# harveybc/gym-fx

Measured on AMD Instinct MI355X. Metric: env-steps/sec (whole node) PPO EURUSD-1m 4096 vec-envs, higher is better.
Workload: dtype bf16; 1 GPU; model=PPO MLP(256,256) actor-critic bf16 MFMA, global_batch=524288, seq_len=32, parallelism=dp1, n_envs_per_gpu=4096, rollout_steps=128, obs_dim=260, preprocessor=feature_window_preprocessor, reward=pnl_reward, pairs=1

## Files before the change

### gymfx_amd/algo/ppo.py

```python
from __future__ import annotations

import time
from dataclasses import dataclass
from typing import Any, Dict, List

import torch

from ..envs.vec_env import VecFxEnv
from ..models.lstm import ActorCriticLSTM
from ..models.mlp import ActorCriticMLP
from ..ops import api


@dataclass
class PPOConfig:
    rollout_steps: int = 128
    ppo_epochs: int = 4
    minibatches: int = 8
    gamma: float = 0.99
    gae_lambda: float = 0.95
    clip_eps: float = 0.2
    ent_coef: float = 0.01
    vf_coef: float = 0.5
    lr: float = 3e-4
    max_grad_norm: float = 0.5
    seed: int = 0
    hidden: int = 256
    normalize_adv: bool = True
    shuffle_rows: bool = True
    use_graphs: bool = True
    policy: str = "mlp"
    bptt_len: int = 16
    fused_rollout: bool = False
    rollout_streams: int = 1
    fuse_sample: bool = True
    fuse_head: bool = False
    overlap_gather: bool = False

    @classmethod
    def from_config(cls, cfg: Dict[str, Any]) -> "PPOConfig":
        out = cls()
        mapping = {
            "rollout_steps": "rollout_steps",
            "ppo_epochs": "ppo_epochs",
            "minibatches": "minibatches",
            "gamma": "gamma",
            "gae_lambda": "gae_lambda",
            "clip_eps": "clip_eps",
            "ent_coef": "ent_coef",
            "vf_coef": "vf_coef",
            "lr": "learning_rate",
            "max_grad_norm": "max_grad_norm",
            "hidden": "hidden_size",
            "normalize_adv": "normalize_adv",
            "shuffle_rows": "shuffle_rows",
            "use_graphs": "use_graphs",
            "policy": "policy_model",
            "bptt_len": "bptt_len",
            "rollout_streams": "rollout_streams",
            "fused_rollout": "fused_rollout",
            "fuse_sample": "fuse_sample",
            "fuse_head": "fuse_head",
            "overlap_gather": "overlap_gather",
        }
        from ..config.merger import convert_type

        for attr, key in mapping.items():
            if cfg.get(key) is not None:
                cur = getattr(out, attr)
                val = convert_type(cfg[key]) if isinstance(cur, bool) else cfg[key]
                setattr(out, attr, type(cur)(val))
        if cfg.get("seed") is not None:
            out.seed = int(cfg["seed"])
        return out


class PPOTrainer:
    def __init__(self, env: VecFxEnv, cfg: PPOConfig, *, rank: int = 0,
                 world_size: int = 1, process_group=None):
        self.env = env
        self.cfg = cfg
        self.rank = rank
        self.world_size = world_size
        self.pg = process_group
        self.device = env.device
        if getattr(env.params, "action_space_mode", "discrete") != "discrete":
            raise ValueError(
                "PPO training uses the 3-way discrete head; set "
                "action_space_mode='discrete' (continuous mode is for "
                "external agents driving the env, reference "
                "env.py:343-360 coercion semantics)")

        N = env.n_envs
        T = cfg.rollout_steps
        D = env.obs_dim
        self.N, self.T, self.D = N, T, D
        n_actions = 3

        self.recurrent = cfg.policy == "lstm"
        if self.recurrent:
            if T % cfg.bptt_len != 0:
                raise ValueError("rollout_steps must divide by bptt_len")
            if not cfg.shuffle_rows:
                raise ValueError("recurrent PPO requires shuffle_rows")
            self.model = ActorCriticLSTM(
                D, n_actions, cfg.hidden, device=self.device, seed=cfg.seed
            )
        else:
            self.model = ActorCriticMLP(
                D, n_actions, cfg.hidden, device=self.device, seed=cfg.seed
            )

        dev = self.device
        self.obs_buf = torch.empty(T, N, D, dtype=torch.bfloat16, device=dev)
        self.act_buf = torch.empty(T, N, dtype=torch.int64, device=dev)
        self.logp_buf = torch.empty(T, N, dtype=torch.float32, device=dev)
        self.val_buf = torch.empty(T + 1, N, dtype=torch.float32, device=dev)
        self.rew_buf = torch.empty(T, N, dtype=torch.float32, device=dev)
        self.done_buf = torch.empty(T, N, dtype=torch.bool, device=dev)
        self.adv_buf = torch.empty(T, N, dtype=torch.float32, device=dev)
        self.ret_buf = torch.empty(T, N, dtype=torch.float32, device=dev)
        self._adv_part = torch.empty(512, dtype=torch.float32, device=dev)

        self.acts_rollout = self.model.alloc_acts(N)
        self.obs_bf16_step = torch.empty(N, D, dtype=torch.bfloat16, device=dev)

        TN = T * N
        self.obs_flat = self.obs_buf.view(TN, D)
        self.act_flat = self.act_buf.view(TN)
        self.logp_flat = self.logp_buf.view(TN)
        self.adv_flat = self.adv_buf.view(TN)
        self.ret_flat = self.ret_buf.view(TN)
        self.losses = torch.zeros(5, dtype=torch.float32, device=dev)

        if self.recurrent:
            H = cfg.hidden
            L = cfg.bptt_len
            self.n_chunks = T // L
            n_seq = self.n_chunks * N
            if n_seq % cfg.minibatches != 0:
                raise ValueError("(T/bptt_len)*n_envs must divide by minibatches")
            Mseq = n_seq // cfg.minibatches
            self.mseq = Mseq
            self.mb_rows = L * Mseq
            self.rnn_state = self.model.alloc_state(N)
            self.h0_buf = torch.zeros(self.n_chunks, N, H, dtype=torch.float32, device=dev)
            self.c0_buf = torch.zeros(self.n_chunks, N, H, dtype=torch.float32, device=dev)
            self.obs_mb_seq = torch.empty(L, Mseq, D, dtype=torch.bfloat16, device=dev)
            self.act_mb = torch.empty(L, Mseq, dtype=torch.int64, device=dev)
            self.logp_mb = torch.empty(L, Mseq, dtype=torch.float32, device=dev)
            self.adv_mb = torch.empty(L, Mseq, dtype=torch.float32, device=dev)
            self.ret_mb = torch.empty(L, Mseq, dtype=torch.float32, device=dev)
            self.done_mb = torch.empty(L, Mseq, dtype=torch.bool, device=dev)
            self.h0_mb = torch.empty(Mseq, H, dtype=torch.bfloat16, device=dev)
            self.c0_mb = torch.empty(Mseq, H, dtype=torch.float32, device=dev)
            self.bptt = self.model.alloc_bptt(L, Mseq)
            self.dhead = torch.empty(L * Mseq, n_actions + 1,
                                     dtype=torch.bfloat16, device=dev)
            self._boot_state = self.model.alloc_state(N)
            self._overlap = False
        else:
            M = TN // cfg.minibatches
            if M * cfg.minibatches != TN:
                raise ValueError("rollout_steps * n_envs must divide by minibatches")
            self.mb_rows = M
            self.acts_train = self.model.alloc_acts(M)
            self.scratch = self.model.alloc_scratch(M)
            self.dhead = torch.empty(M, n_actions + 1, dtype=torch.bfloat16, device=dev)
            self._overlap = (self.device.type == "cuda" and cfg.overlap_gather
                             and cfg.shuffle_rows)
            ns = 2 if self._overlap else 1
            self.obs_mb_s = [torch.empty(M, D, dtype=torch.bfloat16, device=dev)
                             for _ in range(ns)]
            self.act_mb_s = [torch.empty(M, dtype=torch.int64, device=dev)
                             for _ in range(ns)]
            self.logp_mb_s = [torch.empty(M, dtype=torch.float32, device=dev)
                              for _ in range(ns)]
            self.adv_mb_s = [torch.empty(M, dtype=torch.float32, device=dev)
                             for _ in range(ns)]
            self.ret_mb_s = [torch.empty(M, dtype=torch.float32, device=dev)
                             for _ in range(ns)]
            self.obs_mb = self.obs_mb_s[0]
            self.act_mb = self.act_mb_s[0]
            self.logp_mb = self.logp_mb_s[0]
            self.adv_mb = self.adv_mb_s[0]
            self.ret_mb = self.ret_mb_s[0]

        self.step_base = torch.zeros((), dtype=torch.int64, device=dev)
        self.mb_ctr = torch.zeros((), dtype=torch.int64, device=dev)
        self.sample_seed = cfg.seed * 1_000_003 + rank
        self.shuffle_seed = cfg.seed * 9973 + rank

        import os as _os
        self._fuse_gather = (
            not self.recurrent and self.device.type == "cuda"
            and cfg.shuffle_rows and not self._overlap
            and _os.environ.get("GYMFX_FUSE_GATHER", "0") == "1")
        self._fm = {"seed": self.shuffle_seed, "minibatches": cfg.minibatches,
                    "ctr_off": -1, "step_base": self.step_base,
                    "mb_ctr": self.mb_ctr}

        self.global_step = 0
        self.update_count = 0
        self.use_graphs = bool(cfg.use_graphs) and self.device.type == "cuda"
        self._split = (self.device.type == "cuda" and cfg.rollout_streams > 1
                       and N % 2 == 0)
        self._fused = (self.device.type == "cuda" and cfg.fused_rollout
                       and not self.recurrent and cfg.hidden == 256)
        self._fuse_sample = (self.device.type == "cuda" and cfg.fuse_sample
                             and getattr(env, "_native", None) is not None
                             and env.params.action_space_mode != "continuous")
        self._fuse_head = (self._fuse_sample and cfg.fuse_head
                           and cfg.hidden % 8 == 0 and n_actions + 1 <= 8
                           and not cfg.fused_rollout)
        if self._split:
            self._s2 = torch.cuda.Stream()
            self.acts_half = [self.model.alloc_acts(N // 2),
                              self.model.alloc_acts(N // 2)]
        if self._overlap:
            self._gs = torch.cuda.Stream()
        self._graphs_ready = False
        self.g_rollout = None
        self.g_gather = None
        self.g_fwd_bwd = None
        self.g_opt = None
        from ..parallel.ddp import GradAllReducer
        self._reducer = GradAllReducer(world_size, process_group)

    def _rollout_half(self, lo: int, hi: int, acts) -> None:
        env, model = self.env, self.model
        T = self.T
        rec = self.recurrent
        L = self.cfg.bptt_len if rec else 0
        state = None
        if rec:
            state = {"h": self.rnn_state["h"][lo:hi],
                     "c": self.rnn_state["c"][lo:hi]}
        for t in range(T):
            obs_t = self.obs_buf[t][lo:hi]
            h2 = None
            if rec:
                if t % L == 0:
                    ch = t // L
                    self.h0_buf[ch][lo:hi].copy_(state["h"])
                    self.c0_buf[ch][lo:hi].copy_(state["c"])
                if self._fuse_head:
                    model.step_forward(obs_t, state, acts, skip_head=True)
                    head, h2 = None, state["h"]
                else:
                    head = model.step_forward(obs_t, state, acts)
            elif self._fused:
                model.fused_step(
                    obs_t, self.act_buf[t][lo:hi], self.logp_buf[t][lo:hi],
                    self.val_buf[t][lo:hi], seed=self.sample_seed, step=t,
                    step_base=self.step_base, row_offset=lo,
                )
                head = None
            elif self._fuse_head:
                h2 = model.forward_hidden(obs_t, acts)
                head = None
            else:
                head = model.forward(obs_t, acts)
            fuse = self._fuse_sample and (head is not None or h2 is not None)
            if head is not None and not fuse:
                api.sample_head(
                    head, self.sample_seed, t,
                    self.act_buf[t][lo:hi], self.logp_buf[t][lo:hi],
                    self.val_buf[t][lo:hi], step_base=self.step_base,
                    row_offset=lo,
                )
            nxt = self.obs_buf[t + 1] if t + 1 < T else self.obs_bf16_step
            wname = "Wy" if rec else "W3"
            bname = "by" if rec else "b3"
            env.step(
                self.act_buf[t], reward_out=self.rew_buf[t],
                terminated_out=self.done_buf[t], obs_bf16_out=nxt,
                env_lo=lo, env_hi=hi,
                head=head if fuse else None,
                h2=h2 if fuse else None,
                w3t=model.wt(wname) if (fuse and h2 is not None) else None,
                b3=model.f32(bname) if (fuse and h2 is not None) else None,
                logp_out=self.logp_buf[t] if fuse else None,
                value_out=self.val_buf[t] if fuse else None,
                step_base=self.step_base if fuse else None,
                sample_seed=self.sample_seed, sample_step=t,
                rnn_h=state["h"] if rec else None,
                rnn_c=state["c"] if rec else None,
            )

    def _rollout_body(self) -> None:
        env, model = self.env, self.model
        T = self.T
        api.f32_to_bf16(env._obs, self.obs_buf[0])
        if self._split:
            half = self.N // 2
            ev_fork = torch.cuda.Event()
            ev_join = torch.cuda.Event()
            ev_fork.record()
            with torch.cuda.stream(self._s2):
                self._s2.wait_event(ev_fork)
                self._rollout_half(half, self.N, self.acts_half[1])
                ev_join.record()
            self._rollout_half(0, half, self.acts_half[0])
            torch.cuda.current_stream().wait_event(ev_join)
        else:
            self._rollout_half(0, self.N, self.acts_rollout)
        if self.recurrent:
            self._boot_state["h"].copy_(self.rnn_state["h"])
            self._boot_state["c"].copy_(self.rnn_state["c"])
            head = model.step_forward(self.obs_bf16_step, self._boot_state,
                                      self.acts_rollout, fused=False)
        else:
            head = model.forward(self.obs_bf16_step, self.acts_rollout)
        self.val_buf[T].copy_(head[:, -1])
        api.increment_counter(self.step_base, T)

    def _gae_body(self) -> None:
        api.gae(
            self.rew_buf, self.val_buf, self.done_buf, self.adv_buf,
            self.ret_buf, self.cfg.gamma, self.cfg.gae_lambda,
        )
        if self.cfg.normalize_adv:
            api.adv_normalize(self.adv_buf.view(-1), self._adv_part)

    def _gather_body(self, slot: int = 0) -> None:
        cfg = self.cfg
        if self.recurrent:
            api.mb_gather_seq(
                self.obs_buf, self.act_buf, self.logp_buf, self.adv_buf,
                self.ret_buf, self.done_buf, self.h0_buf, self.c0_buf,
                self.obs_mb_seq, self.act_mb, self.logp_mb, self.adv_mb,
                self.ret_mb, self.done_mb, self.h0_mb, self.c0_mb,
                L=cfg.bptt_len, seed=self.shuffle_seed,
                minibatches=cfg.minibatches, step_base=self.step_base,
                mb_ctr=self.mb_ctr,
            )
        else:
            api.mb_gather(
                self.obs_flat, self.act_flat, self.logp_flat, self.adv_flat,
                self.ret_flat, self.obs_mb_s[slot], self.act_mb_s[slot],
                self.logp_mb_s[slot], self.adv_mb_s[slot], self.ret_mb_s[slot],
                seed=self.shuffle_seed, minibatches=cfg.minibatches,
                step_base=self.step_base, mb_ctr=self.mb_ctr,
                skip_obs=self._fuse_gather,
            )
        api.increment_counter(self.mb_ctr, 1)

    def _fwd_bwd_body(self, slot: int = 0) -> None:
        cfg, model = self.cfg, self.model
        if self.recurrent:
            head = model.bptt_forward(self.obs_mb_seq, self.done_mb,
                                      self.h0_mb, self.c0_mb, self.bptt)
            api.ppo_loss_bwd(
                head, self.act_mb.view(-1), self.logp_mb.view(-1),
                self.adv_mb.view(-1), self.ret_mb.view(-1), self.dhead,
                clip_eps=cfg.clip_eps, ent_coef=cfg.ent_coef,
                vf_coef=cfg.vf_coef, inv_count=1.0 / self.mb_rows,
                losses=self.losses,
            )
            model.bptt_backward(self.obs_mb_seq, self.done_mb, self.dhead,
                                self.bptt)
            return
        if self._fuse_gather:
            head = model.forward(self.obs_flat, self.acts_train,
                                 a_feistel=self._fm)
        else:
            head = model.forward(self.obs_mb_s[slot], self.acts_train)
        api.ppo_loss_bwd(
            head, self.act_mb_s[slot], self.logp_mb_s[slot],
            self.adv_mb_s[slot], self.ret_mb_s[slot],
            self.dhead, clip_eps=cfg.clip_eps, ent_coef=cfg.ent_coef,
            vf_coef=cfg.vf_coef, inv_count=1.0 / self.mb_rows,
            losses=self.losses,
        )
        if self._fuse_gather:
            model.backward(self.obs_flat, self.acts_train, self.dhead,
                           self.scratch, a_feistel=self._fm)
        else:
            model.backward(self.obs_mb_s[slot], self.acts_train, self.dhead,
                           self.scratch)

    def _mb_body(self, slot: int = 0) -> None:
        self._gather_body(slot)
        self._fwd_bwd_body(slot)

    def _mb_body_noshuffle(self, epoch_mb: int) -> None:
        cfg, model = self.cfg, self.model
        M = self.mb_rows
        mb = epoch_mb % cfg.minibatches
        sl = slice(mb * M, (mb + 1) * M)
        self.obs_mb.copy_(self.obs_flat[sl])
        self.act_mb.copy_(self.act_flat[sl])
        self.logp_mb.copy_(self.logp_flat[sl])
        self.adv_mb.copy_(self.adv_flat[sl])
        self.ret_mb.copy_(self.ret_flat[sl])
        head = model.forward(self.obs_mb, self.acts_train)
        api.ppo_loss_bwd(
            head, self.act_mb, self.logp_mb, self.adv_mb, self.ret_mb,
            self.dhead, clip_eps=cfg.clip_eps, ent_coef=cfg.ent_coef,
            vf_coef=cfg.vf_coef, inv_count=1.0 / M, losses=self.losses,
        )
        model.backward(self.obs_mb, self.acts_train, self.dhead, self.scratch)

    def _opt_body(self) -> None:
        self.model.adam(self.cfg.lr, max_grad_norm=self.cfg.max_grad_norm)

    def _snapshot(self) -> Dict[str, Any]:
        m = self.model
        snap = {
            "params": m.params.clone(), "m": m.m.clone(), "v": m.v.clone(),
            "params_bf16": m.params_bf16.clone(),
            "adam_ctr": m.adam_ctr.clone(), "adam_step": m.adam_step,
            "step_base": self.step_base.clone(), "mb_ctr": self.mb_ctr.clone(),
            "obs": self.env._obs.clone(),
            "st": {k: v.clone() for k, v in self.env.st.to_dict().items()},
        }
        if self.recurrent:
            snap["rnn_h"] = self.rnn_state["h"].clone()
            snap["rnn_c"] = self.rnn_state["c"].clone()
        return snap

    def _restore(self, snap: Dict[str, Any]) -> None:
        m = self.model
        m.params.copy_(snap["params"])
        m.m.copy_(snap["m"])
        m.v.copy_(snap["v"])
        m.params_bf16.copy_(snap["params_bf16"])
        m._refresh_wt()
        m.adam_ctr.copy_(snap["adam_ctr"])
        m.adam_step = snap["adam_step"]
        self.step_base.copy_(snap["step_base"])
        self.mb_ctr.copy_(snap["mb_ctr"])
        self.env._obs.copy_(snap["obs"])
        st = self.env.st.to_dict()
        for k, v in snap["st"].items():
            st[k].copy_(v)
        if self.recurrent:
            self.rnn_state["h"].copy_(snap["rnn_h"])
            self.rnn_state["c"].copy_(snap["rnn_c"])

    def _capture_graphs(self) -> None:
        snap = self._snapshot()
        self._rollout_body()
        self._gae_body()
        self.mb_ctr.zero_()
        nslots = 2 if self._overlap else 1
        for s in range(nslots):
            self._mb_body(s)
        self._allreduce_grads()
        self._opt_body()
        torch.cuda.synchronize()
        self.g_rollout = torch.cuda.CUDAGraph()
        with torch.cuda.graph(self.g_rollout):
            self._rollout_body()
            self._gae_body()
        self.g_gather = []
        self.g_fwd_bwd = []
        for s in range(nslots):
            g = torch.cuda.CUDAGraph()
            with torch.cuda.graph(g):
                self._gather_body(s)
            self.g_gather.append(g)
            g = torch.cuda.CUDAGraph()
            with torch.cuda.graph(g):
                self._fwd_bwd_body(s)
            self.g_fwd_bwd.append(g)
        self.g_opt = torch.cuda.CUDAGraph()
        with torch.cuda.graph(self.g_opt):
            self._opt_body()
        torch.cuda.synchronize()
        self._restore(snap)
        torch.cuda.synchronize()
        self._graphs_ready = True

    def collect_rollout(self) -> None:
        if self.use_graphs and self._graphs_ready:
            self.g_rollout.replay()
        else:
            self._rollout_body()
            self._gae_body()
        self.global_step += self.T

    def compute_advantages(self) -> None:
        pass

    def update(self, with_stats: bool = True) -> Dict[str, float]:
        cfg = self.cfg
        self.losses.zero_()
        self.mb_ctr.zero_()
        graphs = self.use_graphs and self._graphs_ready
        n_mb = cfg.ppo_epochs * cfg.minibatches
        if not cfg.shuffle_rows:
            for i in range(n_mb):
                self._mb_body_noshuffle(i)
                self._allreduce_grads()
                self._opt_body()
            self.update_count += 1
            return self._stats(n_mb) if with_stats else {}
        def gather(slot: int) -> None:
# ... 157 lines not shown
```

### gymfx_amd/config/defaults.py

```python
from __future__ import annotations

DEFAULT_VALUES = {
    "mode": "inference",
    "driver_mode": "buy_hold",
    "steps": 500,

    "data_feed_plugin": "default_data_feed",
    "broker_plugin": "default_broker",
    "strategy_plugin": "default_strategy",
    "preprocessor_plugin": "default_preprocessor",
    "reward_plugin": "pnl_reward",
    "metrics_plugin": "default_metrics",

    "input_data_file": "examples/data/eurusd.csv",
    "date_column": "DATE_TIME",
    "price_column": "CLOSE",
    "instrument": "EUR_USD",
    "timeframe": "M1",
    "headers": True,
    "max_rows": None,

    "window_size": 32,
    "initial_cash": 10000.0,
    "position_size": 1.0,
    "simulation_engine": "vectorized",
    "execution_cost_profile": None,
    "commission": 0.0,
    "slippage": 0.0,

    "replay_actions_file": None,

    "remote_log": None,
    "remote_load_config": None,
    "remote_save_config": None,
    "username": None,
    "password": None,
    "load_config": None,
    "save_config": "./config_out.json",
    "save_log": "./debug_out.json",
    "results_file": "./results.json",
    "quiet_mode": False,

    "n_envs": 1,
    "device": "auto",
    "seed": None,
    "autoreset": False,
    "env_start_mode": "zero",
    "action_space_mode": "discrete",
    "continuous_action_threshold": 0.33,
    "min_equity": None,
    "financing_enabled": False,
    "rollover_rate_data": None,
    "financing_rate_data_file": None,
    "rollover_hour_utc": 22,
    "enforce_margin_preflight": False,

    "policy_model": "mlp",
    "hidden_size": 256,
    "rollout_steps": 128,
    "ppo_epochs": 4,
    "minibatches": 8,
    "bptt_len": 16,
    "learning_rate": 3e-4,
    "gamma": 0.99,
    "gae_lambda": 0.95,
    "clip_eps": 0.2,
    "ent_coef": 0.01,
    "vf_coef": 0.5,
    "max_grad_norm": 0.5,
    "train_updates": 10,
    "use_graphs": True,
    "fuse_sample": True,
    "overlap_gather": False,
    "checkpoint_file": None,
    "checkpoint_interval": 0,
    "resume": False,
    "trace_file": None,

    "serve_host": "127.0.0.1",
    "serve_port": 8400,

    "optimization_trials": 16,
    "optimization_steps": 256,
    "optimization_refine_trials": 0,
}
```

### gymfx_amd/models/lstm.py

```python
from __future__ import annotations

import math
from dataclasses import dataclass
from typing import Dict, Optional, Tuple

import torch

from ..ops import api


@dataclass
class _ParamSlice:
    name: str
    shape: Tuple[int, ...]
    sl: slice
    is_weight: bool


class ActorCriticLSTM:
    recurrent = True

    def __init__(
        self,
        obs_dim: int,
        n_actions: int = 3,
        hidden: int = 256,
        *,
        device: torch.device,
        seed: int = 0,
    ):
        self.obs_dim = obs_dim
        self.n_actions = n_actions
        self.hidden = hidden
        self.head_dim = n_actions + 1
        self.device = device
        H = hidden

        dims = [
            ("Wx", (obs_dim, 4 * H), True),
            ("Wh", (H, 4 * H), True),
            ("b", (4 * H,), False),
            ("Wy", (H, self.head_dim), True),
            ("by", (self.head_dim,), False),
        ]
        self.slices: Dict[str, _ParamSlice] = {}
        off = 0
        for name, shape, is_w in dims:
            n = int(torch.tensor(shape).prod())
            self.slices[name] = _ParamSlice(name, shape, slice(off, off + n), is_w)
            off += n
        self.n_params = off

        g = torch.Generator().manual_seed(seed)
        flat = torch.empty(off, dtype=torch.float32)
        for name, shape, is_w in dims:
            s = self.slices[name]
            if is_w:
                bound = 1.0 / math.sqrt(shape[0])
                flat[s.sl] = (torch.rand(s.sl.stop - s.sl.start, generator=g) * 2 - 1) * bound
            else:
                flat[s.sl] = 0.0
        b = flat[self.slices["b"].sl].view(H, 4)
        b[:, 1] = 1.0
        self.params = flat.to(device)
        self.grads = torch.zeros_like(self.params)
        self.m = torch.zeros_like(self.params)
        self.v = torch.zeros_like(self.params)
        self.params_bf16 = self.params.to(torch.bfloat16)
        self._wt: Dict[str, torch.Tensor] = {}
        for name in ("Wx", "Wh", "Wy"):
            K_, N_ = self.slices[name].shape
            self._wt[name] = torch.empty(N_, K_, dtype=torch.bfloat16, device=device)
        self._refresh_wt()
        self.adam_step = 0
        self.adam_ctr = torch.zeros((), dtype=torch.int32, device=device)
        self._clip_part = torch.zeros(256, dtype=torch.float32, device=device)
        self._clip_scale = torch.ones(1, dtype=torch.float32, device=device)
        self._wg_ws: Dict[str, Tuple[torch.Tensor, Optional[torch.Tensor], int]] = {}
        self.wgrad_slabs = 64

    def w(self, name: str) -> torch.Tensor:
        s = self.slices[name]
        return self.params_bf16[s.sl].view(*s.shape)

    def wt(self, name: str) -> torch.Tensor:
        return self._wt[name]

    def f32(self, name: str) -> torch.Tensor:
        s = self.slices[name]
        return self.params[s.sl].view(*s.shape)

    def grad(self, name: str) -> torch.Tensor:
        s = self.slices[name]
        return self.grads[s.sl].view(*s.shape)

    def _refresh_wt(self) -> None:
        for name, t in self._wt.items():
            api.transpose_bf16(self.w(name), t)

    def _wg_slabs(self, K: int, N: int) -> int:
        import os
        ov = os.environ.get("GYMFX_WGRAD_SLABS")
        if ov:
            return int(ov)
        tiles = ((K + 63) // 64) * ((N + 63) // 64)
        s = self.wgrad_slabs
        while tiles * s < 2048:
            s *= 2
        return s

    def _wg_workspace(self, name: str, K: int, N: int, want_db: bool):
        key = f"{name}:{K}x{N}"
        if key not in self._wg_ws:
            S = self._wg_slabs(K, N)
            dw = torch.empty(S, K, N, dtype=torch.float32, device=self.device)
            db = torch.empty(S, N, dtype=torch.float32, device=self.device) if want_db else None
            self._wg_ws[key] = (dw, db, S)
        return self._wg_ws[key]

    def alloc_state(self, M: int) -> Dict[str, torch.Tensor]:
        dev, H = self.device, self.hidden
        return {
            "h": torch.zeros(M, H, dtype=torch.bfloat16, device=dev),
            "c": torch.zeros(M, H, dtype=torch.float32, device=dev),
        }

    def alloc_acts(self, M: int) -> Dict[str, torch.Tensor]:
        dev, H = self.device, self.hidden
        return {
            "gates": torch.empty(M, 4 * H, dtype=torch.bfloat16, device=dev),
            "gates_h": torch.empty(M, 4 * H, dtype=torch.bfloat16, device=dev),
            "head": torch.empty(M, self.head_dim, dtype=torch.float32, device=dev),
            "h_tmp": torch.empty(M, H, dtype=torch.bfloat16, device=dev),
        }

    def step_forward(self, obs_bf16: torch.Tensor, state: Dict[str, torch.Tensor],
                     acts: Dict[str, torch.Tensor], *,
                     fused: bool = True,
                     skip_head: bool = False) -> "Optional[torch.Tensor]":
        gates = acts["gates"]
        api.gemm(obs_bf16, self.wt("Wx"), self.f32("b"), gates, act=1, trans_b=True)
        if fused and "h_tmp" in acts:
            api.lstm_step_fused(state["h"], self.wt("Wh"), gates,
                                acts["gates_h"], state["c"], state["c"],
                                acts["h_tmp"])
            state["h"], acts["h_tmp"] = acts["h_tmp"], state["h"]
        else:
            api.gemm(state["h"], self.wt("Wh"), None, acts["gates_h"], act=1,
                     trans_b=True)
            api.lstm_cell_fwd(gates, acts["gates_h"], state["c"], state["c"],
                              state["h"])
        if skip_head:
            return None
        api.gemm(state["h"], self.wt("Wy"), self.f32("by"), acts["head"], act=0, trans_b=True)
        return acts["head"]

    def alloc_bptt(self, L: int, M: int) -> Dict[str, torch.Tensor]:
        dev, H = self.device, self.hidden
        return {
            "h_in": torch.empty(L + 1, M, H, dtype=torch.bfloat16, device=dev),
            "c_in": torch.empty(L + 1, M, H, dtype=torch.float32, device=dev),
            "h_raw": torch.empty(L, M, H, dtype=torch.bfloat16, device=dev),
            "c_raw": torch.empty(L, M, H, dtype=torch.float32, device=dev),
            "gates": torch.empty(L, M, 4 * H, dtype=torch.bfloat16, device=dev),
            "acts": torch.empty(L, M, 4 * H, dtype=torch.bfloat16, device=dev),
            "gh_scratch": torch.empty(M, 4 * H, dtype=torch.bfloat16, device=dev),
            "head": torch.empty(L * M, self.head_dim, dtype=torch.float32, device=dev),
            "dgates": torch.empty(L, M, 4 * H, dtype=torch.bfloat16, device=dev),
            "dh_all": torch.empty(L, M, H, dtype=torch.bfloat16, device=dev),
            "dh_na": torch.empty(M, H, dtype=torch.float32, device=dev),
            "dh_nb": torch.empty(M, H, dtype=torch.float32, device=dev),
            "dc_a": torch.empty(M, H, dtype=torch.float32, device=dev),
            "dc_b": torch.empty(M, H, dtype=torch.float32, device=dev),
        }

    def bptt_forward(self, obs_seq: torch.Tensor, done_seq: torch.Tensor,
                     h0: torch.Tensor, c0: torch.Tensor,
                     buf: Dict[str, torch.Tensor]) -> torch.Tensor:
        L, M, D = obs_seq.shape
        H = self.hidden
        gates_flat = buf["gates"].view(L * M, 4 * H)
        api.gemm(obs_seq.view(L * M, D), self.wt("Wx"), self.f32("b"),
                 gates_flat, act=1, trans_b=True)
        buf["h_in"][0].copy_(h0)
        buf["c_in"][0].copy_(c0)
        for l in range(L):
            api.lstm_step_fused(buf["h_in"][l], self.wt("Wh"),
                                buf["gates"][l], buf["gh_scratch"],
                                buf["c_in"][l], buf["c_raw"][l],
                                buf["h_raw"][l], done_seq[l],
                                buf["h_in"][l + 1], buf["c_in"][l + 1],
                                acts_out=buf["acts"][l])
        api.gemm(buf["h_raw"].view(L * M, H), self.wt("Wy"), self.f32("by"),
                 buf["head"], act=0, trans_b=True)
        return buf["head"]

    def bptt_backward(self, obs_seq: torch.Tensor, done_seq: torch.Tensor,
                      dhead: torch.Tensor, buf: Dict[str, torch.Tensor]) -> None:
        L, M, D = obs_seq.shape
        H = self.hidden
        h_raw_flat = buf["h_raw"].view(L * M, H)
        dw_p, db_p, slabs = self._wg_workspace("Wy", H, self.head_dim, True)
        api.wgrad(h_raw_flat, dhead, self.grad("Wy"), self.grad("by"),
                  workspace=(dw_p, db_p), slabs=slabs)
        dh_flat = buf["dh_all"].view(L * M, H)
        api.gemm(dhead, self.w("Wy"), None, dh_flat, act=1, trans_b=True)
        dc_next: Optional[torch.Tensor] = None
        dh_next: Optional[torch.Tensor] = None
        dc_bufs = (buf["dc_a"], buf["dc_b"])
        dh_bufs = (buf["dh_na"], buf["dh_nb"])
        for l in range(L - 1, -1, -1):
            dc_out = dc_bufs[l & 1]
            dh_out = dh_bufs[l & 1] if l > 0 else None
            api.lstm_bwd_step(buf["acts"][l],
                              buf["c_in"][l], buf["c_raw"][l],
                              buf["dh_all"][l], dh_next, dc_next,
                              done_seq[l], self.w("Wh"), buf["dgates"][l],
                              dc_out, dh_out)
            dc_next = dc_out
            dh_next = dh_out
        dgates_flat = buf["dgates"].view(L * M, 4 * H)
        dw_p, db_p, slabs = self._wg_workspace("Wx", D, 4 * H, True)
        api.wgrad(obs_seq.view(L * M, D), dgates_flat, self.grad("Wx"),
                  self.grad("b"), workspace=(dw_p, db_p), slabs=slabs)
        dw_p, db_p, slabs = self._wg_workspace("Wh", H, 4 * H, False)
        api.wgrad(buf["h_in"][:L].reshape(L * M, H), dgates_flat,
                  self.grad("Wh"), None, workspace=(dw_p, db_p), slabs=slabs)

    def adam(self, lr: float, *, beta1=0.9, beta2=0.999, eps=1e-8,
             max_grad_norm: float = 0.0) -> None:
        self.adam_step += 1
        clip = None
        if max_grad_norm and max_grad_norm > 0:
            clip = (self._clip_part, max_grad_norm)
        api.adam(self.params, self.grads, self.m, self.v, self.params_bf16,
                 lr=lr, beta1=beta1, beta2=beta2, eps=eps, step=self.adam_step,
                 step_ctr=self.adam_ctr, clip=clip)
        api.increment_counter(self.adam_ctr, 1)
        self._refresh_wt()

    def zero_grad(self) -> None:
        self.grads.zero_()

    def state_dict(self) -> Dict[str, torch.Tensor]:
        return {
            "params": self.params.detach().cpu(),
            "m": self.m.detach().cpu(),
            "v": self.v.detach().cpu(),
            "adam_step": torch.tensor(int(self.adam_ctr.item())),
            "obs_dim": torch.tensor(self.obs_dim),
            "n_actions": torch.tensor(self.n_actions),
            "hidden": torch.tensor(self.hidden),
            "arch": "lstm",
        }

    def load_state_dict(self, sd: Dict[str, torch.Tensor]) -> None:
        self.params.copy_(sd["params"].to(self.device))
        self.m.copy_(sd["m"].to(self.device))
        self.v.copy_(sd["v"].to(self.device))
        self.adam_step = int(sd["adam_step"])
        self.adam_ctr.fill_(self.adam_step)
        self.params_bf16.copy_(self.params.to(torch.bfloat16))
        self._refresh_wt()
```

### gymfx_amd/models/mlp.py

```python
from __future__ import annotations

import math
from dataclasses import dataclass
from typing import Dict, Optional, Tuple

import torch

from ..ops import api


@dataclass
class _ParamSlice:
    name: str
    shape: Tuple[int, ...]
    sl: slice
    is_weight: bool


class ActorCriticMLP:
    def __init__(
        self,
        obs_dim: int,
        n_actions: int = 3,
        hidden: int = 256,
        *,
        device: torch.device,
        seed: int = 0,
    ):
        self.obs_dim = obs_dim
        self.n_actions = n_actions
        self.hidden = hidden
        self.head_dim = n_actions + 1
        self.device = device

        dims = [
            ("W1", (obs_dim, hidden), True),
            ("b1", (hidden,), False),
            ("W2", (hidden, hidden), True),
            ("b2", (hidden,), False),
            ("W3", (hidden, self.head_dim), True),
            ("b3", (self.head_dim,), False),
        ]
        self.slices: Dict[str, _ParamSlice] = {}
        off = 0
        for name, shape, is_w in dims:
            n = int(torch.tensor(shape).prod())
            self.slices[name] = _ParamSlice(name, shape, slice(off, off + n), is_w)
            off += n
        self.n_params = off

        g = torch.Generator().manual_seed(seed)
        flat = torch.empty(off, dtype=torch.float32)
        for name, shape, is_w in dims:
            s = self.slices[name]
            if is_w:
                fan_in = shape[0]
                bound = 1.0 / math.sqrt(fan_in)
                flat[s.sl] = (torch.rand(s.sl.stop - s.sl.start, generator=g) * 2 - 1) * bound
            else:
                flat[s.sl] = 0.0
        self.params = flat.to(device)
        self.grads = torch.zeros_like(self.params)
        self.m = torch.zeros_like(self.params)
        self.v = torch.zeros_like(self.params)
        self.params_bf16 = self.params.to(torch.bfloat16)
        self._wt: Dict[str, torch.Tensor] = {}
        for name in ("W1", "W2", "W3"):
            s = self.slices[name]
            K_, N_ = s.shape
            self._wt[name] = torch.empty(N_, K_, dtype=torch.bfloat16, device=device)
        self._refresh_wt()
        self.adam_step = 0
        self.adam_ctr = torch.zeros((), dtype=torch.int32, device=device)
        self._clip_part = torch.zeros(256, dtype=torch.float32, device=device)
        self._clip_scale = torch.ones(1, dtype=torch.float32, device=device)
        self._wg_ws: Dict[str, Tuple[torch.Tensor, Optional[torch.Tensor]]] = {}
        self.wgrad_slabs = 64

    def w(self, name: str) -> torch.Tensor:
        s = self.slices[name]
        return self.params_bf16[s.sl].view(*s.shape)

    def wt(self, name: str) -> torch.Tensor:
        return self._wt[name]

    def _refresh_wt(self) -> None:
        for name, t in self._wt.items():
            api.transpose_bf16(self.w(name), t)

    def f32(self, name: str) -> torch.Tensor:
        s = self.slices[name]
        return self.params[s.sl].view(*s.shape)

    def grad(self, name: str) -> torch.Tensor:
        s = self.slices[name]
        return self.grads[s.sl].view(*s.shape)

    def _wg_slabs(self, K: int, N: int) -> int:
        import os
        ov = os.environ.get("GYMFX_WGRAD_SLABS")
        if ov:
            return int(ov)
        tiles = ((K + 63) // 64) * ((N + 63) // 64)
        s = self.wgrad_slabs
        while tiles * s < 2048:
            s *= 2
        return s

    def _wg_workspace(self, name: str, K: int, N: int, want_db: bool):
        key = f"{name}:{K}x{N}"
        if key not in self._wg_ws:
            S = self._wg_slabs(K, N)
            dw = torch.empty(S, K, N, dtype=torch.float32, device=self.device)
            db = torch.empty(S, N, dtype=torch.float32, device=self.device) if want_db else None
            self._wg_ws[key] = (dw, db, S)
        return self._wg_ws[key]

    def alloc_acts(self, M: int) -> Dict[str, torch.Tensor]:
        dev = self.device
        return {
            "h1": torch.empty(M, self.hidden, dtype=torch.bfloat16, device=dev),
            "h2": torch.empty(M, self.hidden, dtype=torch.bfloat16, device=dev),
            "head": torch.empty(M, self.head_dim, dtype=torch.float32, device=dev),
        }

    def fused_step(self, obs_bf16: torch.Tensor, actions: torch.Tensor,
                   logp: torch.Tensor, value: torch.Tensor, *, seed: int,
                   step: int, step_base: torch.Tensor, row_offset: int = 0,
                   greedy: bool = False) -> None:
        from ..ops import native
        native.require().mlp_policy_rollout(
            obs_bf16, self.wt("W1"), self.f32("b1"), self.wt("W2"),
            self.f32("b2"), self.wt("W3"), self.f32("b3"), actions, logp,
            value, seed, step, step_base, row_offset, greedy)

    def forward(self, obs_bf16: torch.Tensor, acts: Dict[str, torch.Tensor],
                a_feistel: "Optional[dict]" = None) -> torch.Tensor:
        api.gemm(obs_bf16, self.wt("W1"), self.f32("b1"), acts["h1"], act=2,
                 trans_b=True, a_perm=a_feistel)
        api.gemm(acts["h1"], self.wt("W2"), self.f32("b2"), acts["h2"], act=2, trans_b=True)
        api.gemm(acts["h2"], self.wt("W3"), self.f32("b3"), acts["head"], act=0, trans_b=True)
        return acts["head"]

    def forward_hidden(self, obs_bf16: torch.Tensor,
                       acts: Dict[str, torch.Tensor]) -> torch.Tensor:
        api.gemm(obs_bf16, self.wt("W1"), self.f32("b1"), acts["h1"], act=2, trans_b=True)
        api.gemm(acts["h1"], self.wt("W2"), self.f32("b2"), acts["h2"], act=2, trans_b=True)
        return acts["h2"]

    def backward(
        self,
        obs_bf16: torch.Tensor,
        acts: Dict[str, torch.Tensor],
        dhead: torch.Tensor,
        scratch: Dict[str, torch.Tensor],
        a_feistel: "Optional[dict]" = None,
    ) -> None:
        M = dhead.shape[0]
        dh2 = scratch["dh2"]
        dh1 = scratch["dh1"]
        dw_p, db_p, slabs = self._wg_workspace("W3", self.hidden, self.head_dim, True)
        api.wgrad(acts["h2"], dhead, self.grad("W3"), self.grad("b3"),
                  workspace=(dw_p, db_p), slabs=slabs)
        api.gemm(dhead, self.w("W3"), None, dh2, Yact=acts["h2"], trans_b=True,
                 act=1, dact_tanh=True)
        dw_p, db_p, slabs = self._wg_workspace("W2", self.hidden, self.hidden, True)
        api.wgrad(acts["h1"], dh2, self.grad("W2"), self.grad("b2"),
                  workspace=(dw_p, db_p), slabs=slabs)
        api.gemm(dh2, self.w("W2"), None, dh1, Yact=acts["h1"], trans_b=True,
                 act=1, dact_tanh=True)
        dw_p, db_p, slabs = self._wg_workspace("W1", self.obs_dim, self.hidden, True)
        api.wgrad(obs_bf16, dh1, self.grad("W1"), self.grad("b1"),
                  workspace=(dw_p, db_p), slabs=slabs, x_perm=a_feistel)

    def alloc_scratch(self, M: int) -> Dict[str, torch.Tensor]:
        dev = self.device
        return {
            "dh2": torch.empty(M, self.hidden, dtype=torch.bfloat16, device=dev),
            "dh1": torch.empty(M, self.hidden, dtype=torch.bfloat16, device=dev),
        }

    def adam(self, lr: float, *, beta1=0.9, beta2=0.999, eps=1e-8,
             max_grad_norm: float = 0.0) -> None:
        self.adam_step += 1
        clip = None
        if max_grad_norm and max_grad_norm > 0:
            clip = (self._clip_part, max_grad_norm)
        api.adam(self.params, self.grads, self.m, self.v, self.params_bf16,
                 lr=lr, beta1=beta1, beta2=beta2, eps=eps, step=self.adam_step,
                 step_ctr=self.adam_ctr, clip=clip)
        api.increment_counter(self.adam_ctr, 1)
        self._refresh_wt()

    def zero_grad(self) -> None:
        self.grads.zero_()

    def state_dict(self) -> Dict[str, torch.Tensor]:
        return {
            "params": self.params.detach().cpu(),
            "m": self.m.detach().cpu(),
            "v": self.v.detach().cpu(),
            "adam_step": torch.tensor(int(self.adam_ctr.item())),
            "obs_dim": torch.tensor(self.obs_dim),
            "n_actions": torch.tensor(self.n_actions),
            "hidden": torch.tensor(self.hidden),
        }

    def load_state_dict(self, sd: Dict[str, torch.Tensor]) -> None:
        self.params.copy_(sd["params"].to(self.device))
        self.m.copy_(sd["m"].to(self.device))
        self.v.copy_(sd["v"].to(self.device))
        self.adam_step = int(sd["adam_step"])
        self.adam_ctr.fill_(self.adam_step)
        self.params_bf16.copy_(self.params.to(torch.bfloat16))
        self._refresh_wt()
```

### gymfx_amd/ops/api.py

```python
from __future__ import annotations

from typing import Optional, Tuple

import os

import torch

from . import native

_LSTM_FUSED = os.environ.get("GYMFX_LSTM_FUSED", "1") != "0"
_LSTM_BWD_FUSED = os.environ.get("GYMFX_LSTM_BWD_FUSED", "0") == "1"


def _use_native(t: torch.Tensor) -> bool:
    if t.is_cuda:
        native.require()
        return True
    return False



def gemm(
    A: torch.Tensor,
    B: torch.Tensor,
    bias: Optional[torch.Tensor],
    C: torch.Tensor,
    *,
    Yact: Optional[torch.Tensor] = None,
    trans_b: bool = False,
    act: int = 1,
    dact_tanh: bool = False,
    accum: bool = False,
    a_perm: "Optional[dict]" = None,
) -> torch.Tensor:
    if _use_native(A):
        if a_perm is not None:
            native.require().gemm(A, B, bias, C, Yact, trans_b, act,
                                  dact_tanh, accum,
                                  ap_seed=a_perm["seed"],
                                  ap_minibatches=a_perm["minibatches"],
                                  ap_ctr_off=a_perm.get("ctr_off", 0),
                                  ap_step_base=a_perm["step_base"],
                                  ap_mb_ctr=a_perm["mb_ctr"])
            return C
        native.require().gemm(A, B, bias, C, Yact, trans_b, act, dact_tanh,
                              accum)
        return C
    if a_perm is not None:
        A = A[_perm_rows(A.shape[0], C.shape[0], a_perm)]
    a = A.to(torch.float32)
    b = B.to(torch.float32)
    if trans_b:
        b = b.t()
    out = a @ b
    if bias is not None:
        out = out + bias
    if act == 2:
        out = torch.tanh(out)
    if dact_tanh:
        y = Yact.to(torch.float32)
        out = out * (1.0 - y * y)
    if act == 0:
        if accum:
            C.add_(out)
        else:
            C.copy_(out)
    else:
        C.copy_(out.to(torch.bfloat16))
    return C


def lstm_cell_fwd(
    gates_pre: torch.Tensor,
    gates_h: "Optional[torch.Tensor]",
    c_prev: torch.Tensor,
    c_new: torch.Tensor,
    h_new: torch.Tensor,
    done: "Optional[torch.Tensor]" = None,
    h_masked: "Optional[torch.Tensor]" = None,
    c_masked: "Optional[torch.Tensor]" = None,
    acts_out: "Optional[torch.Tensor]" = None,
) -> None:
    if _use_native(gates_pre):
        native.require().lstm_cell_fwd(gates_pre, gates_h, c_prev, c_new,
                                       h_new, done, h_masked, c_masked,
                                       acts_out)
        return
    gp = gates_pre.to(torch.float32)
    if gates_h is not None:
        gp = gp + gates_h.to(torch.float32)
    M, H4 = gp.shape
    H = H4 // 4
    gv = gp.view(M, H, 4)
    i = torch.sigmoid(gv[..., 0])
    f = torch.sigmoid(gv[..., 1])
    g = torch.tanh(gv[..., 2])
    o = torch.sigmoid(gv[..., 3])
    if acts_out is not None:
        acts_out.copy_(torch.stack([i, f, g, o], dim=2).view(M, 4 * H)
                       .to(torch.bfloat16))
    c = f * c_prev + i * g
    c_new.copy_(c)
    h_new.copy_((o * torch.tanh(c)).to(torch.bfloat16))
    if done is not None:
        keep = (~done).unsqueeze(1)
        h_masked.copy_(torch.where(keep, h_new, torch.zeros_like(h_new)))
        c_masked.copy_(torch.where(keep, c_new, torch.zeros_like(c_new)))


def lstm_cell_bwd(
    acts: torch.Tensor,
    c_prev: torch.Tensor,
    c_new: torch.Tensor,
    dh_head: torch.Tensor,
    dh_next: Optional[torch.Tensor],
    dc_next: Optional[torch.Tensor],
    done: Optional[torch.Tensor],
    dgates: torch.Tensor,
    dc_prev: torch.Tensor,
) -> None:
    if _use_native(acts):
        native.require().lstm_cell_bwd(acts, c_prev, c_new,
                                       dh_head, dh_next, dc_next, done,
                                       dgates, dc_prev)
        return
    M, H4 = acts.shape
    H = H4 // 4
    mask = None
    if done is not None:
        mask = (~done).to(torch.float32).unsqueeze(1)
    dh_head = dh_head.to(torch.float32)
    av = acts.to(torch.float32).view(M, H, 4)
    i = av[..., 0]
    f = av[..., 1]
    g = av[..., 2]
    o = av[..., 3]
    tc = torch.tanh(c_new)
    dh = dh_head.clone()
    if dh_next is not None:
        dh = dh + (mask * dh_next if mask is not None else dh_next)
    dc = dh * o * (1 - tc * tc)
    if dc_next is not None:
        dc = dc + (mask * dc_next if mask is not None else dc_next)
    d = torch.stack([
        dc * g * i * (1 - i),
        dc * c_prev * f * (1 - f),
        dc * i * (1 - g * g),
        dh * tc * o * (1 - o),
    ], dim=2).view(M, 4 * H)
    dgates.copy_(d.to(torch.bfloat16))
    dc_prev.copy_(dc * f)


def lstm_step_fused(
    h_in: torch.Tensor,
    wh_t: torch.Tensor,
    gates_pre: torch.Tensor,
    gates_h_buf: torch.Tensor,
    c_prev: torch.Tensor,
    c_new: torch.Tensor,
    h_new: torch.Tensor,
    done: "Optional[torch.Tensor]" = None,
    h_masked: "Optional[torch.Tensor]" = None,
    c_masked: "Optional[torch.Tensor]" = None,
    acts_out: "Optional[torch.Tensor]" = None,
) -> None:
    if _LSTM_FUSED and _use_native(gates_pre):
        ok = native.require().lstm_gemm_cell_fwd(
            h_in, wh_t, gates_pre, acts_out,
            c_prev, c_new, h_new, done, h_masked, c_masked)
        if ok:
            return
    gemm(h_in, wh_t, None, gates_h_buf, act=1, trans_b=True)
    lstm_cell_fwd(gates_pre, gates_h_buf, c_prev, c_new, h_new, done,
                  h_masked, c_masked, acts_out)


def lstm_bwd_step(
    acts: torch.Tensor,
    c_prev: torch.Tensor,
    c_new: torch.Tensor,
    dh_head: torch.Tensor,
    dh_next: "Optional[torch.Tensor]",
    dc_next: "Optional[torch.Tensor]",
    done: "Optional[torch.Tensor]",
    wh: torch.Tensor,
    dgates: torch.Tensor,
    dc_prev: torch.Tensor,
    dh_prev: "Optional[torch.Tensor]" = None,
) -> None:
    if _LSTM_BWD_FUSED and _use_native(acts):
        ok = native.require().lstm_bwd_fused(
            acts, c_prev, c_new, dh_head, dh_next, dc_next,
            done, wh, dgates, dc_prev, dh_prev)
        if ok:
            return
    lstm_cell_bwd(acts, c_prev, c_new, dh_head, dh_next,
                  dc_next, done, dgates, dc_prev)
    if dh_prev is not None:
        gemm(dgates, wh, None, dh_prev, act=0, trans_b=True)


def mask_reset(h: torch.Tensor, c: torch.Tensor, done: torch.Tensor) -> None:
    if _use_native(c):
        native.require().mask_reset(h, c, done)
        return
    h[done] = 0
    c[done] = 0


def masked_state(h_raw: torch.Tensor, c_raw: torch.Tensor,
                 done: torch.Tensor, h_in: torch.Tensor,
                 c_in: torch.Tensor) -> None:
    if _use_native(c_raw):
        native.require().masked_state(h_raw, c_raw, done, h_in, c_in)
        return
    keep = (~done).unsqueeze(1)
    h_in.copy_(torch.where(keep, h_raw, torch.zeros_like(h_raw)))
    c_in.copy_(torch.where(keep, c_raw, torch.zeros_like(c_raw)))


def wgrad(
    X: torch.Tensor,
    dY: torch.Tensor,
    dW: torch.Tensor,
    db: Optional[torch.Tensor],
    *,
    workspace: Optional[Tuple[torch.Tensor, Optional[torch.Tensor]]] = None,
    slabs: int = 64,
    x_perm: "Optional[dict]" = None,
) -> None:
    if _use_native(X):
        K, N = dW.shape
        if workspace is None:
            dW_part = torch.empty(slabs, K, N, dtype=torch.float32, device=X.device)
            db_part = (
                torch.empty(slabs, N, dtype=torch.float32, device=X.device)
                if db is not None
                else None
            )
        else:
            dW_part, db_part = workspace
        if x_perm is not None:
            native.require().wgrad(X, dY, dW_part, db_part, dW, db, slabs,
                                   ap_seed=x_perm["seed"],
                                   ap_minibatches=x_perm["minibatches"],
                                   ap_ctr_off=x_perm.get("ctr_off", 0),
                                   ap_step_base=x_perm["step_base"],
                                   ap_mb_ctr=x_perm["mb_ctr"])
            return
        native.require().wgrad(X, dY, dW_part, db_part, dW, db, slabs)
        return
    if x_perm is not None:
        X = X[_perm_rows(X.shape[0], dY.shape[0], x_perm)]
    x = X.to(torch.float32)
    dy = dY.to(torch.float32)
    dW.copy_(x.t() @ dy)
    if db is not None:
        db.copy_(dy.sum(dim=0))


def gae(
    rewards: torch.Tensor,
    values: torch.Tensor,
    dones: torch.Tensor,
    adv: torch.Tensor,
    ret: torch.Tensor,
    gamma: float,
    lam: float,
) -> None:
    if _use_native(rewards):
        native.require().gae(rewards, values, dones, adv, ret, gamma, lam)
        return
    T, N = rewards.shape
    running = torch.zeros(N, dtype=torch.float32)
    for t in range(T - 1, -1, -1):
        nonterm = (~dones[t]).to(torch.float32)
        delta = rewards[t] + gamma * values[t + 1] * nonterm - values[t]
        running = delta + gamma * lam * nonterm * running
        adv[t] = running
        ret[t] = running + values[t]


def adam(
    p: torch.Tensor,
    g: torch.Tensor,
    m: torch.Tensor,
    v: torch.Tensor,
    p_bf16: Optional[torch.Tensor],
    *,
    lr: float,
    beta1: float = 0.9,
    beta2: float = 0.999,
    eps: float = 1e-8,
    step: int = 1,
    gscale: Optional[torch.Tensor] = None,
    step_ctr: Optional[torch.Tensor] = None,
    clip: "Optional[Tuple[torch.Tensor, float]]" = None,
) -> None:
    if _use_native(p):
        if clip is not None:
            part, max_norm = clip
            native.require().adam(p, g, m, v, p_bf16, lr, beta1, beta2, eps,
                                  step, None, step_ctr, part, float(max_norm))
        else:
            native.require().adam(p, g, m, v, p_bf16, lr, beta1, beta2, eps,
                                  step, gscale, step_ctr)
        return
    if step_ctr is not None:
        step = int(step_ctr.item()) + 1
    if clip is not None:
        _, max_norm = clip
        norm = g.norm()
        s = float(max_norm / norm) if (max_norm > 0 and norm > max_norm) else 1.0
    else:
        s = float(gscale.item()) if gscale is not None else 1.0
    geff = g * s
    m.mul_(beta1).add_(geff, alpha=1 - beta1)
    v.mul_(beta2).addcmul_(geff, geff, value=1 - beta2)
    mhat = m / (1 - beta1 ** step)
    vhat = v / (1 - beta2 ** step)
    p.addcdiv_(mhat, vhat.sqrt() + eps, value=-lr)
    if p_bf16 is not None:
        p_bf16.copy_(p.to(torch.bfloat16))


def grad_clip_scale(
    g: torch.Tensor, max_norm: float, part: torch.Tensor, scale: torch.Tensor
) -> None:
    if _use_native(g):
        native.require().grad_clip(g, max_norm, part, scale)
        return
    norm = g.norm()
    s = max_norm / norm if (max_norm > 0 and norm > max_norm) else torch.ones(())
    scale.fill_(float(s))


def sample_head(
    head: torch.Tensor,
    seed: int,
    step: int,
    actions: torch.Tensor,
    logp: torch.Tensor,
    value: Optional[torch.Tensor] = None,
    entropy: Optional[torch.Tensor] = None,
    greedy: bool = False,
    step_base: Optional[torch.Tensor] = None,
    row_offset: int = 0,
) -> None:
    if _use_native(head):
        native.require().sample_head(head, seed, step, actions, logp, value,
                                     entropy, greedy, step_base, row_offset)
        return
    if step_base is not None:
        step = step + int(step_base.item())
    M, W = head.shape
    A = W - 1
    logits = head[:, :A]
    logz = torch.logsumexp(logits, dim=1, keepdim=True)
    logpi = logits - logz
    pi = logpi.exp()
    if greedy:
        a = logits.argmax(dim=1)
    else:
        u = _splitmix_uniform(seed, step, M, row_offset)
        cdf = pi.cumsum(dim=1)
        a = (u.unsqueeze(1) >= cdf).sum(dim=1).clamp(max=A - 1)
    actions.copy_(a)
    logp.copy_(logpi.gather(1, a.unsqueeze(1)).squeeze(1))
    if value is not None:
        value.copy_(head[:, A])
    if entropy is not None:
        entropy.copy_(-(pi * logpi).sum(dim=1))


def _splitmix_uniform(seed: int, step: int, M: int,
                      row_offset: int = 0) -> torch.Tensor:
    m = torch.arange(row_offset, row_offset + M, dtype=torch.int64)
    x = (seed ^ (step * 0x51E1F5 + m * 0x9E37)) & 0xFFFFFFFFFFFFFFFF

    def mix(x):
        mask = (1 << 64) - 1
        x = (x + 0x9E3779B97F4A7C15) & mask
        x = ((x ^ (x >> 30)) * 0xBF58476D1CE4E5B9) & mask
        x = ((x ^ (x >> 27)) * 0x94D049BB133111EB) & mask
        return x ^ (x >> 31)

    vals = [mix(int(v)) for v in x.tolist()]
    u = torch.tensor([(v >> 11) * (1.0 / 9007199254740992.0) for v in vals],
                     dtype=torch.float32)
    return u.clamp(max=0.999999)


def ppo_loss_bwd(
    head: torch.Tensor,
    actions: torch.Tensor,
    old_logp: torch.Tensor,
    adv: torch.Tensor,
    ret: torch.Tensor,
    dhead: torch.Tensor,
    *,
    clip_eps: float,
    ent_coef: float,
    vf_coef: float,
    inv_count: float,
    losses: Optional[torch.Tensor] = None,
) -> None:
    if _use_native(head):
        native.require().ppo_loss_bwd(
            head, actions, old_logp, adv, ret, dhead, clip_eps, ent_coef,
            vf_coef, inv_count, losses,
        )
        return
    M, W = head.shape
    A = W - 1
    logits = head[:, :A]
    logz = torch.logsumexp(logits, dim=1, keepdim=True)
    logpi = logits - logz
    pi = logpi.exp()
    lp = logpi.gather(1, actions.unsqueeze(1)).squeeze(1)
    ratio = (lp - old_logp).exp()
    surr1 = ratio * adv
    rclip = ratio.clamp(1 - clip_eps, 1 + clip_eps)
    surr2 = rclip * adv
    g_lp = torch.where(surr1 <= surr2, -adv * ratio, torch.zeros_like(ratio))
    onehot = torch.nn.functional.one_hot(actions, A).to(torch.float32)
    H = -(pi * logpi).sum(dim=1)
    dlogits = g_lp.unsqueeze(1) * (onehot - pi)
    dlogits = dlogits + ent_coef * pi * (logpi + H.unsqueeze(1))
    v = head[:, A]
    dv = vf_coef * (v - ret)
    d = torch.cat([dlogits, dv.unsqueeze(1)], dim=1) * inv_count
    dhead.copy_(d.to(torch.bfloat16))
    if losses is not None:
        losses[0] += float((-torch.minimum(surr1, surr2)).sum()) * inv_count
        losses[1] += float((0.5 * (v - ret) ** 2).sum()) * inv_count
        losses[2] += float(H.sum()) * inv_count
        losses[3] += float((old_logp - lp).sum()) * inv_count
        clipped = (ratio > 1 + clip_eps) | (ratio < 1 - clip_eps)
        losses[4] += float(clipped.to(torch.float32).sum()) * inv_count


def adv_normalize(adv: torch.Tensor, part: torch.Tensor) -> None:
    if _use_native(adv):
        native.require().adv_normalize(adv, part)
        return
    mean = adv.mean()
    var = (adv * adv).mean() - mean * mean
    adv.sub_(mean).div_(var.clamp(min=0).sqrt() + 1e-8)


def f32_to_bf16(src: torch.Tensor, dst: torch.Tensor) -> None:
    if _use_native(src):
        native.require().f32_to_bf16(src, dst)
        return
    dst.view(-1).copy_(src.reshape(-1).to(torch.bfloat16))



_U64 = (1 << 64) - 1


def _splitmix64_int(x: int) -> int:
    x = (x + 0x9E3779B97F4A7C15) & _U64
    x = ((x ^ (x >> 30)) * 0xBF58476D1CE4E5B9) & _U64
    x = ((x ^ (x >> 27)) * 0x94D049BB133111EB) & _U64
    return x ^ (x >> 31)


def feistel_key(seed: int, step_base: int, epoch: int) -> int:
    return _splitmix64_int(
        (seed ^ (step_base * 0x9E3779B97F4A7C15) ^ (epoch << 32)) & _U64
    )


def _perm_rows(n_rows: int, m_rows: int, perm: dict) -> torch.Tensor:
    ctr = int(perm["mb_ctr"].item()) + int(perm.get("ctr_off", 0))
    minibatches = int(perm["minibatches"])
    epoch, mb = ctr // minibatches, ctr % minibatches
    key = feistel_key(int(perm["seed"]), int(perm["step_base"].item()), epoch)
    return feistel_perm(n_rows, key)[mb * m_rows:(mb + 1) * m_rows]


def feistel_perm(n: int, key: int) -> torch.Tensor:
    import numpy as np

    bits = 2
    while (1 << bits) < n:
        bits += 2
    half = bits // 2
    mask = np.uint64((1 << half) - 1)
    x = np.arange(n, dtype=np.uint64)
    active = np.ones(n, dtype=bool)
    while active.any():
        xa = x[active]
        a = xa & mask
        b = xa >> np.uint64(half)
        for r in range(4):
            h = (np.uint64(key) ^ np.uint64(r << 48) ^ b).astype(np.uint64)
            with np.errstate(over="ignore"):
                h = h + np.uint64(0x9E3779B97F4A7C15)
                h = (h ^ (h >> np.uint64(30))) * np.uint64(0xBF58476D1CE4E5B9)
                h = (h ^ (h >> np.uint64(27))) * np.uint64(0x94D049BB133111EB)
                h = h ^ (h >> np.uint64(31))
            f = h & mask
            a, b = b, a ^ f
        xa = (b << np.uint64(half)) | a
        x[active] = xa
        active = x >= n
    return torch.from_numpy(x.astype(np.int64))


def mb_gather(
    obs_src: torch.Tensor,
    act_src: torch.Tensor,
    logp_src: torch.Tensor,
    adv_src: torch.Tensor,
    ret_src: torch.Tensor,
    obs_mb: torch.Tensor,
    act_mb: torch.Tensor,
    logp_mb: torch.Tensor,
    adv_mb: torch.Tensor,
    ret_mb: torch.Tensor,
    *,
    seed: int,
    minibatches: int,
    step_base: torch.Tensor,
    mb_ctr: torch.Tensor,
    skip_obs: bool = False,
) -> None:
    if _use_native(obs_src):
        native.require().mb_gather(
            obs_src, act_src, logp_src, adv_src, ret_src, obs_mb, act_mb,
            logp_mb, adv_mb, ret_mb, seed, minibatches, step_base, mb_ctr,
            skip_obs,
        )
        return
    n = obs_src.shape[0]
    M = obs_mb.shape[0]
    ctr = int(mb_ctr.item())
    epoch, mb = ctr // minibatches, ctr % minibatches
    key = feistel_key(seed, int(step_base.item()), epoch)
    src = feistel_perm(n, key)[mb * M:(mb + 1) * M]
    if not skip_obs:
        obs_mb.copy_(obs_src[src])
    act_mb.copy_(act_src[src])
    logp_mb.copy_(logp_src[src])
    adv_mb.copy_(adv_src[src])
    ret_mb.copy_(ret_src[src])


def mb_gather_seq(
    obs_src: torch.Tensor,
    act_src: torch.Tensor,
    logp_src: torch.Tensor,
    adv_src: torch.Tensor,
    ret_src: torch.Tensor,
    done_src: torch.Tensor,
    h0_src: torch.Tensor,
    c0_src: torch.Tensor,
    obs_mb: torch.Tensor,
    act_mb: torch.Tensor,
    logp_mb: torch.Tensor,
    adv_mb: torch.Tensor,
    ret_mb: torch.Tensor,
    done_mb: torch.Tensor,
    h0_mb: torch.Tensor,
    c0_mb: torch.Tensor,
    *,
    L: int,
    seed: int,
    minibatches: int,
    step_base: torch.Tensor,
    mb_ctr: torch.Tensor,
) -> None:
    n_chunks, N, H = h0_src.shape
    if _use_native(obs_src):
        native.require().mb_gather_seq(
            obs_src.view(-1, obs_src.shape[-1]), act_src.view(-1),
            logp_src.view(-1), adv_src.view(-1), ret_src.view(-1),
            done_src.view(-1),
            h0_src, c0_src, obs_mb.view(-1, obs_mb.shape[-1]),
            act_mb.view(-1), logp_mb.view(-1), adv_mb.view(-1),
            ret_mb.view(-1), done_mb.view(-1), h0_mb, c0_mb, L, N, seed,
            minibatches, step_base, mb_ctr,
        )
        return
    Mseq = c0_mb.shape[0]
    n_seq = n_chunks * N
    ctr = int(mb_ctr.item())
    epoch, mb = ctr // minibatches, ctr % minibatches
    key = feistel_key(seed, int(step_base.item()), epoch)
    src = feistel_perm(n_seq, key)[mb * Mseq:(mb + 1) * Mseq]
    chunk = src // N
    env = src % N
    h0_mb.copy_(h0_src[chunk, env].to(torch.bfloat16))
    c0_mb.copy_(c0_src[chunk, env])
    for li in range(L):
        t = chunk * L + li
        obs_mb[li].copy_(obs_src[t, env])
        act_mb[li].copy_(act_src[t, env])
        logp_mb[li].copy_(logp_src[t, env])
        adv_mb[li].copy_(adv_src[t, env])
        ret_mb[li].copy_(ret_src[t, env])
        done_mb[li].copy_(done_src[t, env])


def increment_counter(ctr: torch.Tensor, delta: int) -> None:
    if _use_native(ctr):
        native.require().increment_counter(ctr, delta)
        return
    ctr.add_(delta)


def transpose_bf16(src: torch.Tensor, dst: torch.Tensor) -> None:
    if _use_native(src):
        native.require().transpose_bf16(src, dst)
        return
    dst.copy_(src.t())
```

### gymfx_amd/ops/csrc/bindings.cpp

```cpp
#include <torch/extension.h>

#include <c10/hip/HIPStream.h>
#include <hip/hip_runtime.h>

#include <unordered_map>
#include <string>
#include <vector>

#include "env_common.h"

namespace gymfx {

void launch_env_step(const EnvPtrs& P, const EnvParamsK& K, int env_lo,
                     int env_cnt, hipStream_t stream);
void launch_build_obs(const EnvPtrs& P, const EnvParamsK& K, int env_lo,
                      int env_cnt, hipStream_t stream);
void launch_env_step_obs(const EnvPtrs& P, const EnvParamsK& K, int env_lo,
                         int env_cnt, hipStream_t stream);
void launch_gemm(const void* A, const void* B, const float* bias, void* C,
                 const void* Yact, int M, int N, int K, bool trans_b, int act,
                 bool dact_tanh, bool add_bias, bool accum, hipStream_t stream,
                 const FeistelMap* fmp = nullptr);
void launch_lstm_cell_fwd(const void* gates_pre, const void* gates_h,
                          const float* c_prev, float* c_new, void* h_new,
                          const bool* done, void* h_masked, float* c_masked,
                          void* acts_out, int64_t M, int H,
                          hipStream_t stream);
void launch_lstm_cell_bwd(const void* acts, const float* c_prev,
                          const float* c_new, const void* dh_head,
                          const float* dh_next, const float* dc_next,
                          const bool* done, void* dgates, float* dc_prev,
                          int64_t M, int H, hipStream_t stream);
bool launch_lstm_gemm_cell_fwd(const void* A, const void* B,
                               const void* gates_pre, void* acts_out,
                               const float* c_prev, float* c_new, void* h_new,
                               const bool* done, void* h_masked,
                               float* c_masked, int M, int N, int K,
                               hipStream_t stream);
bool launch_lstm_bwd_fused(const void* acts, const float* c_prev,
                           const float* c_new, const void* dh_head,
                           const float* dh_next, const float* dc_next,
                           const bool* done, const void* B, void* dgates,
                           float* dc_prev, float* dh_prev, int M, int H,
                           hipStream_t stream);
void launch_mask_reset(void* h, float* c, const bool* done, int64_t M, int H,
                       hipStream_t stream);
void launch_masked_state(const void* h_raw, const float* c_raw,
                         const bool* done, void* h_in, float* c_in, int64_t M,
                         int H, hipStream_t stream);
void launch_mb_gather_seq(const void* obs_src, const int64_t* act_src,
                          const float* logp_src, const float* adv_src,
                          const float* ret_src, const bool* done_src,
                          const float* h0_src,
                          const float* c0_src, void* obs_mb, int64_t* act_mb,
                          float* logp_mb, float* adv_mb, float* ret_mb,
                          bool* done_mb,
                          void* h0_mb, float* c0_mb, int Mseq, int L, int D,
                          int H, int N, uint32_t n_seq, int half,
                          uint64_t seed, int minibatches,
                          const unsigned long long* step_base,
                          const unsigned long long* mb_ctr,
                          hipStream_t stream);
void launch_wgrad(const void* X, const void* dY, float* dW_part, float* db_part,
                  float* dW, float* db, int M, int N, int K, int slabs,
                  hipStream_t stream, const FeistelMap* fmp = nullptr);
void launch_gae(const float* rewards, const float* values, const bool* dones,
                float* adv, float* ret, int T, int N, float gamma, float lam,
                hipStream_t stream);
void launch_adam(float* p, const float* g, float* m, float* v, void* p_bf16,
                 int64_t n, float lr, float beta1, float beta2, float eps,
                 float bc1, float bc2, const float* gscale, const int* step_ctr,
                 hipStream_t stream);
void launch_grad_clip(const float* g, int64_t n, float max_norm, float* part,
                      float* scale, int nparts, hipStream_t stream);
void launch_grad_sumsq(const float* g, int64_t n, float* part, int nparts,
                       hipStream_t stream);
void launch_adam_clip(float* p, const float* g, float* m, float* v,
                      void* p_bf16, int64_t n, float lr, float beta1,
                      float beta2, float eps, float bc1, float bc2,
                      const int* step_ctr, const float* clip_part, int nparts,
                      float max_norm, hipStream_t stream);
void launch_sample_head(const float* head, int M, int n_actions, uint64_t seed,
                        uint64_t step, int64_t* actions, float* logp,
                        float* value, float* entropy, int greedy,
                        const unsigned long long* step_base, int row_offset,
                        hipStream_t stream);
void launch_increment_u64(unsigned long long* ctr, unsigned long long delta,
                          hipStream_t stream);
void launch_mlp_policy_rollout(const void* obs, const void* W1t,
                               const float* b1, const void* W2t,
                               const float* b2, const void* W3t,
                               const float* b3, int64_t* actions, float* logp,
                               float* value, int N, int D, int n_actions,
                               uint64_t seed, uint64_t step,
                               const unsigned long long* step_base,
                               int row_offset, int greedy, hipStream_t stream);
void launch_increment_i32(int* ctr, int delta, hipStream_t stream);
void launch_mb_gather(const void* obs_src, const int64_t* act_src,
                      const float* logp_src, const float* adv_src,
                      const float* ret_src, void* obs_mb, int64_t* act_mb,
                      float* logp_mb, float* adv_mb, float* ret_mb, int M,
                      int D, uint32_t n, int half, uint64_t seed,
                      int minibatches, const unsigned long long* step_base,
                      const unsigned long long* mb_ctr, hipStream_t stream,
                      int skip_obs = 0);
void launch_ppo_loss_bwd(const float* head, const int64_t* actions,
                         const float* old_logp, const float* adv,
                         const float* ret, void* dhead, int M, int n_actions,
                         float clip_eps, float ent_coef, float vf_coef,
                         float inv_count, float* losses, hipStream_t stream);
void launch_adv_normalize(float* adv, int64_t n, float* part, int nparts,
                          hipStream_t stream);
void launch_f32_to_bf16(const float* in, void* out, int64_t n,
                        hipStream_t stream);
void launch_transpose_bf16(const void* src, void* dst, int K, int N,
                           hipStream_t stream);

namespace {

using TensorMap = std::unordered_map<std::string, torch::Tensor>;

template <typename T>
T* ptr(TensorMap& m, const char* key, bool required = true) {
  auto it = m.find(key);
  if (it == m.end() || !it->second.defined()) {
    TORCH_CHECK(!required, "GymFxEngine: missing tensor '", key, "'");
    return nullptr;
  }
  return it->second.data_ptr<T>();
}

}

struct GymFxEngine {
  EnvPtrs P{};
  EnvParamsK K{};
  TensorMap state, market, outputs;
  bool continuous = false;

  GymFxEngine(const py::dict& iparams, const py::dict& fparams,
              const py::dict& state_d, const py::dict& market_d) {
    for (auto item : state_d)
      state[py::cast<std::string>(item.first)] = py::cast<torch::Tensor>(item.second);
    for (auto item : market_d)
      market[py::cast<std::string>(item.first)] = py::cast<torch::Tensor>(item.second);

    auto gi = [&](const char* k) { return py::cast<int64_t>(iparams[k]); };
    auto gf = [&](const char* k) { return py::cast<double>(fparams[k]); };

    K.n_envs = (int)gi("n_envs");
    K.T = (int)gi("T");
    K.window = (int)gi("window");
    K.n_features = (int)gi("n_features");
    K.reward_id = (int)gi("reward_id");
    K.strategy_id = (int)gi("strategy_id");
    K.prep_id = (int)gi("prep_id");
    K.scaling_mode = (int)gi("scaling_mode");
    K.scale_window = (int)gi("scale_window");
    K.sharpe_window = (int)gi("sharpe_window");
    K.atr_period = (int)gi("atr_period");
    K.size_mode = (int)gi("size_mode");
    K.risk_mode = (int)gi("risk_mode");
    K.collision_policy = (int)gi("collision_policy");
    K.limit_policy = (int)gi("limit_policy");
    K.latency_bars = (int)gi("latency_bars");
    K.margin_model = (int)gi("margin_model");
    K.flags = (int)gi("flags");
    K.obs_dim = (int)gi("obs_dim");
    K.off_features = (int)gi("off_features");
    K.off_prices = (int)gi("off_prices");
    K.off_returns = (int)gi("off_returns");
    K.off_agent = (int)gi("off_agent");
    K.off_fc = (int)gi("off_fc");
    K.off_cal = (int)gi("off_cal");
    continuous = (K.flags & F_CONTINUOUS) != 0;

    K.initial_cash = gf("initial_cash");
    K.position_size = gf("position_size");
    K.commission = gf("commission");
    K.slippage = gf("slippage");
    K.leverage = gf("leverage");
    K.min_equity = gf("min_equity");
    K.cont_threshold = gf("cont_threshold");
    K.reward_scale = gf("reward_scale");
    K.annualization = gf("annualization");
    K.penalty_lambda = gf("penalty_lambda");
    K.sl_pips = gf("sl_pips");
    K.tp_pips = gf("tp_pips");
    K.pip_size = gf("pip_size");
    K.k_sl = gf("k_sl");
    K.k_tp = gf("k_tp");
    K.rel_volume = gf("rel_volume");
    K.min_order_volume = gf("min_order_volume");
    K.max_order_volume = gf("max_order_volume");
    K.min_sltp_frac = gf("min_sltp_frac");
    K.max_sltp_frac = gf("max_sltp_frac");
    K.baseline_rel_volume = gf("baseline_rel_volume");
    K.max_risk_rel_volume = gf("max_risk_rel_volume");
    K.sl_shrink_alpha = gf("sl_shrink_alpha");
    K.tp_shrink_alpha = gf("tp_shrink_alpha");
    K.min_k_sl = gf("min_k_sl");
    K.min_rr = gf("min_rr");
    K.mplf = gf("mplf");
    K.fc_pen_coef = gf("fc_pen_coef");
    K.fc_pen_window_hours = gf("fc_pen_window_hours");
    K.feature_clip = gf("feature_clip");
    K.overlay_threshold = gf("overlay_threshold");
    K.margin_init_rate = gf("margin_init_rate");

    P.open_px = ptr<float>(market, "open");
    P.high_px = ptr<float>(market, "high");
    P.low_px = ptr<float>(market, "low");
    P.close_px = ptr<float>(market, "close");
    P.price_px = ptr<float>(market, "price");
    P.features = ptr<float>(market, "features", false);
    P.p1 = ptr<double>(market, "feat_prefix1", false);
    P.p2 = ptr<double>(market, "feat_prefix2", false);
    P.binary_mask = ptr<bool>(market, "binary_mask", false);
    P.ev_no_trade = ptr<float>(market, "ev_no_trade");
    P.force_close = ptr<float>(market, "force_close", false);
    P.calendar = ptr<float>(market, "calendar", false);
    P.sess_entry = ptr<bool>(market, "sess_entry");
    P.sess_close = ptr<bool>(market, "sess_close");
    P.roll_rate = ptr<float>(market, "roll_rate", false);

    P.cursor = ptr<int>(state, "cursor");
    P.started = ptr<bool>(state, "started");
    P.terminated = ptr<bool>(state, "terminated");
    P.pos = ptr<double>(state, "pos");
    P.avg_entry = ptr<double>(state, "avg_entry");
    P.cash = ptr<double>(state, "cash");
    P.margin_used = ptr<double>(state, "margin_used");
    P.equity = ptr<double>(state, "equity");
    P.prev_equity = ptr<double>(state, "prev_equity");
    P.peak_equity = ptr<double>(state, "peak_equity");
    P.commission_paid = ptr<double>(state, "commission_paid");
    P.last_trade_cost = ptr<double>(state, "last_trade_cost");
    P.trade_count = ptr<int>(state, "trade_count");
    P.pend_close = ptr<bool>(state, "pend_close");
    P.pend_open_dir = ptr<int8_t>(state, "pend_open_dir");
    P.pend_open_size = ptr<float>(state, "pend_open_size");
    P.pend_sl = ptr<float>(state, "pend_sl");
    P.pend_tp = ptr<float>(state, "pend_tp");
    P.pend_wait = ptr<int>(state, "pend_wait");
    P.br_active = ptr<bool>(state, "br_active");
    P.br_armed = ptr<bool>(state, "br_armed");
    P.br_sl = ptr<float>(state, "br_sl");
    P.br_tp = ptr<float>(state, "br_tp");
    P.tr_ring = ptr<float>(state, "tr_ring");
    P.tr_count = ptr<int>(state, "tr_count");
    P.tr_sum = ptr<float>(state, "tr_sum");
    P.prev_close_atr = ptr<float>(state, "prev_close_atr");
    P.rew_ring = ptr<float>(state, "rew_ring");
    P.rew_count = ptr<int>(state, "rew_count");
    P.rew_s1 = ptr<double>(state, "rew_s1");
    P.rew_s2 = ptr<double>(state, "rew_s2");
    P.trade_won = ptr<int>(state, "trade_won");
    P.trade_lost = ptr<int>(state, "trade_lost");
// ... 82 lines not shown
                      rnn_h->scalar_type() == torch::kBFloat16 &&
                      rnn_h->dim() == 2 && rnn_h->size(0) == cnt,
                  "rnn_h must be contiguous bf16 [env_cnt, H]");
      TORCH_CHECK(rnn_c->is_contiguous() &&
                      rnn_c->scalar_type() == torch::kFloat32 &&
                      rnn_c->sizes() == rnn_h->sizes(),
                  "rnn_c must be contiguous f32 [env_cnt, H]");
      P.rnn_h = rnn_h->data_ptr();
      P.rnn_c = rnn_c->data_ptr<float>();
      K.rnn_hidden = (int)rnn_h->size(1);
    }
    if (h2.has_value()) {
      TORCH_CHECK(!continuous, "fused sampling requires discrete actions");
      TORCH_CHECK(!head.has_value(), "pass either head or h2, not both");
      TORCH_CHECK(w3t.has_value() && b3.has_value(), "h2 needs w3t and b3");
      TORCH_CHECK(h2->is_contiguous() &&
                      h2->scalar_type() == torch::kBFloat16 && h2->dim() == 2,
                  "h2 must be contiguous bf16 [env_cnt, H]");
      TORCH_CHECK(w3t->is_contiguous() &&
                      w3t->scalar_type() == torch::kBFloat16 &&
                      w3t->dim() == 2 && w3t->size(1) == h2->size(1),
                  "w3t must be contiguous bf16 [A+1, H]");
      TORCH_CHECK(h2->size(1) % 8 == 0, "H must be a multiple of 8");
      TORCH_CHECK(w3t->size(0) <= 8, "head width must be <= 8");
      TORCH_CHECK(b3->scalar_type() == torch::kFloat32 &&
                      b3->numel() == w3t->size(0),
                  "b3 must be f32 [A+1]");
      TORCH_CHECK(logp_out.has_value() && value_out.has_value(),
                  "fused sampling needs logp_out and value_out");
      P.h2 = h2->data_ptr();
      P.w3t = w3t->data_ptr();
      P.b3 = b3->data_ptr<float>();
      P.actions_out = actions.data_ptr<int64_t>();
      P.logp_out = logp_out->data_ptr<float>();
      P.value_out = value_out->data_ptr<float>();
      K.head_hidden = (int)h2->size(1);
      K.sample_nact = (int)w3t->size(0) - 1;
      K.sample_seed = (unsigned long long)sample_seed;
      K.sample_step = (long long)sample_step;
      if (step_base.has_value()) {
        P.step_base = reinterpret_cast<const unsigned long long*>(
            step_base->data_ptr());
      }
    }
    if (head.has_value()) {
      TORCH_CHECK(!continuous, "fused sampling requires discrete actions");
      TORCH_CHECK(head->is_contiguous() &&
                      head->scalar_type() == torch::kFloat32 &&
                      head->dim() == 2 &&
                      head->size(0) >= (env_hi <= 0 ? K.n_envs : env_hi) - env_lo,
                  "head must be contiguous f32 [env_cnt, A+1]");
      TORCH_CHECK(logp_out.has_value() && value_out.has_value(),
                  "fused sampling needs logp_out and value_out");
      TORCH_CHECK(logp_out->is_contiguous() &&
                      logp_out->scalar_type() == torch::kFloat32 &&
                      logp_out->numel() == K.n_envs,
                  "logp_out must be contiguous f32 [n_envs]");
      TORCH_CHECK(value_out->is_contiguous() &&
                      value_out->scalar_type() == torch::kFloat32 &&
                      value_out->numel() == K.n_envs,
                  "value_out must be contiguous f32 [n_envs]");
      P.head = head->data_ptr<float>();
      P.actions_out = actions.data_ptr<int64_t>();
      P.logp_out = logp_out->data_ptr<float>();
      P.value_out = value_out->data_ptr<float>();
      K.sample_nact = (int)head->size(1) - 1;
      K.sample_seed = (unsigned long long)sample_seed;
      K.sample_step = (long long)sample_step;
      if (step_base.has_value()) {
        TORCH_CHECK(step_base->scalar_type() == torch::kUInt64 ||
                        step_base->scalar_type() == torch::kInt64,
                    "step_base must be a 64-bit counter tensor");
        P.step_base = reinterpret_cast<const unsigned long long*>(
            step_base->data_ptr());
      }
    }
    torch::Tensor rew = outputs["reward"];
    if (reward_out.has_value()) {
      TORCH_CHECK(reward_out->is_contiguous() &&
                      reward_out->scalar_type() == torch::kFloat32 &&
                      reward_out->numel() == K.n_envs,
                  "reward_out must be contiguous f32 [n_envs]");
      rew = *reward_out;
    }
    torch::Tensor term = outputs["terminated"];
    if (terminated_out.has_value()) {
      TORCH_CHECK(terminated_out->is_contiguous() &&
                      terminated_out->scalar_type() == torch::kBool &&
                      terminated_out->numel() == K.n_envs,
                  "terminated_out must be contiguous bool [n_envs]");
      term = *terminated_out;
    }
    P.reward_out = rew.data_ptr<float>();
    P.terminated_out = term.data_ptr<bool>();
    hipStream_t stream = c10::hip::getCurrentHIPStream().stream();
    if (fuse_obs) {
      set_obs_ptrs(obs_out, obs_bf16_out);
      launch_env_step_obs(P, K, (int)env_lo, (int)(env_hi - env_lo), stream);
    } else {
      launch_env_step(P, K, (int)env_lo, (int)(env_hi - env_lo), stream);
      build_obs(obs_out, obs_bf16_out, env_lo, env_hi);
    }
    py::dict out;
    out["reward"] = rew;
    out["base_reward"] = outputs["base_reward"];
    out["force_close_reward_penalty"] = outputs["penalty"];
    out["terminated"] = term;
    out["coerced_action"] = outputs["coerced"];
    return out;
  }

  void set_obs_ptrs(torch::Tensor& obs_out,
                    c10::optional<torch::Tensor>& obs_bf16_out) {
    TORCH_CHECK(obs_out.is_contiguous() && obs_out.scalar_type() == torch::kFloat32,
                "obs_out must be contiguous f32");
    TORCH_CHECK(obs_out.numel() == (int64_t)K.n_envs * K.obs_dim, "obs_out shape");
    P.obs_out = obs_out.data_ptr<float>();
    P.obs_bf16_out = nullptr;
    if (obs_bf16_out.has_value()) {
      TORCH_CHECK(obs_bf16_out->is_contiguous() &&
                      obs_bf16_out->scalar_type() == torch::kBFloat16 &&
                      obs_bf16_out->numel() == (int64_t)K.n_envs * K.obs_dim,
                  "obs_bf16_out must be contiguous bf16 [n_envs, obs_dim]");
      P.obs_bf16_out = obs_bf16_out->data_ptr();
    }
  }

  void build_obs(torch::Tensor obs_out,
                 c10::optional<torch::Tensor> obs_bf16_out,
                 int64_t env_lo = 0, int64_t env_hi = 0) {
    if (env_hi <= 0) env_hi = K.n_envs;
    set_obs_ptrs(obs_out, obs_bf16_out);
    hipStream_t stream = c10::hip::getCurrentHIPStream().stream();
    launch_build_obs(P, K, (int)env_lo, (int)(env_hi - env_lo), stream);
  }
};

}

namespace {

hipStream_t cur_stream() { return c10::hip::getCurrentHIPStream().stream(); }

void check_bf16(const torch::Tensor& t, const char* name) {
  TORCH_CHECK(t.is_contiguous() && t.scalar_type() == torch::kBFloat16,
              name, " must be contiguous bf16");
}

void check_f32(const torch::Tensor& t, const char* name) {
  TORCH_CHECK(t.is_contiguous() && t.scalar_type() == torch::kFloat32,
              name, " must be contiguous f32");
}

static gymfx::FeistelMap make_fmap(int64_t n_rows, int M_mb, int64_t seed,
                                   int64_t minibatches, int64_t ctr_off,
                                   torch::Tensor step_base,
                                   torch::Tensor mb_ctr) {
  gymfx::FeistelMap fm;
  fm.n = (uint32_t)n_rows;
  int bits = 2;
  while ((1ll << bits) < n_rows) bits += 2;
  fm.half = bits / 2;
  fm.seed = (uint64_t)seed;
  fm.minibatches = (int)minibatches;
  fm.M_mb = M_mb;
  fm.ctr_off = (long long)ctr_off;
  fm.step_base = reinterpret_cast<const unsigned long long*>(
      step_base.data_ptr());
  fm.mb_ctr = reinterpret_cast<const unsigned long long*>(mb_ctr.data_ptr());
  return fm;
}

void gemm_op(torch::Tensor A, torch::Tensor B, c10::optional<torch::Tensor> bias,
             torch::Tensor C, c10::optional<torch::Tensor> Yact, bool trans_b,
             int64_t act, bool dact_tanh, bool accum,
             int64_t ap_seed, int64_t ap_minibatches, int64_t ap_ctr_off,
             c10::optional<torch::Tensor> ap_step_base,
             c10::optional<torch::Tensor> ap_mb_ctr) {
  TORCH_CHECK(!accum || (act == 0 && !dact_tanh && !bias.has_value()),
              "accum only supported for plain f32-out gemm");
  check_bf16(A, "A");
  check_bf16(B, "B");
  const int M = (int)A.size(0), K = (int)A.size(1);
  const int N = trans_b ? (int)B.size(0) : (int)B.size(1);
  TORCH_CHECK((trans_b ? B.size(1) : B.size(0)) == K, "gemm K mismatch");
  TORCH_CHECK(C.size(1) == N && (C.size(0) == M || ap_step_base.has_value()),
              "gemm C shape");
  if (act == 0) check_f32(C, "C"); else check_bf16(C, "C");
  const float* bias_p = nullptr;
  if (bias.has_value()) {
    check_f32(*bias, "bias");
    TORCH_CHECK(bias->numel() == N, "bias numel");
    bias_p = bias->data_ptr<float>();
  }
  const void* y_p = nullptr;
  if (dact_tanh) {
    TORCH_CHECK(Yact.has_value(), "dact_tanh needs Yact");
    check_bf16(*Yact, "Yact");
    y_p = Yact->data_ptr();
  }
  if (ap_step_base.has_value()) {
    TORCH_CHECK(ap_mb_ctr.has_value(), "a_perm needs mb_ctr");
    const int M_mb = (int)C.size(0);
    gymfx::FeistelMap fm = make_fmap(A.size(0), M_mb, ap_seed,
                                     ap_minibatches, ap_ctr_off,
                                     *ap_step_base, *ap_mb_ctr);
    gymfx::launch_gemm(A.data_ptr(), B.data_ptr(), bias_p, C.data_ptr(), y_p,
                       M_mb, N, K, trans_b, (int)act, dact_tanh,
                       bias_p != nullptr, accum, cur_stream(), &fm);
    return;
  }
  gymfx::launch_gemm(A.data_ptr(), B.data_ptr(), bias_p, C.data_ptr(), y_p, M,
                     N, K, trans_b, (int)act, dact_tanh, bias_p != nullptr,
                     accum, cur_stream());
}

void lstm_cell_fwd_op(torch::Tensor gates_pre,
                      c10::optional<torch::Tensor> gates_h,
                      torch::Tensor c_prev,
                      torch::Tensor c_new, torch::Tensor h_new,
                      c10::optional<torch::Tensor> done,
                      c10::optional<torch::Tensor> h_masked,
                      c10::optional<torch::Tensor> c_masked,
                      c10::optional<torch::Tensor> acts_out) {
  check_bf16(gates_pre, "gates_pre");
  check_f32(c_prev, "c_prev");
  check_f32(c_new, "c_new");
  check_bf16(h_new, "h_new");
  const int64_t M = c_prev.size(0);
  const int H = (int)c_prev.size(1);
  TORCH_CHECK(gates_pre.size(0) == M && gates_pre.size(1) == 4 * H,
              "gates_pre shape");
  const void* gh = nullptr;
  if (gates_h.has_value()) {
    check_bf16(*gates_h, "gates_h");
    gh = gates_h->data_ptr();
  }
  const bool* done_p = nullptr;
  void* hm_p = nullptr;
  float* cm_p = nullptr;
  if (done.has_value()) {
    TORCH_CHECK(h_masked.has_value() && c_masked.has_value(),
                "done needs h_masked and c_masked outputs");
    TORCH_CHECK(done->scalar_type() == torch::kBool && done->numel() == M,
                "done must be bool [M]");
    check_bf16(*h_masked, "h_masked");
    check_f32(*c_masked, "c_masked");
    done_p = done->data_ptr<bool>();
    hm_p = h_masked->data_ptr();
    cm_p = c_masked->data_ptr<float>();
  }
  void* acts_p = nullptr;
  if (acts_out.has_value()) {
    check_bf16(*acts_out, "acts_out");
    acts_p = acts_out->data_ptr();
  }
  gymfx::launch_lstm_cell_fwd(gates_pre.data_ptr(), gh,
                              c_prev.data_ptr<float>(),
                              c_new.data_ptr<float>(), h_new.data_ptr(),
                              done_p, hm_p, cm_p, acts_p, M, H,
                              cur_stream());
}

void lstm_cell_bwd_op(torch::Tensor acts, torch::Tensor c_prev,
                      torch::Tensor c_new, torch::Tensor dh_head,
                      c10::optional<torch::Tensor> dh_next,
                      c10::optional<torch::Tensor> dc_next,
                      c10::optional<torch::Tensor> done,
                      torch::Tensor dgates, torch::Tensor dc_prev) {
  check_bf16(acts, "acts");
  check_f32(c_prev, "c_prev");
  check_f32(c_new, "c_new");
  check_bf16(dh_head, "dh_head");
  check_bf16(dgates, "dgates");
  check_f32(dc_prev, "dc_prev");
  const int64_t M = c_prev.size(0);
  const int H = (int)c_prev.size(1);
  TORCH_CHECK(acts.size(0) == M && acts.size(1) == 4 * H, "acts shape");
  TORCH_CHECK(H % 4 == 0, "H must be a multiple of 4");
  const float* dhn = dh_next.has_value() ? dh_next->data_ptr<float>() : nullptr;
  const float* dcn = dc_next.has_value() ? dc_next->data_ptr<float>() : nullptr;
  const bool* dn = done.has_value() ? done->data_ptr<bool>() : nullptr;
  gymfx::launch_lstm_cell_bwd(
      acts.data_ptr(), c_prev.data_ptr<float>(),
      c_new.data_ptr<float>(), dh_head.data_ptr(), dhn, dcn, dn,
      dgates.data_ptr(), dc_prev.data_ptr<float>(), M, H, cur_stream());
}

bool lstm_gemm_cell_fwd_op(torch::Tensor A, torch::Tensor B,
                           torch::Tensor gates_pre,
                           c10::optional<torch::Tensor> acts_out,
                           torch::Tensor c_prev, torch::Tensor c_new,
                           torch::Tensor h_new,
                           c10::optional<torch::Tensor> done,
                           c10::optional<torch::Tensor> h_masked,
                           c10::optional<torch::Tensor> c_masked) {
  check_bf16(A, "A");
  check_bf16(B, "B");
  check_bf16(gates_pre, "gates_pre");
  check_f32(c_prev, "c_prev");
  check_f32(c_new, "c_new");
  check_bf16(h_new, "h_new");
  const int M = (int)A.size(0);
  const int K = (int)A.size(1);
  const int N = (int)B.size(0);
  TORCH_CHECK(B.size(1) == K, "B must be Wh^T [4H, H]");
  TORCH_CHECK(N == 4 * K, "N must equal 4*H");
  TORCH_CHECK(gates_pre.size(0) == M && gates_pre.size(1) == N,
              "gates_pre shape");
  void* acts_p = nullptr;
  if (acts_out.has_value()) {
    check_bf16(*acts_out, "acts_out");
    acts_p = acts_out->data_ptr();
  }
  const bool* done_p = nullptr;
  void* hm_p = nullptr;
  float* cm_p = nullptr;
  if (done.has_value()) {
    TORCH_CHECK(h_masked.has_value() && c_masked.has_value(),
                "done needs h_masked and c_masked outputs");
    done_p = done->data_ptr<bool>();
    hm_p = h_masked->data_ptr();
    cm_p = c_masked->data_ptr<float>();
  }
  return gymfx::launch_lstm_gemm_cell_fwd(
      A.data_ptr(), B.data_ptr(), gates_pre.data_ptr(), acts_p,
      c_prev.data_ptr<float>(), c_new.data_ptr<float>(), h_new.data_ptr(),
      done_p, hm_p, cm_p, M, N, K, cur_stream());
}

bool lstm_bwd_fused_op(torch::Tensor acts, torch::Tensor c_prev,
                       torch::Tensor c_new, torch::Tensor dh_head,
                       c10::optional<torch::Tensor> dh_next,
                       c10::optional<torch::Tensor> dc_next,
                       c10::optional<torch::Tensor> done, torch::Tensor B,
                       torch::Tensor dgates, torch::Tensor dc_prev,
                       c10::optional<torch::Tensor> dh_prev) {
  check_bf16(acts, "acts");
  check_f32(c_prev, "c_prev");
  check_f32(c_new, "c_new");
  check_bf16(dh_head, "dh_head");
  check_bf16(B, "B");
  check_bf16(dgates, "dgates");
  check_f32(dc_prev, "dc_prev");
  const int M = (int)c_prev.size(0);
  const int H = (int)c_prev.size(1);
  TORCH_CHECK(B.size(0) == H && B.size(1) == 4 * H, "B must be Wh [H, 4H]");
  const float* dhn = dh_next.has_value() ? dh_next->data_ptr<float>() : nullptr;
  const float* dcn = dc_next.has_value() ? dc_next->data_ptr<float>() : nullptr;
  const bool* dn = done.has_value() ? done->data_ptr<bool>() : nullptr;
  float* dhp = dh_prev.has_value() ? dh_prev->data_ptr<float>() : nullptr;
  return gymfx::launch_lstm_bwd_fused(
      acts.data_ptr(), c_prev.data_ptr<float>(),
      c_new.data_ptr<float>(), dh_head.data_ptr(), dhn, dcn, dn,
      B.data_ptr(), dgates.data_ptr(), dc_prev.data_ptr<float>(), dhp, M, H,
      cur_stream());
}

void mask_reset_op(torch::Tensor h, torch::Tensor c, torch::Tensor done) {
  check_bf16(h, "h");
  check_f32(c, "c");
  const int64_t M = c.size(0);
  const int H = (int)c.size(1);
  gymfx::launch_mask_reset(h.data_ptr(), c.data_ptr<float>(),
                           done.data_ptr<bool>(), M, H, cur_stream());
}

void masked_state_op(torch::Tensor h_raw, torch::Tensor c_raw,
                     torch::Tensor done, torch::Tensor h_in,
                     torch::Tensor c_in) {
  check_bf16(h_raw, "h_raw");
  check_f32(c_raw, "c_raw");
  check_bf16(h_in, "h_in");
  check_f32(c_in, "c_in");
  const int64_t M = c_raw.size(0);
  const int H = (int)c_raw.size(1);
  gymfx::launch_masked_state(h_raw.data_ptr(), c_raw.data_ptr<float>(),
                             done.data_ptr<bool>(), h_in.data_ptr(),
                             c_in.data_ptr<float>(), M, H, cur_stream());
}

void mb_gather_seq_op(torch::Tensor obs_src, torch::Tensor act_src,
                      torch::Tensor logp_src, torch::Tensor adv_src,
                      torch::Tensor ret_src, torch::Tensor done_src,
                      torch::Tensor h0_src,
                      torch::Tensor c0_src, torch::Tensor obs_mb,
                      torch::Tensor act_mb, torch::Tensor logp_mb,
                      torch::Tensor adv_mb, torch::Tensor ret_mb,
                      torch::Tensor done_mb,
                      torch::Tensor h0_mb, torch::Tensor c0_mb, int64_t L,
                      int64_t N, int64_t seed, int64_t minibatches,
                      torch::Tensor step_base, torch::Tensor mb_ctr) {
  check_bf16(obs_src, "obs_src");
  check_bf16(obs_mb, "obs_mb");
  check_bf16(h0_mb, "h0_mb");
  check_f32(h0_src, "h0_src");
  check_f32(c0_src, "c0_src");
  check_f32(c0_mb, "c0_mb");
  const int D = (int)obs_src.size(-1);
  const int H = (int)c0_mb.size(-1);
  const int Mseq = (int)c0_mb.size(0);
  const int64_t n_chunks = h0_src.numel() / ((int64_t)N * H);
  const int64_t n_seq = n_chunks * N;
  TORCH_CHECK((int64_t)Mseq * minibatches == n_seq,
              "Mseq * minibatches != n_seq");
  int bits = 2;
  while ((1ll << bits) < n_seq) bits += 2;
  gymfx::launch_mb_gather_seq(
      obs_src.data_ptr(), act_src.data_ptr<int64_t>(),
      logp_src.data_ptr<float>(), adv_src.data_ptr<float>(),
      ret_src.data_ptr<float>(), done_src.data_ptr<bool>(),
      h0_src.data_ptr<float>(),
      c0_src.data_ptr<float>(), obs_mb.data_ptr(),
      act_mb.data_ptr<int64_t>(), logp_mb.data_ptr<float>(),
      adv_mb.data_ptr<float>(), ret_mb.data_ptr<float>(),
      done_mb.data_ptr<bool>(), h0_mb.data_ptr(),
      c0_mb.data_ptr<float>(), Mseq, (int)L, D, H, (int)N, (uint32_t)n_seq,
      bits / 2, (uint64_t)seed, (int)minibatches,
      reinterpret_cast<const unsigned long long*>(step_base.data_ptr()),
      reinterpret_cast<const unsigned long long*>(mb_ctr.data_ptr()),
      cur_stream());
}



void wgrad_op(torch::Tensor X, torch::Tensor dY, torch::Tensor dW_part,
              c10::optional<torch::Tensor> db_part, torch::Tensor dW,
              c10::optional<torch::Tensor> db, int64_t slabs,
              int64_t ap_seed, int64_t ap_minibatches, int64_t ap_ctr_off,
              c10::optional<torch::Tensor> ap_step_base,
              c10::optional<torch::Tensor> ap_mb_ctr) {
  check_bf16(X, "X");
  check_bf16(dY, "dY");
  check_f32(dW, "dW");
  check_f32(dW_part, "dW_part");
  const bool aperm = ap_step_base.has_value();
  const int M = aperm ? (int)dY.size(0) : (int)X.size(0);
  const int K = (int)X.size(1), N = (int)dY.size(1);
  TORCH_CHECK(dY.size(0) == M, "wgrad M mismatch");
  TORCH_CHECK(dW.size(0) == K && dW.size(1) == N, "dW shape");
  TORCH_CHECK(dW_part.numel() >= slabs * (int64_t)K * N, "dW_part too small");
  float* dbp = nullptr;
  float* dbo = nullptr;
  if (db_part.has_value() && db.has_value()) {
    check_f32(*db_part, "db_part");
    check_f32(*db, "db");
    dbp = db_part->data_ptr<float>();
    dbo = db->data_ptr<float>();
  }
  if (aperm) {
    TORCH_CHECK(ap_mb_ctr.has_value(), "a_perm needs mb_ctr");
    gymfx::FeistelMap fm = make_fmap(X.size(0), M, ap_seed, ap_minibatches,
                                     ap_ctr_off, *ap_step_base, *ap_mb_ctr);
    gymfx::launch_wgrad(X.data_ptr(), dY.data_ptr(),
                        dW_part.data_ptr<float>(), dbp, dW.data_ptr<float>(),
                        dbo, M, N, K, (int)slabs, cur_stream(), &fm);
    return;
  }
  gymfx::launch_wgrad(X.data_ptr(), dY.data_ptr(), dW_part.data_ptr<float>(),
                      dbp, dW.data_ptr<float>(), dbo, M, N, K, (int)slabs,
                      cur_stream());
}

void gae_op(torch::Tensor rewards, torch::Tensor values, torch::Tensor dones,
            torch::Tensor adv, torch::Tensor ret, double gamma, double lam) {
  check_f32(rewards, "rewards");
  check_f32(values, "values");
  check_f32(adv, "adv");
  check_f32(ret, "ret");
  TORCH_CHECK(dones.scalar_type() == torch::kBool && dones.is_contiguous());
  const int T = (int)rewards.size(0), N = (int)rewards.size(1);
  TORCH_CHECK(values.size(0) == T + 1 && values.size(1) == N, "values shape");
  gymfx::launch_gae(rewards.data_ptr<float>(), values.data_ptr<float>(),
                    dones.data_ptr<bool>(), adv.data_ptr<float>(),
                    ret.data_ptr<float>(), T, N, (float)gamma, (float)lam,
                    cur_stream());
}

void adam_op(torch::Tensor p, torch::Tensor g, torch::Tensor m, torch::Tensor v,
             c10::optional<torch::Tensor> p_bf16, double lr, double beta1,
             double beta2, double eps, int64_t step,
             c10::optional<torch::Tensor> gscale,
             c10::optional<torch::Tensor> step_ctr,
             c10::optional<torch::Tensor> clip_part, double clip_max_norm) {
  check_f32(p, "p");
  check_f32(g, "g");
  check_f32(m, "m");
  check_f32(v, "v");
  const int64_t n = p.numel();
  TORCH_CHECK(g.numel() == n && m.numel() == n && v.numel() == n);
  void* pb = nullptr;
  if (p_bf16.has_value()) {
    check_bf16(*p_bf16, "p_bf16");
    pb = p_bf16->data_ptr();
  }
  const float* gs = nullptr;
  if (gscale.has_value()) gs = gscale->data_ptr<float>();
  const int* sc = nullptr;
  if (step_ctr.has_value()) {
    TORCH_CHECK(step_ctr->scalar_type() == torch::kInt32, "step_ctr int32");
    sc = step_ctr->data_ptr<int>();
  }
  const float bc1 = 1.f - powf((float)beta1, (float)step);
  const float bc2 = 1.f - powf((float)beta2, (float)step);
  if (clip_part.has_value() && clip_max_norm > 0) {
    check_f32(*clip_part, "clip_part");
    float* part = clip_part->data_ptr<float>();
    const int nparts = (int)clip_part->numel();
    gymfx::launch_grad_sumsq(g.data_ptr<float>(), n, part, nparts,
                             cur_stream());
    gymfx::launch_adam_clip(p.data_ptr<float>(), g.data_ptr<float>(),
                            m.data_ptr<float>(), v.data_ptr<float>(), pb, n,
                            (float)lr, (float)beta1, (float)beta2, (float)eps,
                            bc1, bc2, sc, part, nparts, (float)clip_max_norm,
                            cur_stream());
    return;
  }
  gymfx::launch_adam(p.data_ptr<float>(), g.data_ptr<float>(),
                     m.data_ptr<float>(), v.data_ptr<float>(), pb, n, (float)lr,
                     (float)beta1, (float)beta2, (float)eps, bc1, bc2, gs, sc,
                     cur_stream());
}

void grad_clip_op(torch::Tensor g, double max_norm, torch::Tensor part,
                  torch::Tensor scale) {
  check_f32(g, "g");
  check_f32(part, "part");
  check_f32(scale, "scale");
  gymfx::launch_grad_clip(g.data_ptr<float>(), g.numel(), (float)max_norm,
                          part.data_ptr<float>(), scale.data_ptr<float>(),
                          (int)part.numel(), cur_stream());
}

void sample_head_op(torch::Tensor head, int64_t seed, int64_t step,
                    torch::Tensor actions, torch::Tensor logp,
                    c10::optional<torch::Tensor> value,
                    c10::optional<torch::Tensor> entropy, bool greedy,
                    c10::optional<torch::Tensor> step_base,
                    int64_t row_offset) {
  check_f32(head, "head");
  const int M = (int)head.size(0);
  const int n_actions = (int)head.size(1) - 1;
  TORCH_CHECK(actions.scalar_type() == torch::kInt64);
  const unsigned long long* sb = nullptr;
  if (step_base.has_value()) {
    TORCH_CHECK(step_base->scalar_type() == torch::kUInt64 ||
                    step_base->scalar_type() == torch::kInt64,
                "step_base must be a 64-bit counter tensor");
    sb = reinterpret_cast<const unsigned long long*>(step_base->data_ptr());
  }
  gymfx::launch_sample_head(
      head.data_ptr<float>(), M, n_actions, (uint64_t)seed, (uint64_t)step,
      actions.data_ptr<int64_t>(), logp.data_ptr<float>(),
      value.has_value() ? value->data_ptr<float>() : nullptr,
      entropy.has_value() ? entropy->data_ptr<float>() : nullptr,
      greedy ? 1 : 0, sb, (int)row_offset, cur_stream());
}

void mlp_policy_rollout_op(torch::Tensor obs, torch::Tensor W1t,
                           torch::Tensor b1, torch::Tensor W2t,
                           torch::Tensor b2, torch::Tensor W3t,
                           torch::Tensor b3, torch::Tensor actions,
                           torch::Tensor logp, torch::Tensor value,
                           int64_t seed, int64_t step,
                           c10::optional<torch::Tensor> step_base,
                           int64_t row_offset, bool greedy) {
  check_bf16(obs, "obs");
  check_bf16(W1t, "W1t");
  check_bf16(W2t, "W2t");
  check_bf16(W3t, "W3t");
  const int N = (int)obs.size(0);
  const int D = (int)obs.size(1);
  const int H = (int)W1t.size(0);
  const int head_dim = (int)W3t.size(0);
  TORCH_CHECK(H == 256 && W2t.size(0) == 256 && W2t.size(1) == 256,
              "fused rollout requires hidden == 256");
  TORCH_CHECK(W1t.size(1) == D, "W1t shape");
  TORCH_CHECK(head_dim <= 16 && W3t.size(1) == 256, "W3t shape");
  const unsigned long long* sb = nullptr;
  if (step_base.has_value())
    sb = reinterpret_cast<const unsigned long long*>(step_base->data_ptr());
  gymfx::launch_mlp_policy_rollout(
      obs.data_ptr(), W1t.data_ptr(), b1.data_ptr<float>(), W2t.data_ptr(),
      b2.data_ptr<float>(), W3t.data_ptr(), b3.data_ptr<float>(),
      actions.data_ptr<int64_t>(), logp.data_ptr<float>(),
      value.data_ptr<float>(), N, D, head_dim - 1, (uint64_t)seed,
      (uint64_t)step, sb, (int)row_offset, greedy, cur_stream());
}

void increment_counter_op(torch::Tensor ctr, int64_t delta) {
  TORCH_CHECK(ctr.numel() == 1, "counter must be scalar");
  if (ctr.scalar_type() == torch::kInt32) {
    gymfx::launch_increment_i32(ctr.data_ptr<int>(), (int)delta, cur_stream());
  } else {
    TORCH_CHECK(ctr.scalar_type() == torch::kUInt64 ||
                    ctr.scalar_type() == torch::kInt64,
                "counter must be i32/i64/u64");
    gymfx::launch_increment_u64(
        reinterpret_cast<unsigned long long*>(ctr.data_ptr()),
        (unsigned long long)delta, cur_stream());
  }
}

void mb_gather_op(torch::Tensor obs_src, torch::Tensor act_src,
                  torch::Tensor logp_src, torch::Tensor adv_src,
                  torch::Tensor ret_src, torch::Tensor obs_mb,
                  torch::Tensor act_mb, torch::Tensor logp_mb,
                  torch::Tensor adv_mb, torch::Tensor ret_mb, int64_t seed,
                  int64_t minibatches, torch::Tensor step_base,
                  torch::Tensor mb_ctr, bool skip_obs) {
  check_bf16(obs_src, "obs_src");
  check_bf16(obs_mb, "obs_mb");
  const int64_t n = obs_src.size(0);
  const int D = (int)obs_src.size(1);
  const int M = (int)obs_mb.size(0);
  TORCH_CHECK(obs_mb.size(1) == D, "obs_mb D mismatch");
  TORCH_CHECK(act_src.numel() == n && logp_src.numel() == n &&
                  adv_src.numel() == n && ret_src.numel() == n,
              "src numel mismatch");
  TORCH_CHECK(act_mb.numel() == M && logp_mb.numel() == M &&
                  adv_mb.numel() == M && ret_mb.numel() == M,
              "mb numel mismatch");
  TORCH_CHECK((int64_t)M * minibatches == n, "M * minibatches != n");
  int bits = 2;
  while ((1ll << bits) < n) bits += 2;
  gymfx::launch_mb_gather(
      obs_src.data_ptr(), act_src.data_ptr<int64_t>(),
      logp_src.data_ptr<float>(), adv_src.data_ptr<float>(),
      ret_src.data_ptr<float>(), obs_mb.data_ptr(),
      act_mb.data_ptr<int64_t>(), logp_mb.data_ptr<float>(),
      adv_mb.data_ptr<float>(), ret_mb.data_ptr<float>(), M, D, (uint32_t)n,
      bits / 2, (uint64_t)seed, (int)minibatches,
      reinterpret_cast<const unsigned long long*>(step_base.data_ptr()),
      reinterpret_cast<const unsigned long long*>(mb_ctr.data_ptr()),
      cur_stream(), skip_obs ? 1 : 0);
}

void ppo_loss_bwd_op(torch::Tensor head, torch::Tensor actions,
                     torch::Tensor old_logp, torch::Tensor adv,
                     torch::Tensor ret, torch::Tensor dhead, double clip_eps,
                     double ent_coef, double vf_coef, double inv_count,
                     c10::optional<torch::Tensor> losses) {
  check_f32(head, "head");
  check_bf16(dhead, "dhead");
  const int M = (int)head.size(0);
  const int n_actions = (int)head.size(1) - 1;
  gymfx::launch_ppo_loss_bwd(
      head.data_ptr<float>(), actions.data_ptr<int64_t>(),
      old_logp.data_ptr<float>(), adv.data_ptr<float>(), ret.data_ptr<float>(),
      dhead.data_ptr(), M, n_actions, (float)clip_eps, (float)ent_coef,
      (float)vf_coef, (float)inv_count,
      losses.has_value() ? losses->data_ptr<float>() : nullptr, cur_stream());
}

void adv_normalize_op(torch::Tensor adv, torch::Tensor part) {
  check_f32(adv, "adv");
  check_f32(part, "part");
  gymfx::launch_adv_normalize(adv.data_ptr<float>(), adv.numel(),
                              part.data_ptr<float>(), (int)(part.numel() / 2),
                              cur_stream());
}

void f32_to_bf16_op(torch::Tensor in, torch::Tensor out) {
  check_f32(in, "in");
  check_bf16(out, "out");
  gymfx::launch_f32_to_bf16(in.data_ptr<float>(), out.data_ptr(), in.numel(),
                            cur_stream());
}

void transpose_bf16_op(torch::Tensor src, torch::Tensor dst) {
  check_bf16(src, "src");
  check_bf16(dst, "dst");
  const int K = (int)src.size(0), N = (int)src.size(1);
  TORCH_CHECK(dst.size(0) == N && dst.size(1) == K, "transpose shape");
  gymfx::launch_transpose_bf16(src.data_ptr(), dst.data_ptr(), K, N,
                               cur_stream());
}

}

PYBIND11_MODULE(TORCH_EXTENSION_NAME, m) {
  m.def("gemm", &gemm_op,
        "C = act(A @ B + bias); trans_b reads B as [N,K]; act 0=f32 1=bf16 "
        "2=tanh-bf16; dact_tanh multiplies by (1-Yact^2); accum does C += ",
        py::arg("A"), py::arg("B"), py::arg("bias"), py::arg("C"),
        py::arg("Yact") = py::none(), py::arg("trans_b") = false,
        py::arg("act") = 1, py::arg("dact_tanh") = false,
        py::arg("accum") = false, py::arg("ap_seed") = 0,
        py::arg("ap_minibatches") = 1, py::arg("ap_ctr_off") = 0,
        py::arg("ap_step_base") = py::none(),
        py::arg("ap_mb_ctr") = py::none());
  m.def("lstm_cell_fwd", &lstm_cell_fwd_op, py::arg("gates_pre"),
        py::arg("gates_h"), py::arg("c_prev"), py::arg("c_new"),
        py::arg("h_new"), py::arg("done") = py::none(),
        py::arg("h_masked") = py::none(), py::arg("c_masked") = py::none(),
        py::arg("acts_out") = py::none());
  m.def("lstm_gemm_cell_fwd", &lstm_gemm_cell_fwd_op,
        "fused h@Wh^T recurrent GEMM + LSTM cell epilogue; returns False "
        "when the shape has no fused kernel (caller falls back)",
        py::arg("A"), py::arg("B"), py::arg("gates_pre"),
        py::arg("acts_out"), py::arg("c_prev"), py::arg("c_new"),
        py::arg("h_new"), py::arg("done") = py::none(),
        py::arg("h_masked") = py::none(), py::arg("c_masked") = py::none());
  m.def("lstm_bwd_fused", &lstm_bwd_fused_op,
        "fused LSTM cell backward + dgates @ Wh recurrent dgrad; returns "
        "False when the shape has no fused kernel (caller falls back)",
        py::arg("acts"), py::arg("c_prev"),
        py::arg("c_new"), py::arg("dh_head"), py::arg("dh_next"),
        py::arg("dc_next"), py::arg("done"), py::arg("B"), py::arg("dgates"),
        py::arg("dc_prev"), py::arg("dh_prev") = py::none());
  m.def("lstm_cell_bwd", &lstm_cell_bwd_op, py::arg("acts"),
        py::arg("c_prev"), py::arg("c_new"), py::arg("dh_head"),
        py::arg("dh_next"), py::arg("dc_next"), py::arg("done"),
        py::arg("dgates"), py::arg("dc_prev"));
  m.def("mask_reset", &mask_reset_op, py::arg("h"), py::arg("c"),
        py::arg("done"));
  m.def("masked_state", &masked_state_op, py::arg("h_raw"), py::arg("c_raw"),
        py::arg("done"), py::arg("h_in"), py::arg("c_in"));
  m.def("mb_gather_seq", &mb_gather_seq_op, py::arg("obs_src"),
        py::arg("act_src"), py::arg("logp_src"), py::arg("adv_src"),
        py::arg("ret_src"), py::arg("done_src"), py::arg("h0_src"),
        py::arg("c0_src"),
        py::arg("obs_mb"), py::arg("act_mb"), py::arg("logp_mb"),
        py::arg("adv_mb"), py::arg("ret_mb"), py::arg("done_mb"),
        py::arg("h0_mb"),
        py::arg("c0_mb"), py::arg("L"), py::arg("N"), py::arg("seed"),
        py::arg("minibatches"), py::arg("step_base"), py::arg("mb_ctr"));
  m.def("wgrad", &wgrad_op, py::arg("X"), py::arg("dY"), py::arg("dW_part"),
        py::arg("db_part"), py::arg("dW"), py::arg("db"), py::arg("slabs"),
        py::arg("ap_seed") = 0, py::arg("ap_minibatches") = 1,
        py::arg("ap_ctr_off") = 0, py::arg("ap_step_base") = py::none(),
        py::arg("ap_mb_ctr") = py::none());
  m.def("gae", &gae_op);
  m.def("adam", &adam_op, py::arg("p"), py::arg("g"), py::arg("m"),
        py::arg("v"), py::arg("p_bf16"), py::arg("lr"), py::arg("beta1"),
        py::arg("beta2"), py::arg("eps"), py::arg("step"),
        py::arg("gscale") = py::none(), py::arg("step_ctr") = py::none(),
        py::arg("clip_part") = py::none(), py::arg("clip_max_norm") = 0.0);
  m.def("grad_clip", &grad_clip_op);
  m.def("sample_head", &sample_head_op, py::arg("head"), py::arg("seed"),
        py::arg("step"), py::arg("actions"), py::arg("logp"),
        py::arg("value") = py::none(), py::arg("entropy") = py::none(),
        py::arg("greedy") = false, py::arg("step_base") = py::none(),
        py::arg("row_offset") = 0);
  m.def("increment_counter", &increment_counter_op, py::arg("ctr"),
        py::arg("delta"));
  m.def("mlp_policy_rollout", &mlp_policy_rollout_op, py::arg("obs"),
        py::arg("W1t"), py::arg("b1"), py::arg("W2t"), py::arg("b2"),
        py::arg("W3t"), py::arg("b3"), py::arg("actions"), py::arg("logp"),
        py::arg("value"), py::arg("seed"), py::arg("step"),
        py::arg("step_base") = py::none(), py::arg("row_offset") = 0,
        py::arg("greedy") = false);
  m.def("mb_gather", &mb_gather_op, py::arg("obs_src"), py::arg("act_src"),
        py::arg("logp_src"), py::arg("adv_src"), py::arg("ret_src"),
        py::arg("obs_mb"), py::arg("act_mb"), py::arg("logp_mb"),
        py::arg("adv_mb"), py::arg("ret_mb"), py::arg("seed"),
        py::arg("minibatches"), py::arg("step_base"), py::arg("mb_ctr"), py::arg("skip_obs") = false);
  m.def("ppo_loss_bwd", &ppo_loss_bwd_op, py::arg("head"), py::arg("actions"),
        py::arg("old_logp"), py::arg("adv"), py::arg("ret"), py::arg("dhead"),
        py::arg("clip_eps"), py::arg("ent_coef"), py::arg("vf_coef"),
        py::arg("inv_count"), py::arg("losses") = py::none());
  m.def("adv_normalize", &adv_normalize_op);
  m.def("f32_to_bf16", &f32_to_bf16_op);
  m.def("transpose_bf16", &transpose_bf16_op);
  py::class_<gymfx::GymFxEngine>(m, "GymFxEngine")
      .def(py::init<const py::dict&, const py::dict&, const py::dict&, const py::dict&>())
      .def("step", &gymfx::GymFxEngine::step, py::arg("actions"),
           py::arg("obs_out"), py::arg("reward_out") = py::none(),
           py::arg("terminated_out") = py::none(),
           py::arg("obs_bf16_out") = py::none(), py::arg("env_lo") = 0,
           py::arg("env_hi") = 0, py::arg("head") = py::none(),
           py::arg("logp_out") = py::none(), py::arg("value_out") = py::none(),
           py::arg("step_base") = py::none(), py::arg("sample_seed") = 0,
           py::arg("sample_step") = 0, py::arg("fuse_obs") = false,
           py::arg("h2") = py::none(), py::arg("w3t") = py::none(),
           py::arg("b3") = py::none(), py::arg("rnn_h") = py::none(),
           py::arg("rnn_c") = py::none())
      .def("build_obs", &gymfx::GymFxEngine::build_obs, py::arg("obs_out"),
           py::arg("obs_bf16_out") = py::none(), py::arg("env_lo") = 0,
           py::arg("env_hi") = 0);
  m.attr("EXEC_COUNTER_N") = (int)gymfx::EXEC_COUNTER_N;
  m.attr("ACT_COUNTER_N") = (int)gymfx::ACT_COUNTER_N;
}
```

### gymfx_amd/ops/csrc/env_common.h

```cpp
#pragma once

#include <hip/hip_runtime.h>
#include <cstdint>

#define GFX_DEV __device__ __forceinline__

namespace gymfx {

enum RewardId { REWARD_PNL = 0, REWARD_SHARPE = 1, REWARD_DD = 2 };
enum StrategyId { STRAT_DIRECT = 0, STRAT_FIXED = 1, STRAT_ATR = 2 };
enum PrepId { PREP_DEFAULT = 0, PREP_FEATURE_WINDOW = 1 };
enum ScalingMode { SCALE_NONE = 0, SCALE_ROLLING = 1, SCALE_EXPANDING = 2 };
enum SizeMode { SIZE_FX_UNITS = 0, SIZE_NOTIONAL = 1 };
enum RiskMode { RISK_FIXED = 0, RISK_RELVOL = 1, RISK_MARGIN = 2 };
enum CollisionPolicy { COLL_WORST = 0, COLL_OHLC = 1, COLL_ADAPTIVE = 2 };
enum LimitPolicy { LIM_TOUCH = 0, LIM_CROSS = 1, LIM_CONSERVATIVE = 2 };
enum MarginModel { MARGIN_LEVERAGED = 0, MARGIN_STANDARD = 1 };

enum Flags {
  F_CONTINUOUS = 1 << 0,
  F_INCLUDE_PRICE = 1 << 1,
  F_INCLUDE_AGENT = 1 << 2,
  F_STAGEB_OBS = 1 << 3,
  F_CALENDAR_OBS = 1 << 4,
  F_OVERLAY = 1 << 5,
  F_OVERLAY_BLOCK = 1 << 6,
  F_OVERLAY_FF = 1 << 7,
  F_SESSION_FILTER = 1 << 8,
  F_HAS_MINFRAC = 1 << 9,
  F_HAS_MAXFRAC = 1 << 10,
  F_HAS_RELVOL = 1 << 11,
  F_HAS_MPLF = 1 << 12,
  F_STAGEB_PENALTY = 1 << 13,
  F_AUTORESET = 1 << 14,
  F_FINANCING = 1 << 15,
  F_PREFLIGHT = 1 << 16,
};

enum ExecCounter {
  E_ENTRY_ACTIONS_SEEN = 0,
  E_ENTRY_ORDERS_SUBMITTED,
  E_BLOCKED_SESSION_FILTER,
  E_BLOCKED_ATR_WARMUP,
  E_BLOCKED_NON_POSITIVE_ATR,
  E_BLOCKED_NON_POSITIVE_SIZE,
  E_BLOCKED_NON_POSITIVE_PRICE,
  E_DEFAULT_ORDERS_SUBMITTED,
  E_PLUGIN_APPLY_ERRORS,
  E_EV_NO_TRADE_ACTIVE_STEPS,
  E_EV_ACTION_OVERRIDES,
  E_EV_BLOCKED_ENTRIES,
  E_EV_FORCED_FLAT_ACTIONS,
  E_EV_FORCED_FLAT_ORDERS,
  E_SESSION_FORCE_CLOSES,
  E_BRACKET_SL_FILLS,
  E_BRACKET_TP_FILLS,
  E_MARGIN_PREFLIGHT_DENIED,
  EXEC_COUNTER_N,
};

enum ActCounter {
  A_STEPS = 0,
  A_HOLD,
  A_LONG,
  A_SHORT,
  A_NON_HOLD,
  A_DEADBAND,
  ACT_COUNTER_N,
};

#ifdef __HIPCC__
GFX_DEV float fast_exp(float x) {
  return __builtin_amdgcn_exp2f(x * 1.4426950408889634f);
}
GFX_DEV float fast_log(float x) {
  return __builtin_amdgcn_logf(x) * 0.6931471805599453f;
}
GFX_DEV uint64_t splitmix64(uint64_t x) {
  x += 0x9E3779B97F4A7C15ull;
  x = (x ^ (x >> 30)) * 0xBF58476D1CE4E5B9ull;
  x = (x ^ (x >> 27)) * 0x94D049BB133111EBull;
  return x ^ (x >> 31);
}
GFX_DEV float head_logz(const float* row, int n_actions) {
  float mx = row[0];
  for (int j = 1; j < n_actions; ++j) mx = fmaxf(mx, row[j]);
  float z = 0.f;
  for (int j = 0; j < n_actions; ++j) z += fast_exp(row[j] - mx);
  return fast_log(z) + mx;
}
GFX_DEV int sample_categorical(const float* row, int n_actions, float logz,
                               uint64_t seed, uint64_t step, int64_t mg) {
  const uint64_t r =
      splitmix64(seed ^ (step * 0x51E1F5ull + (uint64_t)mg * 0x9E37ull));
  float u = (float)((r >> 11) * (1.0 / 9007199254740992.0));
  u = fminf(u, 0.999999f);
  float c = 0.f;
  int a = n_actions - 1;
  for (int j = 0; j < n_actions; ++j) {
    c += fast_exp(row[j] - logz);
    if (u < c) { a = j; break; }
  }
  return a;
}
#endif

struct FeistelMap {
  uint32_t n = 0;
  int half = 0;
  uint64_t seed = 0;
  int minibatches = 1;
  int M_mb = 0;
  long long ctr_off = 0;
  const unsigned long long* step_base = nullptr;
  const unsigned long long* mb_ctr = nullptr;
};

struct EnvParamsK {
  int n_envs, T, window, n_features;
  int reward_id, strategy_id, prep_id;
  int scaling_mode, scale_window, sharpe_window, atr_period;
  int size_mode, risk_mode;
  int collision_policy, limit_policy, latency_bars, margin_model;
  int flags;
  int obs_dim;
  int off_features, off_prices, off_returns, off_agent, off_fc, off_cal;

  double initial_cash, position_size, commission, slippage, leverage, min_equity;
  double cont_threshold, reward_scale, annualization, penalty_lambda;
  double sl_pips, tp_pips, pip_size;
  double k_sl, k_tp, rel_volume, min_order_volume, max_order_volume;
  double min_sltp_frac, max_sltp_frac;
  double baseline_rel_volume, max_risk_rel_volume;
  double sl_shrink_alpha, tp_shrink_alpha, min_k_sl, min_rr, mplf;
  double fc_pen_coef, fc_pen_window_hours;
  double feature_clip, overlay_threshold;
  double margin_init_rate;
  int head_hidden;
  int rnn_hidden;
  unsigned long long sample_seed;
  long long sample_step;
  int sample_nact;
};

struct EnvPtrs {
  const float *open_px, *high_px, *low_px, *close_px, *price_px;
  const float *features;
  const double *p1, *p2;
  const bool *binary_mask;
  const float *ev_no_trade;
  const float *force_close;
  const float *calendar;
  const bool *sess_entry, *sess_close;
  const float *roll_rate;
  int *cursor;
  bool *started, *terminated;
  double *pos, *avg_entry, *cash, *margin_used, *equity, *prev_equity, *peak_equity;
  double *commission_paid, *last_trade_cost;
  int *trade_count;
  bool *pend_close;
  int8_t *pend_open_dir;
  float *pend_open_size, *pend_sl, *pend_tp;
  int *pend_wait;
  bool *br_active, *br_armed;
  float *br_sl, *br_tp;
  float *tr_ring;
  int *tr_count;
  float *tr_sum;
  float *prev_close_atr;
  float *rew_ring;
  int *rew_count;
  double *rew_s1, *rew_s2;
  int *trade_won, *trade_lost;
  double *trade_pnl_sum, *trade_pnl_sumsq;
  double *metric_peak, *max_dd_money, *max_dd_pct, *ret_sum, *ret_sumsq;
  int *ret_count;
  int *episode_step;
  double *episode_return;
  int *start_offset;
  const int *lo_bar;
  const int *end_bar;
  const int *inst_id;
  const float *pip_env;
  int *exec_diag;
  int *act_diag;
  float *raw_abs_sum, *raw_min, *raw_max;
  const float *head;
  const void *h2;
  const void *w3t;
  const float *b3;
  void *rnn_h;
  float *rnn_c;
  int64_t *actions_out;
  float *logp_out;
  float *value_out;
  const unsigned long long *step_base;
  const void *actions;
  float *reward_out, *base_reward_out, *penalty_out;
  bool *terminated_out;
  int64_t *coerced_out;
  float *obs_out;
  void *obs_bf16_out;
};

}
```

### gymfx_amd/ops/csrc/ppo_kernels.hip

```cpp
#include "env_common.h"

#include <hip/hip_bf16.h>

#include <algorithm>

namespace gymfx {

typedef __attribute__((ext_vector_type(8))) __bf16 bf16x8;
typedef __attribute__((ext_vector_type(4))) float f32x4;

GFX_DEV float bf2f(__bf16 v) { return (float)v; }
GFX_DEV __bf16 f2bf(float v) { return (__bf16)v; }

GFX_DEV float fast_tanh(float x) {
  x = fminf(fmaxf(x, -15.f), 15.f);
  const float e = __builtin_amdgcn_exp2f(x * 2.885390081777927f);
  return 1.f - 2.f * __builtin_amdgcn_rcpf(e + 1.f);
}

GFX_DEV uint32_t feistel_encrypt_once(uint32_t x, int half, uint32_t mask,
                                      uint64_t key) {
  uint32_t a = x & mask;
  uint32_t b = x >> half;
  for (int r = 0; r < 4; ++r) {
// ... 523 lines not shown
  if (e >= elems) return;
  float s = 0.f;
  for (int k = threadIdx.x; k < slabs; k += 256)
    s += part[(int64_t)k * elems + e];
  red[threadIdx.x] = s;
  __syncthreads();
  for (int w = 128; w > 0; w >>= 1) {
    if (threadIdx.x < w) red[threadIdx.x] += red[threadIdx.x + w];
    __syncthreads();
  }
  if (threadIdx.x == 0) out[e] = red[0];
}

__global__ __launch_bounds__(256) void transpose_bf16_kernel(
    const __bf16* __restrict__ src, __bf16* __restrict__ dst, int K, int N) {
  __shared__ __bf16 tile[64][64 + 4];
  const int kb = blockIdx.x * 64;
  const int nb = blockIdx.y * 64;
  for (int e = threadIdx.x; e < 64 * 8; e += 256) {
    const int r = e >> 3;
    const int c8 = (e & 7) * 8;
    const int gk = kb + r;
    const int gn = nb + c8;
    bf16x8 v = {};
    if (gk < K) {
      if (gn + 8 <= N) {
        v = *reinterpret_cast<const bf16x8*>(&src[(int64_t)gk * N + gn]);
      } else {
        for (int i = 0; i < 8; ++i)
          v[i] = (gn + i < N) ? src[(int64_t)gk * N + gn + i] : (__bf16)0.f;
      }
    }
    *reinterpret_cast<bf16x8*>(&tile[r][c8]) = v;
  }
  __syncthreads();
  for (int e = threadIdx.x; e < 64 * 8; e += 256) {
    const int r = e >> 3;
    const int c8 = (e & 7) * 8;
    const int gn = nb + r;
    const int gk = kb + c8;
    if (gn >= N) continue;
    if (gk + 8 <= K) {
      bf16x8 v;
      for (int i = 0; i < 8; ++i) v[i] = tile[c8 + i][r];
      *reinterpret_cast<bf16x8*>(&dst[(int64_t)gn * K + gk]) = v;
    } else {
      for (int i = 0; i < 8 && gk + i < K; ++i)
        dst[(int64_t)gn * K + gk + i] = tile[c8 + i][r];
    }
  }
}

__global__ void f32_to_bf16_kernel(const float* __restrict__ in,
                                   __bf16* __restrict__ out, int64_t n) {
  for (int64_t i = (int64_t)blockIdx.x * blockDim.x + threadIdx.x; i < n;
       i += (int64_t)gridDim.x * blockDim.x)
    out[i] = f2bf(in[i]);
}

__global__ void gae_kernel(const float* __restrict__ rewards,
                           const float* __restrict__ values,
                           const bool* __restrict__ dones,
                           float* __restrict__ adv, float* __restrict__ ret,
                           int T, int N, float gamma, float lam) {
  const int n = blockIdx.x * blockDim.x + threadIdx.x;
  if (n >= N) return;
  float running = 0.f;
  for (int t = T - 1; t >= 0; --t) {
    const float nonterm = dones[(int64_t)t * N + n] ? 0.f : 1.f;
    const float delta = rewards[(int64_t)t * N + n] +
                        gamma * values[(int64_t)(t + 1) * N + n] * nonterm -
                        values[(int64_t)t * N + n];
    running = delta + gamma * lam * nonterm * running;
    adv[(int64_t)t * N + n] = running;
    ret[(int64_t)t * N + n] = running + values[(int64_t)t * N + n];
  }
}

__global__ void adam_kernel(float* __restrict__ p, const float* __restrict__ g,
                            float* __restrict__ m, float* __restrict__ v,
                            __bf16* __restrict__ p_bf16, int64_t n, float lr,
                            float beta1, float beta2, float eps, float bc1,
                            float bc2, const float* __restrict__ gscale,
                            const int* __restrict__ step_ctr,
                            const float* __restrict__ clip_part, int nparts,
                            float max_norm) {
  if (step_ctr) {
    const float st = (float)(*step_ctr + 1);
    bc1 = 1.f - powf(beta1, st);
    bc2 = 1.f - powf(beta2, st);
  }
  float s = 1.f;
  if (clip_part) {
    __shared__ float red[256];
    float acc = 0.f;
    for (int i = threadIdx.x; i < nparts; i += 256) acc += clip_part[i];
    red[threadIdx.x] = acc;
    __syncthreads();
    for (int w = 128; w > 0; w >>= 1) {
      if (threadIdx.x < w) red[threadIdx.x] += red[threadIdx.x + w];
      __syncthreads();
    }
    const float norm = sqrtf(red[0]);
    s = (max_norm > 0.f && norm > max_norm) ? max_norm / norm : 1.f;
  } else if (gscale) {
    s = *gscale;
  }
  for (int64_t i = (int64_t)blockIdx.x * blockDim.x + threadIdx.x; i < n;
       i += (int64_t)gridDim.x * blockDim.x) {
    const float gi = g[i] * s;
    const float mi = beta1 * m[i] + (1.f - beta1) * gi;
    const float vi = beta2 * v[i] + (1.f - beta2) * gi * gi;
    m[i] = mi;
    v[i] = vi;
    const float mhat = mi / bc1;
    const float vhat = vi / bc2;
    const float pi = p[i] - lr * mhat / (sqrtf(vhat) + eps);
    p[i] = pi;
    if (p_bf16) p_bf16[i] = f2bf(pi);
  }
}

__global__ void sumsq_partial_kernel(const float* __restrict__ g, int64_t n,
                                     float* __restrict__ part) {
  __shared__ float red[256];
  float s = 0.f;
  for (int64_t i = (int64_t)blockIdx.x * blockDim.x + threadIdx.x; i < n;
       i += (int64_t)gridDim.x * blockDim.x)
    s += g[i] * g[i];
  red[threadIdx.x] = s;
  __syncthreads();
  for (int w = 128; w > 0; w >>= 1) {
    if (threadIdx.x < w) red[threadIdx.x] += red[threadIdx.x + w];
    __syncthreads();
  }
  if (threadIdx.x == 0) part[blockIdx.x] = red[0];
}

__global__ void clip_scale_kernel(const float* __restrict__ part, int nparts,
                                  float max_norm, float* __restrict__ scale) {
  __shared__ float red[256];
  float s = 0.f;
  for (int i = threadIdx.x; i < nparts; i += 256) s += part[i];
  red[threadIdx.x] = s;
  __syncthreads();
  for (int w = 128; w > 0; w >>= 1) {
    if (threadIdx.x < w) red[threadIdx.x] += red[threadIdx.x + w];
    __syncthreads();
  }
  if (threadIdx.x == 0) {
    const float norm = sqrtf(red[0]);
    *scale = (max_norm > 0.f && norm > max_norm) ? max_norm / norm : 1.f;
  }
}

__global__ void sample_head_kernel(const float* __restrict__ head, int M,
                                   int n_actions, uint64_t seed, uint64_t step,
                                   int64_t* __restrict__ actions,
                                   float* __restrict__ logp,
                                   float* __restrict__ value,
                                   float* __restrict__ entropy,
                                   int greedy,
                                   const unsigned long long* __restrict__ step_base,
                                   int row_offset) {
  const int m = blockIdx.x * blockDim.x + threadIdx.x;
  if (m >= M) return;
  if (step_base) step += *step_base;
  const int64_t mg = m + row_offset;
  const float* row = head + (int64_t)m * (n_actions + 1);
  const float logz = head_logz(row, n_actions);

  int a = 0;
  if (greedy) {
    float best = row[0];
    for (int j = 1; j < n_actions; ++j)
      if (row[j] > best) { best = row[j]; a = j; }
  } else {
    a = sample_categorical(row, n_actions, logz, seed, step, mg);
  }
  actions[m] = a;
  logp[m] = row[a] - logz;
  if (value) value[m] = row[n_actions];
  if (entropy) {
    float h = 0.f;
    for (int j = 0; j < n_actions; ++j) {
      const float lp = row[j] - logz;
      h -= fast_exp(lp) * lp;
    }
    entropy[m] = h;
  }
}

__global__ void ppo_loss_bwd_kernel(
    const float* __restrict__ head, const int64_t* __restrict__ actions,
    const float* __restrict__ old_logp, const float* __restrict__ adv,
    const float* __restrict__ ret, __bf16* __restrict__ dhead, int M,
    int n_actions, float clip_eps, float ent_coef, float vf_coef,
    float inv_count, float* __restrict__ losses) {
  const int m = blockIdx.x * blockDim.x + threadIdx.x;
  float l_pi = 0.f, l_v = 0.f, l_ent = 0.f, l_kl = 0.f, l_clip = 0.f;
  if (m < M) {
    const float* row = head + (int64_t)m * (n_actions + 1);
    __bf16* drow = dhead + (int64_t)m * (n_actions + 1);
    float mx = row[0];
    for (int j = 1; j < n_actions; ++j) mx = fmaxf(mx, row[j]);
    float z = 0.f;
    for (int j = 0; j < n_actions; ++j) z += expf(row[j] - mx);
    const float logz = logf(z) + mx;
    const int a = (int)actions[m];
    const float lp = row[a] - logz;
    const float ratio = expf(lp - old_logp[m]);
    const float A = adv[m];
    const bool clipped = (ratio > 1.f + clip_eps) || (ratio < 1.f - clip_eps);
    const float surr1 = ratio * A;
    const float rclip = fminf(fmaxf(ratio, 1.f - clip_eps), 1.f + clip_eps);
    const float surr2 = rclip * A;
    const float g_lp = (surr1 <= surr2) ? (-A * ratio) : 0.f;
    float H = 0.f;
    for (int j = 0; j < n_actions; ++j) {
      const float lpj = row[j] - logz;
      H -= expf(lpj) * lpj;
    }
    for (int j = 0; j < n_actions; ++j) {
      const float pj = expf(row[j] - logz);
      const float onehot = (j == a) ? 1.f : 0.f;
      float d = g_lp * (onehot - pj);
      d += ent_coef * pj * ((row[j] - logz) + H);
      drow[j] = f2bf(d * inv_count);
    }
    const float v = row[n_actions];
    const float dv = vf_coef * (v - ret[m]);
    drow[n_actions] = f2bf(dv * inv_count);

    l_pi = -fminf(surr1, surr2);
    l_v = 0.5f * (v - ret[m]) * (v - ret[m]);
    l_ent = H;
    l_kl = old_logp[m] - lp;
    l_clip = clipped ? 1.f : 0.f;
  }
  __shared__ float red[256];
  float vals[5] = {l_pi, l_v, l_ent, l_kl, l_clip};
  for (int s = 0; s < 5; ++s) {
    red[threadIdx.x] = vals[s];
    __syncthreads();
    for (int w = 128; w > 0; w >>= 1) {
      if (threadIdx.x < w) red[threadIdx.x] += red[threadIdx.x + w];
      __syncthreads();
    }
    if (threadIdx.x == 0 && losses) atomicAdd(&losses[s], red[0] * inv_count);
    __syncthreads();
  }
}

__global__ void adv_norm_stats_kernel(const float* __restrict__ adv, int64_t n,
                                      float* __restrict__ part ) {
  __shared__ float red[512];
  float s = 0.f, ss = 0.f;
  for (int64_t i = (int64_t)blockIdx.x * blockDim.x + threadIdx.x; i < n;
       i += (int64_t)gridDim.x * blockDim.x) {
    s += adv[i];
    ss += adv[i] * adv[i];
  }
  red[threadIdx.x] = s;
  red[256 + threadIdx.x] = ss;
  __syncthreads();
  for (int w = 128; w > 0; w >>= 1) {
    if (threadIdx.x < w) {
      red[threadIdx.x] += red[threadIdx.x + w];
      red[256 + threadIdx.x] += red[256 + threadIdx.x + w];
    }
    __syncthreads();
  }
  if (threadIdx.x == 0) {
    part[blockIdx.x] = red[0];
    part[gridDim.x + blockIdx.x] = red[256];
  }
}

__global__ void adv_norm_apply_kernel(float* __restrict__ adv, int64_t n,
                                      const float* __restrict__ part,
                                      int nparts) {
  __shared__ float mean_s, inv_std_s;
  if (threadIdx.x == 0) {
    float s = 0.f, ss = 0.f;
    for (int i = 0; i < nparts; ++i) { s += part[i]; ss += part[nparts + i]; }
    const float mean = s / (float)n;
    float var = ss / (float)n - mean * mean;
    var = fmaxf(var, 0.f);
    mean_s = mean;
    inv_std_s = 1.f / (sqrtf(var) + 1e-8f);
  }
  __syncthreads();
  for (int64_t i = (int64_t)blockIdx.x * blockDim.x + threadIdx.x; i < n;
       i += (int64_t)gridDim.x * blockDim.x)
    adv[i] = (adv[i] - mean_s) * inv_std_s;
}

GFX_DEV float fast_sigmoid(float x) {
  x = fminf(fmaxf(x, -30.f), 30.f);
  return __builtin_amdgcn_rcpf(1.f + __builtin_amdgcn_exp2f(-x * 1.4426950408889634f));
}

typedef __attribute__((ext_vector_type(4))) __bf16 bf16x4;

GFX_DEV f32x4 gate_pre4(const __bf16* __restrict__ gates_pre,
                        const __bf16* __restrict__ gates_h, int64_t idx4) {
// ... 453 lines not shown
  const int wr = wave >> 1, wc = wave & 1;
  const int row_a = lane & 15;
  const int kseg = lane >> 4;
  const int a_r = tid >> 2, a_c8 = (tid & 3) * 8;
  const int b_r = tid >> 2, b_c8 = (tid & 3) * 8;
  const int crow_base = (lane >> 4) * 4;
  const int ccol = lane & 15;
  f32x4 acc[2][8];
  bf16x8 ra, rb[4];

  for (int layer = 0; layer < 2; ++layer) {
    const bool from_global = layer == 0;
    const __bf16* Wt = from_global ? W1t : W2t;
    const float* bias = from_global ? b1 : b2;
    const int K = from_global ? D : H;
    const __bf16(*Ximg)[LDH] = Himg[0];
    __bf16(*Yimg)[LDH] = Himg[layer];
    const int ktiles = (K + BK - 1) / BK;
    for (int mi = 0; mi < 2; ++mi)
      for (int ni = 0; ni < 8; ++ni) acc[mi][ni] = f32x4{};
    for (int kt = -1; kt + 1 < ktiles + 1; ++kt) {
      const int knext = (kt + 1) * BK;
      if (kt + 1 < ktiles) {
        if (from_global) {
          ra = bf16x8{};
          const int gr = bm + a_r;
          if (gr < N) {
            const int gk = knext + a_c8;
            if (gk + 8 <= K) {
              ra = *reinterpret_cast<const bf16x8*>(&obs[(int64_t)gr * D + gk]);
            } else {
              for (int i = 0; i < 8; ++i)
                ra[i] = (gk + i < K) ? obs[(int64_t)gr * D + gk + i]
                                     : (__bf16)0.f;
            }
          }
        } else {
          ra = *reinterpret_cast<const bf16x8*>(&Ximg[a_r][knext + a_c8]);
        }
        for (int j = 0; j < 4; ++j) {
          const int gn = b_r + j * 64;
          const int gk = knext + b_c8;
          if (gk + 8 <= K) {
            rb[j] = *reinterpret_cast<const bf16x8*>(&Wt[(int64_t)gn * K + gk]);
          } else {
            rb[j] = bf16x8{};
            for (int i = 0; i < 8; ++i)
              rb[j][i] = (gk + i < K) ? Wt[(int64_t)gn * K + gk + i]
                                      : (__bf16)0.f;
          }
        }
      }
      if (kt >= 0) {
        const int cur = kt & 1;
        bf16x8 af[2], bf[8];
        for (int mi = 0; mi < 2; ++mi)
          af[mi] = *reinterpret_cast<const bf16x8*>(
              &As[cur][wr * 32 + mi * 16 + row_a][kseg * 8]);
        for (int ni = 0; ni < 8; ++ni)
          bf[ni] = *reinterpret_cast<const bf16x8*>(
              &Bs[cur][wc * 128 + ni * 16 + row_a][kseg * 8]);
        for (int mi = 0; mi < 2; ++mi)
          for (int ni = 0; ni < 8; ++ni)
            acc[mi][ni] = __builtin_amdgcn_mfma_f32_16x16x32_bf16(
                af[mi], bf[ni], acc[mi][ni], 0, 0, 0);
      }
      if (kt + 1 < ktiles) {
        const int nxt = (kt + 1) & 1;
        *reinterpret_cast<bf16x8*>(&As[nxt][a_r][a_c8]) = ra;
        for (int j = 0; j < 4; ++j)
          *reinterpret_cast<bf16x8*>(&Bs[nxt][b_r + j * 64][b_c8]) = rb[j];
      }
      __syncthreads();
    }
    for (int mi = 0; mi < 2; ++mi)
      for (int ni = 0; ni < 8; ++ni) {
        const int lcol = wc * 128 + ni * 16 + ccol;
        for (int r = 0; r < 4; ++r) {
          const int lrow = wr * 32 + mi * 16 + crow_base + r;
          float v = acc[mi][ni][r] + bias[lcol];
          Yimg[lrow][lcol] = f2bf(fast_tanh(v));
        }
      }
    __syncthreads();
  }

  {
    f32x4 hacc = {};
    const int hrow = wave * 16 + row_a;
    for (int kt = 0; kt < H / BK; ++kt) {
      bf16x8 af, bf;
      af = *reinterpret_cast<const bf16x8*>(
          &Himg[1][hrow][kt * BK + kseg * 8]);
      for (int i = 0; i < 8; ++i) {
        const int k = kt * BK + kseg * 8 + i;
        bf[i] = (row_a <= n_actions) ? W3t[(int64_t)row_a * H + k] : (__bf16)0.f;
      }
      hacc = __builtin_amdgcn_mfma_f32_16x16x32_bf16(af, bf, hacc, 0, 0, 0);
    }
    for (int r = 0; r < 4; ++r) {
      const int lrow = wave * 16 + crow_base + r;
      if (ccol <= n_actions)
        Head[lrow][ccol] = hacc[r] + b3[ccol];
    }
  }
  __syncthreads();

  if (tid < BM) {
    const int gr = bm + tid;
    if (gr < N) {
      const float* row = Head[tid];
      float mx = row[0];
      for (int j = 1; j < n_actions; ++j) mx = fmaxf(mx, row[j]);
      float z = 0.f;
      for (int j = 0; j < n_actions; ++j) z += fast_exp(row[j] - mx);
      const float logz = fast_log(z) + mx;
      uint64_t st = step;
      if (step_base) st += *step_base;
      int a = 0;
      if (greedy) {
        float best = row[0];
        for (int j = 1; j < n_actions; ++j)
          if (row[j] > best) { best = row[j]; a = j; }
      } else {
        const int64_t mg = gr + row_offset;
        const uint64_t r =
            splitmix64(seed ^ (st * 0x51E1F5ull + (uint64_t)mg * 0x9E37ull));
        float u = (float)((r >> 11) * (1.0 / 9007199254740992.0));
        u = fminf(u, 0.999999f);
        float c = 0.f;
        a = n_actions - 1;
        for (int j = 0; j < n_actions; ++j) {
          c += fast_exp(row[j] - logz);
          if (u < c) { a = j; break; }
        }
      }
      actions[gr] = a;
      logp[gr] = row[a] - logz;
      if (value) value[gr] = row[n_actions];
    }
  }
}

__global__ void increment_u64_kernel(unsigned long long* __restrict__ ctr,
                                     unsigned long long delta) {
  if (threadIdx.x == 0 && blockIdx.x == 0) *ctr += delta;
}

__global__ void increment_i32_kernel(int* __restrict__ ctr, int delta) {
  if (threadIdx.x == 0 && blockIdx.x == 0) *ctr += delta;
}


__global__ __launch_bounds__(256) void mb_gather_kernel(
    const __bf16* __restrict__ obs_src, const int64_t* __restrict__ act_src,
    const float* __restrict__ logp_src, const float* __restrict__ adv_src,
    const float* __restrict__ ret_src, __bf16* __restrict__ obs_mb,
    int64_t* __restrict__ act_mb, float* __restrict__ logp_mb,
    float* __restrict__ adv_mb, float* __restrict__ ret_mb, int M, int D,
    uint32_t n, int half, uint64_t seed, int minibatches,
    const unsigned long long* __restrict__ step_base,
    const unsigned long long* __restrict__ mb_ctr, int skip_obs) {
  const int row = blockIdx.x * 4 + (threadIdx.x >> 6);
  const int lane = threadIdx.x & 63;
  if (row >= M) return;
  const unsigned long long ctr = *mb_ctr;
  const uint32_t epoch = (uint32_t)(ctr / (unsigned)minibatches);
  const uint32_t mb = (uint32_t)(ctr % (unsigned)minibatches);
  const uint64_t key = splitmix64(seed ^ (*step_base * 0x9E3779B97F4A7C15ull) ^
                                  ((uint64_t)epoch << 32));
  const uint32_t dst = mb * (uint32_t)M + (uint32_t)row;
  const uint32_t src = feistel_perm_idx(dst, n, half, key);

  const __bf16* src_row = obs_src + (int64_t)src * D;
  __bf16* dst_row = obs_mb + (int64_t)row * D;
  if (skip_obs) {
  } else if ((D & 3) == 0) {
    const int chunks = D >> 2;
    const uint64_t* s64 = reinterpret_cast<const uint64_t*>(src_row);
    uint64_t* d64 = reinterpret_cast<uint64_t*>(dst_row);
    for (int c = lane; c < chunks; c += 64) d64[c] = s64[c];
  } else {
    for (int c = lane; c < D; c += 64) dst_row[c] = src_row[c];
  }
  if (lane == 0) {
    act_mb[row] = act_src[src];
    logp_mb[row] = logp_src[src];
    adv_mb[row] = adv_src[src];
    ret_mb[row] = ret_src[src];
  }
}

__global__ __launch_bounds__(256) void mb_gather_seq_kernel(
    const __bf16* __restrict__ obs_src,
    const int64_t* __restrict__ act_src,
    const float* __restrict__ logp_src, const float* __restrict__ adv_src,
    const float* __restrict__ ret_src,
    const bool* __restrict__ done_src,
    const float* __restrict__ h0_src,
    const float* __restrict__ c0_src,
    __bf16* __restrict__ obs_mb,
    int64_t* __restrict__ act_mb,
    float* __restrict__ logp_mb, float* __restrict__ adv_mb,
    float* __restrict__ ret_mb,
    bool* __restrict__ done_mb,
    __bf16* __restrict__ h0_mb,
    float* __restrict__ c0_mb,
    int Mseq, int L, int D, int H, int N, uint32_t n_seq, int half,
    uint64_t seed, int minibatches,
    const unsigned long long* __restrict__ step_base,
    const unsigned long long* __restrict__ mb_ctr) {
  const int row = blockIdx.x * 4 + (threadIdx.x >> 6);
  const int lane = threadIdx.x & 63;
  if (row >= Mseq) return;
  const unsigned long long ctr = *mb_ctr;
  const uint32_t epoch = (uint32_t)(ctr / (unsigned)minibatches);
  const uint32_t mb = (uint32_t)(ctr % (unsigned)minibatches);
  const uint64_t key = splitmix64(seed ^ (*step_base * 0x9E3779B97F4A7C15ull) ^
                                  ((uint64_t)epoch << 32));
  const uint32_t dst = mb * (uint32_t)Mseq + (uint32_t)row;
  const uint32_t src = feistel_perm_idx(dst, n_seq, half, key);
  const int chunk = (int)(src / (uint32_t)N);
  const int env = (int)(src % (uint32_t)N);
  {
    const float* hs = h0_src + ((int64_t)chunk * N + env) * H;
    const float* cs = c0_src + ((int64_t)chunk * N + env) * H;
    __bf16* hd = h0_mb + (int64_t)row * H;
    float* cd = c0_mb + (int64_t)row * H;
    for (int j = lane; j < H; j += 64) {
      hd[j] = f2bf(hs[j]);
      cd[j] = cs[j];
    }
  }
  for (int l = 0; l < L; ++l) {
    const int64_t t = (int64_t)chunk * L + l;
    const __bf16* srow = obs_src + (t * N + env) * D;
    __bf16* drow = obs_mb + ((int64_t)l * Mseq + row) * D;
    if ((D & 3) == 0) {
      const int chunks8 = D >> 2;
      const uint64_t* s64 = reinterpret_cast<const uint64_t*>(srow);
      uint64_t* d64 = reinterpret_cast<uint64_t*>(drow);
      for (int c = lane; c < chunks8; c += 64) d64[c] = s64[c];
    } else {
      for (int c = lane; c < D; c += 64) drow[c] = srow[c];
    }
    if (lane == 0) {
      const int64_t si = t * N + env;
      const int64_t di = (int64_t)l * Mseq + row;
      act_mb[di] = act_src[si];
      logp_mb[di] = logp_src[si];
      adv_mb[di] = adv_src[si];
      ret_mb[di] = ret_src[si];
      done_mb[di] = done_src[si];
    }
  }
}

static inline int ceil_div(int a, int b) { return (a + b - 1) / b; }

void launch_lstm_cell_fwd(const void* gates_pre, const void* gates_h,
                          const float* c_prev, float* c_new, void* h_new,
                          const bool* done, void* h_masked, float* c_masked,
                          void* acts_out, int64_t M, int H,
                          hipStream_t stream) {
  int64_t total = M * H;
  int blocks = (int)std::min<int64_t>((total + 255) / 256, 2048);
  hipLaunchKernelGGL(lstm_cell_fwd_kernel, dim3(blocks), dim3(256), 0, stream,
                     reinterpret_cast<const __bf16*>(gates_pre),
                     reinterpret_cast<const __bf16*>(gates_h),
                     c_prev, c_new, reinterpret_cast<__bf16*>(h_new), done,
                     reinterpret_cast<__bf16*>(h_masked), c_masked,
                     reinterpret_cast<__bf16*>(acts_out), M, H);
}

void launch_lstm_cell_bwd(const void* acts, const float* c_prev,
                          const float* c_new, const void* dh_head,
                          const float* dh_next, const float* dc_next,
                          const bool* done, void* dgates, float* dc_prev,
                          int64_t M, int H, hipStream_t stream) {
  int64_t total = M * (H / 4);
  int blocks = (int)std::min<int64_t>((total + 255) / 256, 2048);
  hipLaunchKernelGGL(lstm_cell_bwd_kernel, dim3(blocks), dim3(256), 0, stream,
                     reinterpret_cast<const __bf16*>(acts),
                     c_prev, c_new, reinterpret_cast<const __bf16*>(dh_head),
                     dh_next, dc_next, done,
                     reinterpret_cast<__bf16*>(dgates), dc_prev, M, H);
}

bool launch_lstm_gemm_cell_fwd(const void* A, const void* B,
                               const void* gates_pre, void* acts_out,
                               const float* c_prev, float* c_new, void* h_new,
                               const bool* done, void* h_masked,
                               float* c_masked, int M, int N, int K,
                               hipStream_t stream) {
  if (N % 64 != 0) return false;
  dim3 grid(ceil_div(M, 64), N / 64);
  if (acts_out) {
    hipLaunchKernelGGL((lstm_gemm_cell_fwd_kernel<true>), grid, dim3(256), 0,
                       stream, reinterpret_cast<const __bf16*>(A),
                       reinterpret_cast<const __bf16*>(B),
                       reinterpret_cast<const __bf16*>(gates_pre),
                       reinterpret_cast<__bf16*>(acts_out), c_prev, c_new,
                       reinterpret_cast<__bf16*>(h_new), done,
                       reinterpret_cast<__bf16*>(h_masked), c_masked, M, N, K);
  } else {
    hipLaunchKernelGGL((lstm_gemm_cell_fwd_kernel<false>), grid, dim3(256), 0,
                       stream, reinterpret_cast<const __bf16*>(A),
                       reinterpret_cast<const __bf16*>(B),
                       reinterpret_cast<const __bf16*>(gates_pre), nullptr,
                       c_prev, c_new, reinterpret_cast<__bf16*>(h_new), done,
                       reinterpret_cast<__bf16*>(h_masked), c_masked, M, N, K);
  }
  return true;
}

bool launch_lstm_bwd_fused(const void* acts, const float* c_prev,
                           const float* c_new, const void* dh_head,
                           const float* dh_next, const float* dc_next,
                           const bool* done, const void* B, void* dgates,
                           float* dc_prev, float* dh_prev, int M, int H,
                           hipStream_t stream) {
  if (H % 64 != 0) return false;
  dim3 grid(ceil_div(M, 64), dh_prev ? H / 64 : 1);
  hipLaunchKernelGGL(lstm_bwd_fused_kernel, grid, dim3(256), 0, stream,
                     reinterpret_cast<const __bf16*>(acts), c_prev, c_new,
                     reinterpret_cast<const __bf16*>(dh_head), dh_next,
                     dc_next, done,
                     reinterpret_cast<const __bf16*>(B),
                     reinterpret_cast<__bf16*>(dgates), dc_prev, dh_prev, M,
                     H);
  return true;
}

void launch_mask_reset(void* h, float* c, const bool* done, int64_t M, int H,
                       hipStream_t stream) {
  int64_t total = M * H;
  int blocks = (int)std::min<int64_t>((total + 255) / 256, 2048);
  hipLaunchKernelGGL(mask_reset_kernel, dim3(blocks), dim3(256), 0, stream,
                     reinterpret_cast<__bf16*>(h), c, done, M, H);
}

void launch_masked_state(const void* h_raw, const float* c_raw,
                         const bool* done, void* h_in, float* c_in, int64_t M,
                         int H, hipStream_t stream) {
  int64_t total = M * H;
  int blocks = (int)std::min<int64_t>((total + 255) / 256, 2048);
  hipLaunchKernelGGL(masked_state_kernel, dim3(blocks), dim3(256), 0, stream,
                     reinterpret_cast<const __bf16*>(h_raw), c_raw, done,
                     reinterpret_cast<__bf16*>(h_in), c_in, M, H);
}

void launch_mb_gather_seq(const void* obs_src, const int64_t* act_src,
                          const float* logp_src, const float* adv_src,
                          const float* ret_src, const bool* done_src,
                          const float* h0_src,
                          const float* c0_src, void* obs_mb, int64_t* act_mb,
                          float* logp_mb, float* adv_mb, float* ret_mb,
                          bool* done_mb,
                          void* h0_mb, float* c0_mb, int Mseq, int L, int D,
                          int H, int N, uint32_t n_seq, int half,
                          uint64_t seed, int minibatches,
                          const unsigned long long* step_base,
                          const unsigned long long* mb_ctr,
                          hipStream_t stream) {
  hipLaunchKernelGGL(mb_gather_seq_kernel, dim3(ceil_div(Mseq, 4)), dim3(256),
                     0, stream, reinterpret_cast<const __bf16*>(obs_src),
                     act_src, logp_src, adv_src, ret_src, done_src, h0_src,
                     c0_src, reinterpret_cast<__bf16*>(obs_mb), act_mb,
                     logp_mb, adv_mb, ret_mb, done_mb,
                     reinterpret_cast<__bf16*>(h0_mb), c0_mb,
                     Mseq, L, D, H, N, n_seq, half, seed, minibatches,
                     step_base, mb_ctr);
}

void launch_mlp_policy_rollout(const void* obs, const void* W1t,
                               const float* b1, const void* W2t,
                               const float* b2, const void* W3t,
                               const float* b3, int64_t* actions, float* logp,
                               float* value, int N, int D, int n_actions,
                               uint64_t seed, uint64_t step,
                               const unsigned long long* step_base,
                               int row_offset, int greedy,
                               hipStream_t stream) {
  hipLaunchKernelGGL(mlp_policy_rollout_kernel, dim3(ceil_div(N, 64)),
                     dim3(256), 0, stream,
                     reinterpret_cast<const __bf16*>(obs),
                     reinterpret_cast<const __bf16*>(W1t), b1,
                     reinterpret_cast<const __bf16*>(W2t), b2,
                     reinterpret_cast<const __bf16*>(W3t), b3, actions, logp,
                     value, N, D, n_actions, seed, step, step_base, row_offset,
                     greedy);
}

void launch_increment_u64(unsigned long long* ctr, unsigned long long delta,
                          hipStream_t stream) {
  hipLaunchKernelGGL(increment_u64_kernel, dim3(1), dim3(1), 0, stream, ctr,
                     delta);
}

void launch_increment_i32(int* ctr, int delta, hipStream_t stream) {
  hipLaunchKernelGGL(increment_i32_kernel, dim3(1), dim3(1), 0, stream, ctr,
                     delta);
}

void launch_mb_gather(const void* obs_src, const int64_t* act_src,
                      const float* logp_src, const float* adv_src,
                      const float* ret_src, void* obs_mb, int64_t* act_mb,
                      float* logp_mb, float* adv_mb, float* ret_mb, int M,
                      int D, uint32_t n, int half, uint64_t seed,
                      int minibatches, const unsigned long long* step_base,
                      const unsigned long long* mb_ctr, hipStream_t stream,
                      int skip_obs) {
  hipLaunchKernelGGL(mb_gather_kernel, dim3(ceil_div(M, 4)), dim3(256), 0,
                     stream, reinterpret_cast<const __bf16*>(obs_src), act_src,
                     logp_src, adv_src, ret_src,
                     reinterpret_cast<__bf16*>(obs_mb), act_mb, logp_mb, adv_mb,
                     ret_mb, M, D, n, half, seed, minibatches, step_base,
                     mb_ctr, skip_obs);
}

void launch_gemm(const void* A, const void* B, const float* bias, void* C,
                 const void* Yact, int M, int N, int K, bool trans_b, int act,
                 bool dact_tanh, bool add_bias, bool accum,
                 hipStream_t stream, const FeistelMap* fmp = nullptr) {
  const __bf16* a = reinterpret_cast<const __bf16*>(A);
  const __bf16* b = reinterpret_cast<const __bf16*>(B);
  const __bf16* y = reinterpret_cast<const __bf16*>(Yact);
  static const int wide_env = [] {
    const char* e = getenv("GYMFX_GEMM_WIDE");
    return e ? atoi(e) : -1;
  }();
  static const int bk64_env = [] {
    const char* e = getenv("GYMFX_GEMM_BK64");
    return e ? atoi(e) : -1;
  }();
  const bool mid = (N >= 96) &&
                   (wide_env == 4 ||
                    (wide_env == -1 && N >= 1024 && M >= 16384));
  const bool wide = (N >= 192) && !mid && wide_env == 1;
  const bool bk64 = trans_b && !wide && !mid &&
                    (bk64_env == 1 || (bk64_env != 0 && K >= 512));
  dim3 grid(ceil_div(M, 64), ceil_div(N, wide ? 256 : (mid ? 128 : 64)));
  dim3 block(256);
  static const int n1_env = [] {
    const char* e = getenv("GYMFX_GEMM_N1");
    return e ? atoi(e) : -1;
  }();
  if (bk64 && act == 0 && !dact_tanh && !add_bias && !accum && !fmp &&
      N <= 256 &&
      (n1_env == 1 || (n1_env == -1 && (int64_t)M * N <= 64 * 64 * 256))) {
    dim3 grid_n1(ceil_div(M, 64), ceil_div(N, 32));
    hipLaunchKernelGGL((gemm_kernel<true, 0, false, false, 1, false, 64>),
                       grid_n1, block, 0, stream, a, b, bias, C, y, M, N, K);
    return;
  }
  if (fmp) {
    if (!(trans_b && act == 2 && !dact_tanh && add_bias && !accum)) {
      abort();
    }
    hipLaunchKernelGGL((gemm_kernel<true, 2, false, true, 2, false, 32, true>),
                       grid, block, 0, stream, a, b, bias, C, y, M, N, K,
                       *fmp);
    return;
  }

#define GEMM_LAUNCH(TB, ACT, DT, AB)                                          \
  do {                                                                        \
    if (wide)                                                                 \
      hipLaunchKernelGGL((gemm_kernel<TB, ACT, DT, AB, 8>), grid, block, 0,   \
                         stream, a, b, bias, C, y, M, N, K);                  \
    else if (mid)                                                             \
      hipLaunchKernelGGL((gemm_kernel<TB, ACT, DT, AB, 4>), grid, block, 0,   \
                         stream, a, b, bias, C, y, M, N, K);                  \
    else if (bk64)                                                            \
      hipLaunchKernelGGL((gemm_kernel<TB, ACT, DT, AB, 2, false, 64>), grid,  \
                         block, 0, stream, a, b, bias, C, y, M, N, K);        \
    else                                                                      \
      hipLaunchKernelGGL((gemm_kernel<TB, ACT, DT, AB, 2>), grid, block, 0,   \
                         stream, a, b, bias, C, y, M, N, K);                  \
  } while (0)
  if (accum) {
    if (trans_b)
      if (wide) hipLaunchKernelGGL((gemm_kernel<true, 0, false, false, 8, true>), grid, block, 0, stream, a, b, bias, C, y, M, N, K);
      else if (mid) hipLaunchKernelGGL((gemm_kernel<true, 0, false, false, 4, true>), grid, block, 0, stream, a, b, bias, C, y, M, N, K);
      else hipLaunchKernelGGL((gemm_kernel<true, 0, false, false, 2, true>), grid, block, 0, stream, a, b, bias, C, y, M, N, K);
    else
      if (wide) hipLaunchKernelGGL((gemm_kernel<false, 0, false, false, 8, true>), grid, block, 0, stream, a, b, bias, C, y, M, N, K);
      else if (mid) hipLaunchKernelGGL((gemm_kernel<false, 0, false, false, 4, true>), grid, block, 0, stream, a, b, bias, C, y, M, N, K);
      else hipLaunchKernelGGL((gemm_kernel<false, 0, false, false, 2, true>), grid, block, 0, stream, a, b, bias, C, y, M, N, K);
    return;
  }
  if (!trans_b && !dact_tanh) {
    if (act == 0) { if (add_bias) GEMM_LAUNCH(false, 0, false, true); else GEMM_LAUNCH(false, 0, false, false); }
    else if (act == 1) { if (add_bias) GEMM_LAUNCH(false, 1, false, true); else GEMM_LAUNCH(false, 1, false, false); }
    else { if (add_bias) GEMM_LAUNCH(false, 2, false, true); else GEMM_LAUNCH(false, 2, false, false); }
  } else if (trans_b && !dact_tanh) {
    if (act == 0) { if (add_bias) GEMM_LAUNCH(true, 0, false, true); else GEMM_LAUNCH(true, 0, false, false); }
    else if (act == 1) { if (add_bias) GEMM_LAUNCH(true, 1, false, true); else GEMM_LAUNCH(true, 1, false, false); }
    else { if (add_bias) GEMM_LAUNCH(true, 2, false, true); else GEMM_LAUNCH(true, 2, false, false); }
  } else if (trans_b && dact_tanh) {
    GEMM_LAUNCH(true, 1, true, false);
  } else {
    GEMM_LAUNCH(false, 1, true, false);
  }
#undef GEMM_LAUNCH
}

void launch_wgrad(const void* X, const void* dY, float* dW_part, float* db_part,
                  float* dW, float* db, int M, int N, int K, int slabs,
                  hipStream_t stream, const FeistelMap* fmp = nullptr) {
  const __bf16* x = reinterpret_cast<const __bf16*>(X);
  const __bf16* dy = reinterpret_cast<const __bf16*>(dY);
  static const int big_env = [] {
    const char* e = getenv("GYMFX_WGRAD_BIG");
    return e ? atoi(e) : -1;
  }();
  const bool big = K >= 128 && N >= 128 &&
                   (big_env >= 0
                        ? big_env != 0
                        : (int64_t)ceil_div(K, 128) * ceil_div(N, 128) * slabs >=
                              384);
  const int m_per_slab = (M + slabs - 1) / slabs;
  const int TW = big ? 128 : 64;
  const bool glds_ok = N % TW == 0 && K >= TW && m_per_slab % 64 == 0 &&
                       M % slabs == 0;
  (void)0;
  if (glds_ok) {
#define WG_GLDS(WDB, FK, FN, GRID)                                            \
  do {                                                                        \
    if (fmp)                                                                  \
      hipLaunchKernelGGL((wgrad_glds_kernel<WDB, FK, FN, true>), GRID,        \
                         dim3(256), 0, stream, x, dy, dW_part, db_part, M, N, \
                         K, slabs, *fmp);                                     \
    else                                                                      \
      hipLaunchKernelGGL((wgrad_glds_kernel<WDB, FK, FN>), GRID, dim3(256),   \
                         0, stream, x, dy, dW_part, db_part, M, N, K, slabs); \
  } while (0)
    if (big) {
      const int t44 = ceil_div(K, 128), t54 = ceil_div(K, 160);
      if (t54 < t44 && N <= 512) {
        dim3 g0(t54, N / TW, slabs);
        if (db_part) WG_GLDS(true, 5, 4, g0);
        else WG_GLDS(false, 5, 4, g0);
      } else {
        dim3 g0(t44, N / TW, slabs);
        if (db_part) WG_GLDS(true, 4, 4, g0);
        else WG_GLDS(false, 4, 4, g0);
      }
    } else {
      dim3 g0(ceil_div(K, 64), N / TW, slabs);
      if (db_part) WG_GLDS(true, 2, 2, g0);
      else WG_GLDS(false, 2, 2, g0);
    }
#undef WG_GLDS
  } else {
    dim3 grid(ceil_div(K, big ? 128 : 64), ceil_div(N, big ? 128 : 64), slabs);
#define WG_PART(WDB, FK, FN)                                                  \
  do {                                                                        \
    if (fmp)                                                                  \
      hipLaunchKernelGGL((wgrad_partial_kernel<WDB, FK, FN, true>), grid,     \
                         dim3(256), 0, stream, x, dy, dW_part, db_part, M, N, \
                         K, slabs, 0, *fmp);                                  \
    else                                                                      \
      hipLaunchKernelGGL((wgrad_partial_kernel<WDB, FK, FN>), grid,           \
                         dim3(256), 0, stream, x, dy, dW_part, db_part, M, N, \
                         K, slabs, 0);                                        \
  } while (0)
    if (db_part) {
      if (big) WG_PART(true, 4, 4);
      else WG_PART(true, 2, 2);
    } else {
      if (big) WG_PART(false, 4, 4);
      else WG_PART(false, 2, 2);
    }
#undef WG_PART
  }
  int64_t elems = (int64_t)K * N;
  if (elems <= 4096) {
    hipLaunchKernelGGL(slab_reduce_small_kernel, dim3((int)elems), dim3(256),
                       0, stream, dW_part, dW, elems, slabs);
  } else {
    int blocks = (int)std::min<int64_t>((elems + 1023) / 1024, 1024);
    hipLaunchKernelGGL(slab_reduce_kernel, dim3(blocks), dim3(256), 0, stream,
                       dW_part, dW, elems, slabs);
  }
  if (db_part && db)
    hipLaunchKernelGGL(slab_reduce_small_kernel, dim3(N), dim3(256), 0, stream,
                       db_part, db, (int64_t)N, slabs);
}

void launch_gae(const float* rewards, const float* values, const bool* dones,
                float* adv, float* ret, int T, int N, float gamma, float lam,
                hipStream_t stream) {
  hipLaunchKernelGGL(gae_kernel, dim3(ceil_div(N, 256)), dim3(256), 0, stream,
                     rewards, values, dones, adv, ret, T, N, gamma, lam);
}

void launch_adam(float* p, const float* g, float* m, float* v, void* p_bf16,
                 int64_t n, float lr, float beta1, float beta2, float eps,
                 float bc1, float bc2, const float* gscale, const int* step_ctr,
                 hipStream_t stream) {
  int blocks = (int)std::min<int64_t>((n + 255) / 256, 2048);
  hipLaunchKernelGGL(adam_kernel, dim3(blocks), dim3(256), 0, stream, p, g, m,
                     v, reinterpret_cast<__bf16*>(p_bf16), n, lr, beta1, beta2,
                     eps, bc1, bc2, gscale, step_ctr, nullptr, 0, 0.f);
}

void launch_adam_clip(float* p, const float* g, float* m, float* v,
                      void* p_bf16, int64_t n, float lr, float beta1,
                      float beta2, float eps, float bc1, float bc2,
                      const int* step_ctr, const float* clip_part, int nparts,
                      float max_norm, hipStream_t stream) {
  int blocks = (int)std::min<int64_t>((n + 255) / 256, 2048);
  hipLaunchKernelGGL(adam_kernel, dim3(blocks), dim3(256), 0, stream, p, g, m,
                     v, reinterpret_cast<__bf16*>(p_bf16), n, lr, beta1, beta2,
                     eps, bc1, bc2, nullptr, step_ctr, clip_part, nparts,
                     max_norm);
}

void launch_grad_clip(const float* g, int64_t n, float max_norm, float* part,
                      float* scale, int nparts, hipStream_t stream) {
  hipLaunchKernelGGL(sumsq_partial_kernel, dim3(nparts), dim3(256), 0, stream,
                     g, n, part);
  hipLaunchKernelGGL(clip_scale_kernel, dim3(1), dim3(256), 0, stream, part,
                     nparts, max_norm, scale);
}

void launch_grad_sumsq(const float* g, int64_t n, float* part, int nparts,
                       hipStream_t stream) {
  hipLaunchKernelGGL(sumsq_partial_kernel, dim3(nparts), dim3(256), 0, stream,
                     g, n, part);
}

void launch_sample_head(const float* head, int M, int n_actions, uint64_t seed,
                        uint64_t step, int64_t* actions, float* logp,
                        float* value, float* entropy, int greedy,
                        const unsigned long long* step_base, int row_offset,
                        hipStream_t stream) {
  hipLaunchKernelGGL(sample_head_kernel, dim3(ceil_div(M, 256)), dim3(256), 0,
                     stream, head, M, n_actions, seed, step, actions, logp,
                     value, entropy, greedy, step_base, row_offset);
}

void launch_ppo_loss_bwd(const float* head, const int64_t* actions,
                         const float* old_logp, const float* adv,
                         const float* ret, void* dhead, int M, int n_actions,
                         float clip_eps, float ent_coef, float vf_coef,
                         float inv_count, float* losses, hipStream_t stream) {
  hipLaunchKernelGGL(ppo_loss_bwd_kernel, dim3(ceil_div(M, 256)), dim3(256), 0,
                     stream, head, actions, old_logp, adv, ret,
                     reinterpret_cast<__bf16*>(dhead), M, n_actions, clip_eps,
                     ent_coef, vf_coef, inv_count, losses);
}

void launch_adv_normalize(float* adv, int64_t n, float* part, int nparts,
                          hipStream_t stream) {
  hipLaunchKernelGGL(adv_norm_stats_kernel, dim3(nparts), dim3(256), 0, stream,
                     adv, n, part);
  int blocks = (int)std::min<int64_t>((n + 255) / 256, 2048);
  hipLaunchKernelGGL(adv_norm_apply_kernel, dim3(blocks), dim3(256), 0, stream,
                     adv, n, part, nparts);
}

void launch_transpose_bf16(const void* src, void* dst, int K, int N,
                           hipStream_t stream) {
  dim3 grid(ceil_div(K, 64), ceil_div(N, 64));
  hipLaunchKernelGGL(transpose_bf16_kernel, grid, dim3(256), 0, stream,
                     reinterpret_cast<const __bf16*>(src),
                     reinterpret_cast<__bf16*>(dst), K, N);
}

void launch_f32_to_bf16(const float* in, void* out, int64_t n,
                        hipStream_t stream) {
  int blocks = (int)std::min<int64_t>((n + 255) / 256, 2048);
  hipLaunchKernelGGL(f32_to_bf16_kernel, dim3(blocks), dim3(256), 0, stream, in,
                     reinterpret_cast<__bf16*>(out), n);
}

}
```

Measured before the change: 28.31 million env-steps/sec.

## Fuse gradient slab reduction, norm, Adam and weight transpose into tail kernels

Skips the per-layer slab_reduce launches and instead reduces all wgrad slab partials in one grads_finalize kernel, which can also compute the grad-norm sum of squares. A single adam_tail kernel then applies clipping, the Adam update, the bf16 copy and the transposed weight mirrors, and advances the step counter through a ticket. An optional ticket mechanism lets the gather kernel increment the minibatch counter itself. The aim is fewer small kernel launches and fewer passes over the gradients in each optimizer step. The cost is more complex cross-block ticket synchronisation and changed ordering of counter updates.

```diff
diff --git a/gymfx_amd/algo/ppo.py b/gymfx_amd/algo/ppo.py
--- a/gymfx_amd/algo/ppo.py
+++ b/gymfx_amd/algo/ppo.py
@@ -36,6 +36,7 @@
     fuse_sample: bool = True
     fuse_head: bool = False
     overlap_gather: bool = False
+    fused_opt_tail: bool = True
 
     @classmethod
     def from_config(cls, cfg: Dict[str, Any]) -> "PPOConfig":
@@ -62,6 +63,7 @@
             "fuse_sample": "fuse_sample",
             "fuse_head": "fuse_head",
             "overlap_gather": "overlap_gather",
+            "fused_opt_tail": "fused_opt_tail",
         }
         from ..config.merger import convert_type
 
@@ -199,6 +201,17 @@
         self._fm = {"seed": self.shuffle_seed, "minibatches": cfg.minibatches,
                     "ctr_off": -1, "step_base": self.step_base,
                     "mb_ctr": self.mb_ctr}
+
+        self._fused_tail = bool(cfg.fused_opt_tail) and (
+            not self.recurrent
+            or _os.environ.get("GYMFX_LSTM_OPT_TAIL", "0") == "1")
+        self.model.fused_tail = self._fused_tail
+        self.model.fuse_norm = (self._fused_tail and world_size <= 1
+                                and cfg.max_grad_norm > 0)
+        self._mb_ticket = (
+            torch.zeros((), dtype=torch.int32, device=dev)
+            if self._fused_tail
+            and _os.environ.get("GYMFX_GATHER_TICKET", "0") == "1" else None)
 
         self.global_step = 0
         self.update_count = 0
@@ -333,7 +346,7 @@
                 self.ret_mb, self.done_mb, self.h0_mb, self.c0_mb,
                 L=cfg.bptt_len, seed=self.shuffle_seed,
                 minibatches=cfg.minibatches, step_base=self.step_base,
-                mb_ctr=self.mb_ctr,
+                mb_ctr=self.mb_ctr, ticket=self._mb_ticket,
             )
         else:
             api.mb_gather(
@@ -342,9 +355,10 @@
                 self.logp_mb_s[slot], self.adv_mb_s[slot], self.ret_mb_s[slot],
                 seed=self.shuffle_seed, minibatches=cfg.minibatches,
                 step_base=self.step_base, mb_ctr=self.mb_ctr,
-                skip_obs=self._fuse_gather,
+                skip_obs=self._fuse_gather, ticket=self._mb_ticket,
             )
-        api.increment_counter(self.mb_ctr, 1)
+        if self._mb_ticket is None:
+            api.increment_counter(self.mb_ctr, 1)
 
     def _fwd_bwd_body(self, slot: int = 0) -> None:
         cfg, model = self.cfg, self.model
diff --git a/gymfx_amd/config/defaults.py b/gymfx_amd/config/defaults.py
--- a/gymfx_amd/config/defaults.py
+++ b/gymfx_amd/config/defaults.py
@@ -72,6 +72,7 @@
     "use_graphs": True,
     "fuse_sample": True,
     "overlap_gather": False,
+    "fused_opt_tail": True,
     "checkpoint_file": None,
     "checkpoint_interval": 0,
     "resume": False,
diff --git a/gymfx_amd/models/lstm.py b/gymfx_amd/models/lstm.py
--- a/gymfx_amd/models/lstm.py
+++ b/gymfx_amd/models/lstm.py
@@ -78,6 +78,10 @@
         self._clip_scale = torch.ones(1, dtype=torch.float32, device=device)
         self._wg_ws: Dict[str, Tuple[torch.Tensor, Optional[torch.Tensor], int]] = {}
         self.wgrad_slabs = 64
+        self.fused_tail = False
+        self.fuse_norm = False
+        self._adam_ticket = torch.zeros((), dtype=torch.int32, device=device)
+        self._fin_segs = None
 
     def w(self, name: str) -> torch.Tensor:
         s = self.slices[name]
@@ -108,6 +112,18 @@
         while tiles * s < 2048:
             s *= 2
         return s
+
+    def _finalize_segments(self):
+        if self._fin_segs is None:
+            segs = []
+            for (wn, bn) in (("Wy", "by"), ("Wx", "b"), ("Wh", None)):
+                K, N = self.slices[wn].shape
+                dw, db, S = self._wg_ws[f"{wn}:{K}x{N}"]
+                segs.append((dw, K * N, S, self.slices[wn].sl.start, False))
+                if bn is not None:
+                    segs.append((db, N, S, self.slices[bn].sl.start, True))
+            self._fin_segs = segs
+        return self._fin_segs
 
     def _wg_workspace(self, name: str, K: int, N: int, want_db: bool):
         key = f"{name}:{K}x{N}"
@@ -200,9 +216,10 @@
         L, M, D = obs_seq.shape
         H = self.hidden
         h_raw_flat = buf["h_raw"].view(L * M, H)
+        red = not self.fused_tail
         dw_p, db_p, slabs = self._wg_workspace("Wy", H, self.head_dim, True)
         api.wgrad(h_raw_flat, dhead, self.grad("Wy"), self.grad("by"),
-                  workspace=(dw_p, db_p), slabs=slabs)
+                  workspace=(dw_p, db_p), slabs=slabs, reduce=red)
         dh_flat = buf["dh_all"].view(L * M, H)
         api.gemm(dhead, self.w("Wy"), None, dh_flat, act=1, trans_b=True)
         dc_next: Optional[torch.Tensor] = None
@@ -222,10 +239,15 @@
         dgates_flat = buf["dgates"].view(L * M, 4 * H)
         dw_p, db_p, slabs = self._wg_workspace("Wx", D, 4 * H, True)
         api.wgrad(obs_seq.view(L * M, D), dgates_flat, self.grad("Wx"),
-                  self.grad("b"), workspace=(dw_p, db_p), slabs=slabs)
+                  self.grad("b"), workspace=(dw_p, db_p), slabs=slabs,
+                  reduce=red)
         dw_p, db_p, slabs = self._wg_workspace("Wh", H, 4 * H, False)
         api.wgrad(buf["h_in"][:L].reshape(L * M, H), dgates_flat,
-                  self.grad("Wh"), None, workspace=(dw_p, db_p), slabs=slabs)
+                  self.grad("Wh"), None, workspace=(dw_p, db_p), slabs=slabs,
+                  reduce=red)
+        if self.fused_tail:
+            api.grads_finalize(self._finalize_segments(), self.grads,
+                               self._clip_part if self.fuse_norm else None)
 
     def adam(self, lr: float, *, beta1=0.9, beta2=0.999, eps=1e-8,
              max_grad_norm: float = 0.0) -> None:
@@ -233,6 +255,15 @@
         clip = None
         if max_grad_norm and max_grad_norm > 0:
             clip = (self._clip_part, max_grad_norm)
+        if self.fused_tail:
+            api.adam_tail(self.params, self.grads, self.m, self.v,
+                          self.params_bf16, lr=lr, beta1=beta1, beta2=beta2,
+                          eps=eps, step_ctr=self.adam_ctr,
+                          ticket=self._adam_ticket, clip=clip,
+                          sumsq_done=self.fuse_norm,
+                          mirrors=[(self.slices[n].sl.start, t)
+                                   for n, t in self._wt.items()])
+            return
         api.adam(self.params, self.grads, self.m, self.v, self.params_bf16,
                  lr=lr, beta1=beta1, beta2=beta2, eps=eps, step=self.adam_step,
                  step_ctr=self.adam_ctr, clip=clip)
diff --git a/gymfx_amd/models/mlp.py b/gymfx_amd/models/mlp.py
--- a/gymfx_amd/models/mlp.py
+++ b/gymfx_amd/models/mlp.py
@@ -76,6 +76,10 @@
         self._clip_scale = torch.ones(1, dtype=torch.float32, device=device)
         self._wg_ws: Dict[str, Tuple[torch.Tensor, Optional[torch.Tensor]]] = {}
         self.wgrad_slabs = 64
+        self.fused_tail = False
+        self.fuse_norm = False
+        self._adam_ticket = torch.zeros((), dtype=torch.int32, device=device)
+        self._fin_segs = None
 
     def w(self, name: str) -> torch.Tensor:
         s = self.slices[name]
@@ -106,6 +110,17 @@
         while tiles * s < 2048:
             s *= 2
         return s
+
+    def _finalize_segments(self):
+        if self._fin_segs is None:
+            segs = []
+            for (wn, bn) in (("W3", "b3"), ("W2", "b2"), ("W1", "b1")):
+                K, N = self.slices[wn].shape
+                dw, db, S = self._wg_ws[f"{wn}:{K}x{N}"]
+                segs.append((dw, K * N, S, self.slices[wn].sl.start, False))
+                segs.append((db, N, S, self.slices[bn].sl.start, True))
+            self._fin_segs = segs
+        return self._fin_segs
 
     def _wg_workspace(self, name: str, K: int, N: int, want_db: bool):
         key = f"{name}:{K}x{N}"
@@ -159,19 +174,24 @@
         M = dhead.shape[0]
         dh2 = scratch["dh2"]
         dh1 = scratch["dh1"]
+        red = not self.fused_tail
         dw_p, db_p, slabs = self._wg_workspace("W3", self.hidden, self.head_dim, True)
         api.wgrad(acts["h2"], dhead, self.grad("W3"), self.grad("b3"),
-                  workspace=(dw_p, db_p), slabs=slabs)
+                  workspace=(dw_p, db_p), slabs=slabs, reduce=red)
         api.gemm(dhead, self.w("W3"), None, dh2, Yact=acts["h2"], trans_b=True,
                  act=1, dact_tanh=True)
         dw_p, db_p, slabs = self._wg_workspace("W2", self.hidden, self.hidden, True)
         api.wgrad(acts["h1"], dh2, self.grad("W2"), self.grad("b2"),
-                  workspace=(dw_p, db_p), slabs=slabs)
+                  workspace=(dw_p, db_p), slabs=slabs, reduce=red)
         api.gemm(dh2, self.w("W2"), None, dh1, Yact=acts["h1"], trans_b=True,
                  act=1, dact_tanh=True)
         dw_p, db_p, slabs = self._wg_workspace("W1", self.obs_dim, self.hidden, True)
         api.wgrad(obs_bf16, dh1, self.grad("W1"), self.grad("b1"),
-                  workspace=(dw_p, db_p), slabs=slabs, x_perm=a_feistel)
+                  workspace=(dw_p, db_p), slabs=slabs, x_perm=a_feistel,
+                  reduce=red)
+        if self.fused_tail:
+            api.grads_finalize(self._finalize_segments(), self.grads,
+                               self._clip_part if self.fuse_norm else None)
 
     def alloc_scratch(self, M: int) -> Dict[str, torch.Tensor]:
         dev = self.device
@@ -186,6 +206,15 @@
         clip = None
         if max_grad_norm and max_grad_norm > 0:
             clip = (self._clip_part, max_grad_norm)
+        if self.fused_tail:
+            api.adam_tail(self.params, self.grads, self.m, self.v,
+                          self.params_bf16, lr=lr, beta1=beta1, beta2=beta2,
+                          eps=eps, step_ctr=self.adam_ctr,
+                          ticket=self._adam_ticket, clip=clip,
+                          sumsq_done=self.fuse_norm,
+                          mirrors=[(self.slices[n].sl.start, t)
+                                   for n, t in self._wt.items()])
+            return
         api.adam(self.params, self.grads, self.m, self.v, self.params_bf16,
                  lr=lr, beta1=beta1, beta2=beta2, eps=eps, step=self.adam_step,
                  step_ctr=self.adam_ctr, clip=clip)
diff --git a/gymfx_amd/ops/api.py b/gymfx_amd/ops/api.py
--- a/gymfx_amd/ops/api.py
+++ b/gymfx_amd/ops/api.py
@@ -1,6 +1,6 @@
 from __future__ import annotations
 
-from typing import Optional, Tuple
+from typing import Optional, Sequence, Tuple
 
 import os
 
@@ -229,6 +229,7 @@
     workspace: Optional[Tuple[torch.Tensor, Optional[torch.Tensor]]] = None,
     slabs: int = 64,
     x_perm: "Optional[dict]" = None,
+    reduce: bool = True,
 ) -> None:
     if _use_native(X):
         K, N = dW.shape
@@ -247,9 +248,10 @@
                                    ap_minibatches=x_perm["minibatches"],
                                    ap_ctr_off=x_perm.get("ctr_off", 0),
                                    ap_step_base=x_perm["step_base"],
-                                   ap_mb_ctr=x_perm["mb_ctr"])
+                                   ap_mb_ctr=x_perm["mb_ctr"], reduce=reduce)
             return
-        native.require().wgrad(X, dY, dW_part, db_part, dW, db, slabs)
+        native.require().wgrad(X, dY, dW_part, db_part, dW, db, slabs,
+                               reduce=reduce)
         return
     if x_perm is not None:
         X = X[_perm_rows(X.shape[0], dY.shape[0], x_perm)]
@@ -258,6 +260,19 @@
     dW.copy_(x.t() @ dy)
     if db is not None:
         db.copy_(dy.sum(dim=0))
+
+
+def grads_finalize(
+    segments: "Sequence[Tuple[torch.Tensor, int, int, int, bool]]",
+    grads: torch.Tensor,
+    clip_part: Optional[torch.Tensor] = None,
+) -> None:
+    if _use_native(grads):
+        native.require().grads_finalize(
+            [s[0] for s in segments], [int(s[1]) for s in segments],
+            [int(s[2]) for s in segments], [int(s[3]) for s in segments],
+            [bool(s[4]) for s in segments], grads, clip_part)
+        return
 
 
 def gae(
@@ -323,6 +338,40 @@
     p.addcdiv_(mhat, vhat.sqrt() + eps, value=-lr)
     if p_bf16 is not None:
         p_bf16.copy_(p.to(torch.bfloat16))
+
+
+def adam_tail(
+    p: torch.Tensor,
+    g: torch.Tensor,
+    m: torch.Tensor,
+    v: torch.Tensor,
+    p_bf16: Optional[torch.Tensor],
+    *,
+    lr: float,
+    beta1: float = 0.9,
+    beta2: float = 0.999,
+    eps: float = 1e-8,
+    step_ctr: torch.Tensor,
+    ticket: Optional[torch.Tensor] = None,
+    clip: "Optional[Tuple[torch.Tensor, float]]" = None,
+    sumsq_done: bool = False,
+    mirrors: "Sequence[Tuple[int, torch.Tensor]]" = (),
+) -> None:
+    if _use_native(p):
+        part, max_norm = clip if clip is not None else (None, 0.0)
+        native.require().adam_tail(
+            p, g, m, v, p_bf16, lr, beta1, beta2, eps, step_ctr, ticket, part,
+            float(max_norm), sumsq_done, [int(o) for o, _ in mirrors],
+            [t for _, t in mirrors])
+        return
+    adam(p, g, m, v, p_bf16, lr=lr, beta1=beta1, beta2=beta2, eps=eps,
+         step_ctr=step_ctr, clip=clip)
+    if ticket is not None:
+        increment_counter(step_ctr, 1)
+    for off, t in mirrors:
+        N, K = t.shape
+        src = (p_bf16 if p_bf16 is not None else p.to(torch.bfloat16))
+        transpose_bf16(src[off:off + K * N].view(K, N), t)
 
 
 def grad_clip_scale(
@@ -528,12 +577,13 @@
     step_base: torch.Tensor,
     mb_ctr: torch.Tensor,
     skip_obs: bool = False,
+    ticket: Optional[torch.Tensor] = None,
 ) -> None:
     if _use_native(obs_src):
         native.require().mb_gather(
             obs_src, act_src, logp_src, adv_src, ret_src, obs_mb, act_mb,
             logp_mb, adv_mb, ret_mb, seed, minibatches, step_base, mb_ctr,
-            skip_obs,
+            skip_obs, ticket,
         )
         return
     n = obs_src.shape[0]
@@ -548,6 +598,8 @@
     logp_mb.copy_(logp_src[src])
     adv_mb.copy_(adv_src[src])
     ret_mb.copy_(ret_src[src])
+    if ticket is not None:
+        mb_ctr.add_(1)
 
 
 def mb_gather_seq(
@@ -573,6 +625,7 @@
     minibatches: int,
     step_base: torch.Tensor,
     mb_ctr: torch.Tensor,
+    ticket: Optional[torch.Tensor] = None,
 ) -> None:
     n_chunks, N, H = h0_src.shape
     if _use_native(obs_src):
@@ -583,7 +636,7 @@
             h0_src, c0_src, obs_mb.view(-1, obs_mb.shape[-1]),
             act_mb.view(-1), logp_mb.view(-1), adv_mb.view(-1),
             ret_mb.view(-1), done_mb.view(-1), h0_mb, c0_mb, L, N, seed,
-            minibatches, step_base, mb_ctr,
+            minibatches, step_base, mb_ctr, ticket,
         )
         return
     Mseq = c0_mb.shape[0]
@@ -604,6 +657,8 @@
         adv_mb[li].copy_(adv_src[t, env])
         ret_mb[li].copy_(ret_src[t, env])
         done_mb[li].copy_(done_src[t, env])
+    if ticket is not None:
+        mb_ctr.add_(1)
 
 
 def increment_counter(ctr: torch.Tensor, delta: int) -> None:
diff --git a/gymfx_amd/ops/csrc/bindings.cpp b/gymfx_amd/ops/csrc/bindings.cpp
--- a/gymfx_amd/ops/csrc/bindings.cpp
+++ b/gymfx_amd/ops/csrc/bindings.cpp
@@ -59,11 +59,20 @@
                           int H, int N, uint32_t n_seq, int half,
                           uint64_t seed, int minibatches,
                           const unsigned long long* step_base,
-                          const unsigned long long* mb_ctr,
+                          unsigned long long* mb_ctr, unsigned int* ticket,
                           hipStream_t stream);
 void launch_wgrad(const void* X, const void* dY, float* dW_part, float* db_part,
                   float* dW, float* db, int M, int N, int K, int slabs,
-                  hipStream_t stream, const FeistelMap* fmp = nullptr);
+                  hipStream_t stream, const FeistelMap* fmp = nullptr,
+                  bool reduce = true);
+void launch_grads_finalize(const FinalizeTable& tab, float* grads, int64_t n,
+                           float* clip_part, hipStream_t stream);
+void launch_adam_tail(float* p, const float* g, float* m, float* v,
+                      void* p_bf16, int64_t n, float lr, float beta1,
+                      float beta2, float eps, int* step_ctr,
+                      unsigned int* ticket, const float* clip_part, int nparts,
+                      float max_norm, const MirrorTable& mt,
+                      hipStream_t stream);
 void launch_gae(const float* rewards, const float* values, const bool* dones,
                 float* adv, float* ret, int T, int N, float gamma, float lam,
                 hipStream_t stream);
@@ -102,8 +111,8 @@
                       float* logp_mb, float* adv_mb, float* ret_mb, int M,
                       int D, uint32_t n, int half, uint64_t seed,
                       int minibatches, const unsigned long long* step_base,
-                      const unsigned long long* mb_ctr, hipStream_t stream,
-                      int skip_obs = 0);
+                      unsigned long long* mb_ctr, hipStream_t stream,
+                      int skip_obs = 0, unsigned int* ticket = nullptr);
 void launch_ppo_loss_bwd(const float* head, const int64_t* actions,
                          const float* old_logp, const float* adv,
                          const float* ret, void* dhead, int M, int n_actions,
@@ -492,6 +501,13 @@
               name, " must be contiguous f32");
 }
 
+unsigned int* ticket_ptr(const c10::optional<torch::Tensor>& ticket) {
+  if (!ticket.has_value()) return nullptr;
+  TORCH_CHECK(ticket->scalar_type() == torch::kInt32 && ticket->numel() == 1,
+              "ticket must be a scalar int32 tensor");
+  return reinterpret_cast<unsigned int*>(ticket->data_ptr());
+}
+
 static gymfx::FeistelMap make_fmap(int64_t n_rows, int M_mb, int64_t seed,
                                    int64_t minibatches, int64_t ctr_off,
                                    torch::Tensor step_base,
@@ -730,7 +746,8 @@
                       torch::Tensor done_mb,
                       torch::Tensor h0_mb, torch::Tensor c0_mb, int64_t L,
                       int64_t N, int64_t seed, int64_t minibatches,
-                      torch::Tensor step_base, torch::Tensor mb_ctr) {
+                      torch::Tensor step_base, torch::Tensor mb_ctr,
+                      c10::optional<torch::Tensor> ticket) {
   check_bf16(obs_src, "obs_src");
   check_bf16(obs_mb, "obs_mb");
   check_bf16(h0_mb, "h0_mb");
@@ -758,8 +775,8 @@
       c0_mb.data_ptr<float>(), Mseq, (int)L, D, H, (int)N, (uint32_t)n_seq,
       bits / 2, (uint64_t)seed, (int)minibatches,
       reinterpret_cast<const unsigned long long*>(step_base.data_ptr()),
-      reinterpret_cast<const unsigned long long*>(mb_ctr.data_ptr()),
-      cur_stream());
+      reinterpret_cast<unsigned long long*>(mb_ctr.data_ptr()),
+      ticket_ptr(ticket), cur_stream());
 }
 
 
@@ -769,7 +786,7 @@
               c10::optional<torch::Tensor> db, int64_t slabs,
               int64_t ap_seed, int64_t ap_minibatches, int64_t ap_ctr_off,
               c10::optional<torch::Tensor> ap_step_base,
-              c10::optional<torch::Tensor> ap_mb_ctr) {
+              c10::optional<torch::Tensor> ap_mb_ctr, bool reduce) {
   check_bf16(X, "X");
   check_bf16(dY, "dY");
   check_f32(dW, "dW");
@@ -794,12 +811,53 @@
                                      ap_ctr_off, *ap_step_base, *ap_mb_ctr);
     gymfx::launch_wgrad(X.data_ptr(), dY.data_ptr(),
                         dW_part.data_ptr<float>(), dbp, dW.data_ptr<float>(),
-                        dbo, M, N, K, (int)slabs, cur_stream(), &fm);
+                        dbo, M, N, K, (int)slabs, cur_stream(), &fm, reduce);
     return;
   }
   gymfx::launch_wgrad(X.data_ptr(), dY.data_ptr(), dW_part.data_ptr<float>(),
                       dbp, dW.data_ptr<float>(), dbo, M, N, K, (int)slabs,
-                      cur_stream());
+                      cur_stream(), nullptr, reduce);
+}
+
+void grads_finalize_op(std::vector<torch::Tensor> parts,
+                       std::vector<int64_t> elems, std::vector<int64_t> slabs,
+                       std::vector<int64_t> offs, std::vector<bool> is_bias,
+                       torch::Tensor grads,
+                       c10::optional<torch::Tensor> clip_part) {
+  check_f32(grads, "grads");
+  const size_t ns = parts.size();
+  TORCH_CHECK(ns <= (size_t)gymfx::kMaxFinalizeSegs, "too many segments");
+  TORCH_CHECK(elems.size() == ns && slabs.size() == ns && offs.size() == ns &&
+                  is_bias.size() == ns,
+              "segment lists differ in length");
+  const int64_t n = grads.numel();
+  gymfx::FinalizeTable tab;
+  tab.nseg = (int)ns;
+  for (size_t s = 0; s < ns; ++s) {
+    check_f32(parts[s], "parts");
+    TORCH_CHECK(parts[s].device() == grads.device(), "parts device");
+    TORCH_CHECK(elems[s] > 0 && slabs[s] > 0 && slabs[s] < (1 << 30),
+                "bad segment size");
+    TORCH_CHECK(parts[s].numel() >= slabs[s] * elems[s], "parts too small");
+    TORCH_CHECK(offs[s] >= 0 && offs[s] + elems[s] <= n,
+                "segment outside grads");
+    for (size_t r = 0; r < s; ++r)
+      TORCH_CHECK(offs[s] >= offs[r] + elems[r] || offs[r] >= offs[s] + elems[s],
+                  "segments overlap");
+    tab.seg[s].part = parts[s].data_ptr<float>();
+    tab.seg[s].elems = elems[s];
+    tab.seg[s].off = offs[s];
+    tab.seg[s].slabs = (int)slabs[s];
+    tab.seg[s].small = (is_bias[s] || elems[s] <= 4096) ? 1 : 0;
+  }
+  float* cp = nullptr;
+  if (clip_part.has_value()) {
+    check_f32(*clip_part, "clip_part");
+    TORCH_CHECK(clip_part->numel() == 256, "clip_part must hold 256 partials");
+    cp = clip_part->data_ptr<float>();
+  }
+  gymfx::launch_grads_finalize(tab, grads.data_ptr<float>(), n, cp,
+                               cur_stream());
 }
 
 void gae_op(torch::Tensor rewards, torch::Tensor values, torch::Tensor dones,
@@ -860,6 +918,63 @@
                      m.data_ptr<float>(), v.data_ptr<float>(), pb, n, (float)lr,
                      (float)beta1, (float)beta2, (float)eps, bc1, bc2, gs, sc,
                      cur_stream());
+}
+
+void adam_tail_op(torch::Tensor p, torch::Tensor g, torch::Tensor m,
+                  torch::Tensor v, c10::optional<torch::Tensor> p_bf16,
+                  double lr, double beta1, double beta2, double eps,
+                  torch::Tensor step_ctr, c10::optional<torch::Tensor> ticket,
+                  c10::optional<torch::Tensor> clip_part, double clip_max_norm,
+                  bool sumsq_done, std::vector<int64_t> mirror_offs,
+                  std::vector<torch::Tensor> mirrors) {
+  check_f32(p, "p");
+  check_f32(g, "g");
+  check_f32(m, "m");
+  check_f32(v, "v");
+  const int64_t n = p.numel();
+  TORCH_CHECK(g.numel() == n && m.numel() == n && v.numel() == n);
+  void* pb = nullptr;
+  if (p_bf16.has_value()) {
+    check_bf16(*p_bf16, "p_bf16");
+    TORCH_CHECK(p_bf16->numel() == n, "p_bf16 numel");
+    pb = p_bf16->data_ptr();
+  }
+  TORCH_CHECK(step_ctr.scalar_type() == torch::kInt32 && step_ctr.numel() == 1,
+              "step_ctr int32 scalar");
+  const size_t ns = mirrors.size();
+  TORCH_CHECK(ns <= (size_t)gymfx::kMaxMirrorSegs && mirror_offs.size() == ns,
+              "bad mirror table");
+  gymfx::MirrorTable mt;
+  mt.nseg = (int)ns;
+  for (size_t s = 0; s < ns; ++s) {
+    check_bf16(mirrors[s], "mirror");
+    TORCH_CHECK(mirrors[s].dim() == 2 && mirrors[s].device() == p.device(),
+                "mirror must be [N,K] on the parameter device");
+    const int64_t N = mirrors[s].size(0), K = mirrors[s].size(1);
+    TORCH_CHECK(K * N > 0 && K * N < (1ll << 31), "mirror size");
+    TORCH_CHECK(mirror_offs[s] >= 0 && mirror_offs[s] + K * N <= n,
+                "mirror segment outside params");
+    mt.seg[s].off = mirror_offs[s];
+    mt.seg[s].K = (int)K;
+    mt.seg[s].N = (int)N;
+    mt.seg[s].dst = mirrors[s].data_ptr();
+  }
+  const float* part = nullptr;
+  int nparts = 0;
+  if (clip_part.has_value() && clip_max_norm > 0) {
+    check_f32(*clip_part, "clip_part");
+    nparts = (int)clip_part->numel();
+    if (!sumsq_done)
+      gymfx::launch_grad_sumsq(g.data_ptr<float>(), n,
+                               clip_part->data_ptr<float>(), nparts,
+                               cur_stream());
+    part = clip_part->data_ptr<float>();
+  }
+  gymfx::launch_adam_tail(p.data_ptr<float>(), g.data_ptr<float>(),
+                          m.data_ptr<float>(), v.data_ptr<float>(), pb, n,
+                          (float)lr, (float)beta1, (float)beta2, (float)eps,
+                          step_ctr.data_ptr<int>(), ticket_ptr(ticket), part,
+                          nparts, (float)clip_max_norm, mt, cur_stream());
 }
 
 void grad_clip_op(torch::Tensor g, double max_norm, torch::Tensor part,
@@ -948,7 +1063,8 @@
                   torch::Tensor act_mb, torch::Tensor logp_mb,
                   torch::Tensor adv_mb, torch::Tensor ret_mb, int64_t seed,
                   int64_t minibatches, torch::Tensor step_base,
-                  torch::Tensor mb_ctr, bool skip_obs) {
+                  torch::Tensor mb_ctr, bool skip_obs,
+                  c10::optional<torch::Tensor> ticket) {
   check_bf16(obs_src, "obs_src");
   check_bf16(obs_mb, "obs_mb");
   const int64_t n = obs_src.size(0);
@@ -972,8 +1088,8 @@
       adv_mb.data_ptr<float>(), ret_mb.data_ptr<float>(), M, D, (uint32_t)n,
       bits / 2, (uint64_t)seed, (int)minibatches,
       reinterpret_cast<const unsigned long long*>(step_base.data_ptr()),
-      reinterpret_cast<const unsigned long long*>(mb_ctr.data_ptr()),
-      cur_stream(), skip_obs ? 1 : 0);
+      reinterpret_cast<unsigned long long*>(mb_ctr.data_ptr()),
+      cur_stream(), skip_obs ? 1 : 0, ticket_ptr(ticket));
 }
 
 void ppo_loss_bwd_op(torch::Tensor head, torch::Tensor actions,
@@ -1065,18 +1181,30 @@
         py::arg("adv_mb"), py::arg("ret_mb"), py::arg("done_mb"),
         py::arg("h0_mb"),
         py::arg("c0_mb"), py::arg("L"), py::arg("N"), py::arg("seed"),
-        py::arg("minibatches"), py::arg("step_base"), py::arg("mb_ctr"));
+        py::arg("minibatches"), py::arg("step_base"), py::arg("mb_ctr"),
+        py::arg("ticket") = py::none());
   m.def("wgrad", &wgrad_op, py::arg("X"), py::arg("dY"), py::arg("dW_part"),
         py::arg("db_part"), py::arg("dW"), py::arg("db"), py::arg("slabs"),
         py::arg("ap_seed") = 0, py::arg("ap_minibatches") = 1,
         py::arg("ap_ctr_off") = 0, py::arg("ap_step_base") = py::none(),
-        py::arg("ap_mb_ctr") = py::none());
+        py::arg("ap_mb_ctr") = py::none(), py::arg("reduce") = true);
+  m.def("grads_finalize", &grads_finalize_op, py::arg("parts"),
+        py::arg("elems"), py::arg("slabs"), py::arg("offs"),
+        py::arg("is_bias"), py::arg("grads"),
+        py::arg("clip_part") = py::none());
   m.def("gae", &gae_op);
   m.def("adam", &adam_op, py::arg("p"), py::arg("g"), py::arg("m"),
         py::arg("v"), py::arg("p_bf16"), py::arg("lr"), py::arg("beta1"),
         py::arg("beta2"), py::arg("eps"), py::arg("step"),
         py::arg("gscale") = py::none(), py::arg("step_ctr") = py::none(),
         py::arg("clip_part") = py::none(), py::arg("clip_max_norm") = 0.0);
+  m.def("adam_tail", &adam_tail_op, py::arg("p"), py::arg("g"), py::arg("m"),
+        py::arg("v"), py::arg("p_bf16"), py::arg("lr"), py::arg("beta1"),
+        py::arg("beta2"), py::arg("eps"), py::arg("step_ctr"),
+        py::arg("ticket") = py::none(), py::arg("clip_part") = py::none(),
+        py::arg("clip_max_norm") = 0.0, py::arg("sumsq_done") = false,
+        py::arg("mirror_offs") = std::vector<int64_t>(),
+        py::arg("mirrors") = std::vector<torch::Tensor>());
   m.def("grad_clip", &grad_clip_op);
   m.def("sample_head", &sample_head_op, py::arg("head"), py::arg("seed"),
         py::arg("step"), py::arg("actions"), py::arg("logp"),
@@ -1095,7 +1223,8 @@
         py::arg("logp_src"), py::arg("adv_src"), py::arg("ret_src"),
         py::arg("obs_mb"), py::arg("act_mb"), py::arg("logp_mb"),
         py::arg("adv_mb"), py::arg("ret_mb"), py::arg("seed"),
-        py::arg("minibatches"), py::arg("step_base"), py::arg("mb_ctr"), py::arg("skip_obs") = false);
+        py::arg("minibatches"), py::arg("step_base"), py::arg("mb_ctr"),
+        py::arg("skip_obs") = false, py::arg("ticket") = py::none());
   m.def("ppo_loss_bwd", &ppo_loss_bwd_op, py::arg("head"), py::arg("actions"),
         py::arg("old_logp"), py::arg("adv"), py::arg("ret"), py::arg("dhead"),
         py::arg("clip_eps"), py::arg("ent_coef"), py::arg("vf_coef"),
diff --git a/gymfx_amd/ops/csrc/env_common.h b/gymfx_amd/ops/csrc/env_common.h
--- a/gymfx_amd/ops/csrc/env_common.h
+++ b/gymfx_amd/ops/csrc/env_common.h
@@ -114,6 +114,30 @@
   long long ctr_off = 0;
   const unsigned long long* step_base = nullptr;
   const unsigned long long* mb_ctr = nullptr;
+};
+
+constexpr int kMaxFinalizeSegs = 12;
+struct FinalizeSeg {
+  const float* part = nullptr;
+  long long elems = 0;
+  long long off = 0;
+  int slabs = 0;
+  int small = 0;
+};
+struct FinalizeTable {
+  FinalizeSeg seg[kMaxFinalizeSegs];
+  int nseg = 0;
+};
+
+constexpr int kMaxMirrorSegs = 8;
+struct MirrorSeg {
+  long long off = 0;
+  int K = 0, N = 0;
+  void* dst = nullptr;
+};
+struct MirrorTable {
+  MirrorSeg seg[kMaxMirrorSegs];
+  int nseg = 0;
 };
 
 struct EnvParamsK {
diff --git a/gymfx_amd/ops/csrc/ppo_kernels.hip b/gymfx_amd/ops/csrc/ppo_kernels.hip
--- a/gymfx_amd/ops/csrc/ppo_kernels.hip
+++ b/gymfx_amd/ops/csrc/ppo_kernels.hip
@@ -699,6 +699,189 @@
     const float norm = sqrtf(red[0]);
     *scale = (max_norm > 0.f && norm > max_norm) ? max_norm / norm : 1.f;
   }
+}
+
+GFX_DEV unsigned int ticket_draw(unsigned int* ticket) {
+  return __hip_atomic_fetch_add(ticket, 1u, __ATOMIC_RELAXED,
+                                __HIP_MEMORY_SCOPE_AGENT);
+}
+
+template <typename T>
+GFX_DEV void ticket_commit(unsigned int drawn, T* ctr, T old, T delta,
+                           unsigned int* ticket) {
+  if (drawn == gridDim.x - 1u) {
+    *ctr = old + delta;
+    *ticket = 0u;
+  }
+}
+
+__global__ __launch_bounds__(1024) void grads_finalize_kernel(
+    FinalizeTable tab, float* __restrict__ grads, int64_t n,
+    float* __restrict__ clip_part) {
+  __shared__ float comb[4][256];
+  const int t = threadIdx.x & 255;
+  const int q = threadIdx.x >> 8;
+  float sq = 0.f;
+  for (int64_t base = (int64_t)blockIdx.x * 256; base < n;
+       base += (int64_t)gridDim.x * 256) {
+    const int64_t i = base + t;
+    const float* part = nullptr;
+    int64_t elems = 0, e = 0;
+    int slabs = 0, small = 0;
+#pragma unroll
+    for (int s = 0; s < kMaxFinalizeSegs; ++s) {
+      const int64_t d = i - tab.seg[s].off;
+      if (s < tab.nseg && i < n && d >= 0 && d < tab.seg[s].elems) {
+        part = tab.seg[s].part;
+        elems = tab.seg[s].elems;
+        e = d;
+        slabs = tab.seg[s].slabs;
+        small = tab.seg[s].small;
+      }
+    }
+    int kind = -1;
+    float val = 0.f;
+    if (part) {
+      const float* pe = part + e;
+      if (small) {
+        kind = 2;
+        float r[64];
+#pragma unroll
+        for (int m = 0; m < 64; ++m) r[m] = 0.f;
+#pragma unroll
+        for (int h = 0; h < 64; h += 16) {
+          for (int k0 = q + 4 * h; k0 < slabs; k0 += 256) {
+            float x[16];
+#pragma unroll
+            for (int u = 0; u < 16; ++u)
+              x[u] = pe[(int64_t)min(k0 + 4 * u, slabs - 1) * elems];
+#pragma unroll
+            for (int u = 0; u < 16; ++u)
+              r[h + u] += (k0 + 4 * u < slabs) ? x[u] : 0.f;
+          }
+        }
+#pragma unroll
+        for (int w = 32; w > 0; w >>= 1)
+#pragma unroll
+          for (int m = 0; m < w; ++m) r[m] += r[m + w];
+        val = r[0];
+      } else if (e < (elems & ~(int64_t)3)) {
+        kind = 0;
+        const int kend = slabs & ~3;
+        float s = 0.f;
+        int k = q;
+        for (; k + 124 < kend; k += 128) {
+          float x[32];
+#pragma unroll
+          for (int u = 0; u < 32; ++u) x[u] = pe[(int64_t)(k + 4 * u) * elems];
+#pragma unroll
+          for (int u = 0; u < 32; ++u) s += x[u];
+        }
+        for (; k + 60 < kend; k += 64) {
+          float x[16];
+#pragma unroll
+          for (int u = 0; u < 16; ++u) x[u] = pe[(int64_t)(k + 4 * u) * elems];
+#pragma unroll
+          for (int u = 0; u < 16; ++u) s += x[u];
+        }
+        for (; k < kend; k += 4) s += pe[(int64_t)k * elems];
+        if (q == 0)
+          for (k = kend; k < slabs; ++k) s += pe[(int64_t)k * elems];
+        val = s;
+      } else {
+        kind = 1;
+        if (q == 0) {
+          float s = 0.f;
+          for (int k = 0; k < slabs; ++k) s += pe[(int64_t)k * elems];
+          val = s;
+        }
+      }
+    }
+    comb[q][t] = val;
+    __syncthreads();
+    if (q == 0 && i < n) {
+      float g;
+      if (kind == 0)
+        g = (comb[0][t] + comb[1][t]) + (comb[2][t] + comb[3][t]);
+      else if (kind == 2)
+        g = (comb[0][t] + comb[2][t]) + (comb[1][t] + comb[3][t]);
+      else if (kind == 1)
+        g = val;
+      else
+        g = grads[i];
+      if (kind >= 0) grads[i] = g;
+      sq += g * g;
+    }
+    __syncthreads();
+  }
+  if (clip_part) {
+    __shared__ float red[256];
+    if (q == 0) red[t] = sq;
+    __syncthreads();
+    for (int w = 128; w > 0; w >>= 1) {
+      if (q == 0 && t < w) red[t] += red[t + w];
+      __syncthreads();
+    }
+    if (threadIdx.x == 0) clip_part[blockIdx.x] = red[0];
+  }
+}
+
+__global__ __launch_bounds__(1024) void adam_tail_kernel(
+    float* __restrict__ p, const float* __restrict__ g, float* __restrict__ m,
+    float* __restrict__ v, __bf16* __restrict__ p_bf16, int64_t n, float lr,
+    float beta1, float beta2, float eps, int* step_ctr,
+    unsigned int* ticket, const float* __restrict__ clip_part, int nparts,
+    float max_norm, MirrorTable mt) {
+  const int ctr = *(volatile const int*)step_ctr;
+  __syncthreads();
+  unsigned int drawn = 0;
+  const bool drawer = ticket && threadIdx.x == 0;
+  if (drawer) drawn = ticket_draw(ticket);
+  const float st = (float)(ctr + 1);
+  const float bc1 = 1.f - powf(beta1, st);
+  const float bc2 = 1.f - powf(beta2, st);
+  float s = 1.f;
+  if (clip_part) {
+    __shared__ float red[256];
+    if (threadIdx.x < 256) {
+      float acc = 0.f;
+      for (int i = threadIdx.x; i < nparts; i += 256) acc += clip_part[i];
+      red[threadIdx.x] = acc;
+    }
+    __syncthreads();
+    for (int w = 128; w > 0; w >>= 1) {
+      if (threadIdx.x < w) red[threadIdx.x] += red[threadIdx.x + w];
+      __syncthreads();
+    }
+    const float norm = sqrtf(red[0]);
+    s = (max_norm > 0.f && norm > max_norm) ? max_norm / norm : 1.f;
+  }
+  for (int64_t i = (int64_t)blockIdx.x * blockDim.x + threadIdx.x; i < n;
+       i += (int64_t)gridDim.x * blockDim.x) {
+    const float gi = g[i] * s;
+    const float mi = beta1 * m[i] + (1.f - beta1) * gi;
+    const float vi = beta2 * v[i] + (1.f - beta2) * gi * gi;
+    m[i] = mi;
+    v[i] = vi;
+    const float mhat = mi / bc1;
+    const float vhat = vi / bc2;
+    const float pi = p[i] - lr * mhat / (sqrtf(vhat) + eps);
+    p[i] = pi;
+    const __bf16 pb = f2bf(pi);
+    if (p_bf16) p_bf16[i] = pb;
+#pragma unroll
+    for (int sgi = 0; sgi < kMaxMirrorSegs; ++sgi) {
+      const int64_t d = i - mt.seg[sgi].off;
+      if (sgi < mt.nseg && d >= 0 &&
+          d < (int64_t)mt.seg[sgi].K * mt.seg[sgi].N) {
+        const unsigned K = (unsigned)mt.seg[sgi].K, N = (unsigned)mt.seg[sgi].N;
+        const unsigned k = (unsigned)d / N;
+        const unsigned c = (unsigned)d - k * N;
+        reinterpret_cast<__bf16*>(mt.seg[sgi].dst)[(int64_t)c * K + k] = pb;
+      }
+    }
+  }
+  if (drawer) ticket_commit(drawn, step_ctr, ctr, 1, ticket);
 }
 
 __global__ void sample_head_kernel(const float* __restrict__ head, int M,
@@ -1458,6 +1641,7 @@
 }
 
 
+template <bool TICKET>
 __global__ __launch_bounds__(256) void mb_gather_kernel(
     const __bf16* __restrict__ obs_src, const int64_t* __restrict__ act_src,
     const float* __restrict__ logp_src, const float* __restrict__ adv_src,
@@ -1466,11 +1650,20 @@
     float* __restrict__ adv_mb, float* __restrict__ ret_mb, int M, int D,
     uint32_t n, int half, uint64_t seed, int minibatches,
     const unsigned long long* __restrict__ step_base,
-    const unsigned long long* __restrict__ mb_ctr, int skip_obs) {
+    unsigned long long* mb_ctr, int skip_obs, unsigned int* ticket) {
   const int row = blockIdx.x * 4 + (threadIdx.x >> 6);
   const int lane = threadIdx.x & 63;
-  if (row >= M) return;
-  const unsigned long long ctr = *mb_ctr;
+  unsigned long long ctr;
+  if (TICKET) {
+    ctr = *(volatile const unsigned long long*)mb_ctr;
+    __syncthreads();
+    if (threadIdx.x == 0)
+      ticket_commit(ticket_draw(ticket), mb_ctr, ctr, 1ull, ticket);
+    if (row >= M) return;
+  } else {
+    if (row >= M) return;
+    ctr = *mb_ctr;
+  }
   const uint32_t epoch = (uint32_t)(ctr / (unsigned)minibatches);
   const uint32_t mb = (uint32_t)(ctr % (unsigned)minibatches);
   const uint64_t key = splitmix64(seed ^ (*step_base * 0x9E3779B97F4A7C15ull) ^
@@ -1497,6 +1690,7 @@
   }
 }
 
+template <bool TICKET>
 __global__ __launch_bounds__(256) void mb_gather_seq_kernel(
     const __bf16* __restrict__ obs_src,
     const int64_t* __restrict__ act_src,
@@ -1515,11 +1709,20 @@
     int Mseq, int L, int D, int H, int N, uint32_t n_seq, int half,
     uint64_t seed, int minibatches,
     const unsigned long long* __restrict__ step_base,
-    const unsigned long long* __restrict__ mb_ctr) {
+    unsigned long long* mb_ctr, unsigned int* ticket) {
   const int row = blockIdx.x * 4 + (threadIdx.x >> 6);
   const int lane = threadIdx.x & 63;
-  if (row >= Mseq) return;
-  const unsigned long long ctr = *mb_ctr;
+  unsigned long long ctr;
+  if (TICKET) {
+    ctr = *(volatile const unsigned long long*)mb_ctr;
+    __syncthreads();
+    if (threadIdx.x == 0)
+      ticket_commit(ticket_draw(ticket), mb_ctr, ctr, 1ull, ticket);
+    if (row >= Mseq) return;
+  } else {
+    if (row >= Mseq) return;
+    ctr = *mb_ctr;
+  }
   const uint32_t epoch = (uint32_t)(ctr / (unsigned)minibatches);
   const uint32_t mb = (uint32_t)(ctr % (unsigned)minibatches);
   const uint64_t key = splitmix64(seed ^ (*step_base * 0x9E3779B97F4A7C15ull) ^
@@ -1667,16 +1870,21 @@
                           int H, int N, uint32_t n_seq, int half,
                           uint64_t seed, int minibatches,
                           const unsigned long long* step_base,
-                          const unsigned long long* mb_ctr,
+                          unsigned long long* mb_ctr, unsigned int* ticket,
                           hipStream_t stream) {
-  hipLaunchKernelGGL(mb_gather_seq_kernel, dim3(ceil_div(Mseq, 4)), dim3(256),
-                     0, stream, reinterpret_cast<const __bf16*>(obs_src),
-                     act_src, logp_src, adv_src, ret_src, done_src, h0_src,
-                     c0_src, reinterpret_cast<__bf16*>(obs_mb), act_mb,
-                     logp_mb, adv_mb, ret_mb, done_mb,
-                     reinterpret_cast<__bf16*>(h0_mb), c0_mb,
-                     Mseq, L, D, H, N, n_seq, half, seed, minibatches,
-                     step_base, mb_ctr);
+#define GATHER_SEQ(TK)                                                        \
+  hipLaunchKernelGGL(mb_gather_seq_kernel<TK>, dim3(ceil_div(Mseq, 4)),       \
+                     dim3(256), 0, stream,                                    \
+                     reinterpret_cast<const __bf16*>(obs_src), act_src,       \
+                     logp_src, adv_src, ret_src, done_src, h0_src, c0_src,    \
+                     reinterpret_cast<__bf16*>(obs_mb), act_mb, logp_mb,      \
+                     adv_mb, ret_mb, done_mb,                                 \
+                     reinterpret_cast<__bf16*>(h0_mb), c0_mb, Mseq, L, D, H,  \
+                     N, n_seq, half, seed, minibatches, step_base, mb_ctr,    \
+                     ticket)
+  if (ticket) GATHER_SEQ(true);
+  else GATHER_SEQ(false);
+#undef GATHER_SEQ
 }
 
 void launch_mlp_policy_rollout(const void* obs, const void* W1t,
@@ -1715,14 +1923,18 @@
                       float* logp_mb, float* adv_mb, float* ret_mb, int M,
                       int D, uint32_t n, int half, uint64_t seed,
                       int minibatches, const unsigned long long* step_base,
-                      const unsigned long long* mb_ctr, hipStream_t stream,
-                      int skip_obs) {
-  hipLaunchKernelGGL(mb_gather_kernel, dim3(ceil_div(M, 4)), dim3(256), 0,
-                     stream, reinterpret_cast<const __bf16*>(obs_src), act_src,
-                     logp_src, adv_src, ret_src,
-                     reinterpret_cast<__bf16*>(obs_mb), act_mb, logp_mb, adv_mb,
-                     ret_mb, M, D, n, half, seed, minibatches, step_base,
-                     mb_ctr, skip_obs);
+                      unsigned long long* mb_ctr, hipStream_t stream,
+                      int skip_obs, unsigned int* ticket) {
+#define GATHER(TK)                                                            \
+  hipLaunchKernelGGL(mb_gather_kernel<TK>, dim3(ceil_div(M, 4)), dim3(256),   \
+                     0, stream, reinterpret_cast<const __bf16*>(obs_src),     \
+                     act_src, logp_src, adv_src, ret_src,                     \
+                     reinterpret_cast<__bf16*>(obs_mb), act_mb, logp_mb,      \
+                     adv_mb, ret_mb, M, D, n, half, seed, minibatches,        \
+                     step_base, mb_ctr, skip_obs, ticket)
+  if (ticket) GATHER(true);
+  else GATHER(false);
+#undef GATHER
 }
 
 void launch_gemm(const void* A, const void* B, const float* bias, void* C,
@@ -1814,7 +2026,8 @@
 
 void launch_wgrad(const void* X, const void* dY, float* dW_part, float* db_part,
                   float* dW, float* db, int M, int N, int K, int slabs,
-                  hipStream_t stream, const FeistelMap* fmp = nullptr) {
+                  hipStream_t stream, const FeistelMap* fmp = nullptr,
+                  bool reduce = true) {
   const __bf16* x = reinterpret_cast<const __bf16*>(X);
   const __bf16* dy = reinterpret_cast<const __bf16*>(dY);
   static const int big_env = [] {
@@ -1881,6 +2094,7 @@
     }
 #undef WG_PART
   }
+  if (!reduce) return;
   int64_t elems = (int64_t)K * N;
   if (elems <= 4096) {
     hipLaunchKernelGGL(slab_reduce_small_kernel, dim3((int)elems), dim3(256),
@@ -1938,6 +2152,27 @@
                      g, n, part);
 }
 
+void launch_grads_finalize(const FinalizeTable& tab, float* grads, int64_t n,
+                           float* clip_part, hipStream_t stream) {
+  const int blocks =
+      clip_part ? 256 : (int)std::min<int64_t>((n + 255) / 256, 256);
+  hipLaunchKernelGGL(grads_finalize_kernel, dim3(blocks), dim3(1024), 0,
+                     stream, tab, grads, n, clip_part);
+}
+
+void launch_adam_tail(float* p, const float* g, float* m, float* v,
+                      void* p_bf16, int64_t n, float lr, float beta1,
+                      float beta2, float eps, int* step_ctr,
+                      unsigned int* ticket, const float* clip_part, int nparts,
+                      float max_norm, const MirrorTable& mt,
+                      hipStream_t stream) {
+  int blocks = (int)std::min<int64_t>((n + 1023) / 1024, 2048);
+  hipLaunchKernelGGL(adam_tail_kernel, dim3(blocks), dim3(1024), 0, stream, p,
+                     g, m, v, reinterpret_cast<__bf16*>(p_bf16), n, lr, beta1,
+                     beta2, eps, step_ctr, ticket, clip_part, nparts, max_norm,
+                     mt);
+}
+
 void launch_sample_head(const float* head, int M, int n_actions, uint64_t seed,
                         uint64_t step, int64_t* actions, float* logp,
                         float* value, float* entropy, int greedy,
```

Result: faster. 29.14 million env-steps/sec, median of 6 (+2.9%).
